# enfiskutensykkel/nvme-strom

Hardware: AMD Instinct MI355X
Metric: SSD→GPU read GiB/s + p50 4KiB IOP latency at 1/2/4/8 MI355X (higher is better)
Workload: dtype uint8

## Files before the change

csrc/engine/core.cc:

```cpp
#include <errno.h>
#include <fcntl.h>
#include <string.h>
#include <sys/mman.h>
#include <time.h>
#include <unistd.h>
#include <x86intrin.h>

#include <new>

#include <chrono>
#include <cstdio>
#include <cstdlib>

#include "engine.h"

namespace strom {

static bool parse_bool(const std::string &v) {
  return v == "1" || v == "true" || v == "yes" || v == "on";
}

Config Config::from_env() {
  Config c;
  static const char *keys[] = {"backend", "workers", "queue_depth", "max_request",
                               "staging_slots", "staging_bytes", "spin_us", "inline_max",
                               "bar_map", "bar_max", "bar_nt", "inline_plain", "coalesce", "trace",
                               "ingest", "ingest_grid", "ingest_piece", "ingest_min", "ingest_prio", "hdp_sync",
                               "fixed_bufs", "io_prof", "fd_kcmp", "stage_by_bytes", "slot_lifo",
                               "strict", "direct_io",
                               "pgcache_probe", "gpu_emulation", "numa_bind", "check_freed",
                               "stat_info", "verbose"};
  for (const char *k : keys) {
    std::string env = "STROM_";
    for (const char *p = k; *p; ++p) env += (char)toupper(*p);
    if (const char *v = getenv(env.c_str())) c.set(k, v);
  }
  return c;
}

int Config::set(const std::string &k, const std::string &v) {
  char *end = nullptr;
  long n = strtol(v.c_str(), &end, 0);
  bool num_ok = end && *end == '\0' && !v.empty();
  if (k == "backend") {
    if (v == "psync") backend = BackendKind::kPsync;
    else if (v == "uring") backend = BackendKind::kUring;
    else if (v == "fake") backend = BackendKind::kFake;
    else if (v == "cache") backend = BackendKind::kCache;
    else return -EINVAL;
    return 0;
  }
  if (k == "strict") { strict = parse_bool(v); return 0; }
  if (k == "direct_io") { direct_io = parse_bool(v); return 0; }
  if (k == "pgcache_probe") { pgcache_probe = parse_bool(v); return 0; }
  if (k == "gpu_emulation") { gpu_emulation = parse_bool(v); return 0; }
  if (k == "numa_bind") { numa_bind = parse_bool(v); return 0; }
  if (k == "check_freed") { check_freed = parse_bool(v); return 0; }
  if (!num_ok) return -EINVAL;
  if (k == "workers") { if (n < 1 || n > 256) return -EINVAL; workers = (int)n; return 0; }
  if (k == "queue_depth") { if (n < 1 || n > 4096) return -EINVAL; queue_depth = (int)n; return 0; }
  if (k == "max_request") {
    if (n < 4096 || n > (64l << 20) || (n & 4095)) return -EINVAL;
    max_request = (uint32_t)n;
    return 0;
  }
  if (k == "staging_slots") { if (n < 1 || n > 1024) return -EINVAL; staging_slots = (int)n; return 0; }
  if (k == "staging_bytes") {
    if (n < 0 || n > (1l << 30)) return -EINVAL;
    staging_bytes = (uint32_t)n;
    return 0;
  }
  if (k == "spin_us") { if (n < 0 || n > 10000) return -EINVAL; spin_us = (uint32_t)n; return 0; }
  if (k == "bar_map") { bar_map = parse_bool(v); return 0; }
  if (k == "coalesce") { coalesce = parse_bool(v); return 0; }
  if (k == "ingest") { ingest = parse_bool(v); return 0; }
  if (k == "hdp_sync") {
    if (!num_ok) { hdp_sync = parse_bool(v) ? 1 : 0; return 0; }
    if (n < 0 || n > 2) return -EINVAL;
    hdp_sync = (int)n;
    return 0;
  }
  if (k == "fixed_bufs") { fixed_bufs = parse_bool(v); return 0; }
  if (k == "io_prof") { io_prof = parse_bool(v); return 0; }
  if (k == "fd_kcmp") { fd_kcmp = parse_bool(v); return 0; }
  if (k == "stage_by_bytes") { stage_by_bytes = parse_bool(v); return 0; }
  if (k == "slot_lifo") { slot_lifo = parse_bool(v); return 0; }
  if (k == "ingest_min") {
    if (n < 0 || n > (64l << 20)) return -EINVAL;
    ingest_min = (uint32_t)n;
    return 0;
  }
  if (k == "ingest_prio") { if (n < 0 || n > 1) return -EINVAL; ingest_prio = (int)n; return 0; }
  if (k == "ingest_grid") { if (n < 1 || n > 256) return -EINVAL; ingest_grid = (int)n; return 0; }
  if (k == "ingest_piece") {
    if (n < 4096 || n > (16l << 20) || (n & 4095)) return -EINVAL;
    ingest_piece = (uint32_t)n;
    return 0;
  }
  if (k == "trace") { trace = parse_bool(v); return 0; }
  if (k == "bar_max") {
    if (n < 0 || n > (64l << 20)) return -EINVAL;
    bar_max = (uint32_t)n;
    return 0;
  }
  if (k == "inline_plain") { inline_plain = parse_bool(v); return 0; }
  if (k == "bar_nt") {
    if (!num_ok) { bar_nt = parse_bool(v) ? 1 : 0; return 0; }
    if (n < 0 || n > 1) return -EINVAL;
    bar_nt = (int)n;
    return 0;
  }
  if (k == "inline_max") {
    if (n < 0 || n > (16l << 20) || (n & 4095)) return -EINVAL;
    inline_max = (uint32_t)n;
    return 0;
  }
  if (k == "stat_info") { stat_info = (int)n; return 0; }
  if (k == "verbose") { verbose = (int)n; return 0; }
  return -ENOENT;
}

int Config::get(const std::string &k, std::string *out) const {
  char buf[64];
  if (k == "backend") {
    *out = backend == BackendKind::kPsync   ? "psync"
           : backend == BackendKind::kUring ? "uring"
           : backend == BackendKind::kCache ? "cache"
                                            : "fake";
    return 0;
  }
  long v;
  if (k == "workers") v = workers;
  else if (k == "queue_depth") v = queue_depth;
  else if (k == "max_request") v = max_request;
  else if (k == "staging_slots") v = staging_slots;
  else if (k == "staging_bytes") v = staging_bytes;
  else if (k == "spin_us") v = spin_us;
  else if (k == "inline_max") v = inline_max;
  else if (k == "bar_map") v = bar_map;
  else if (k == "coalesce") v = coalesce;
  else if (k == "ingest") v = ingest;
  else if (k == "ingest_grid") v = ingest_grid;
  else if (k == "ingest_prio") v = ingest_prio;
  else if (k == "ingest_piece") v = ingest_piece;
  else if (k == "hdp_sync") v = hdp_sync;
  else if (k == "fixed_bufs") v = fixed_bufs;
  else if (k == "io_prof") v = io_prof;
  else if (k == "fd_kcmp") v = fd_kcmp;
  else if (k == "stage_by_bytes") v = stage_by_bytes;
  else if (k == "slot_lifo") v = slot_lifo;
  else if (k == "ingest_min") v = ingest_min;
  else if (k == "trace") v = trace;
  else if (k == "bar_max") v = bar_max;
  else if (k == "bar_nt") v = bar_nt;
  else if (k == "inline_plain") v = inline_plain;
  else if (k == "strict") v = strict;
  else if (k == "direct_io") v = direct_io;
  else if (k == "pgcache_probe") v = pgcache_probe;
  else if (k == "gpu_emulation") v = gpu_emulation;
  else if (k == "numa_bind") v = numa_bind;
  else if (k == "check_freed") v = check_freed;
  else if (k == "stat_info") v = stat_info;
  else if (k == "verbose") v = verbose;
  else return -ENOENT;
  snprintf(buf, sizeof buf, "%ld", v);
  *out = buf;
  return 0;
}

Config &config() {
  static Config c = Config::from_env();
  return c;
}

uint64_t tsc_now() { return __rdtsc(); }

uint64_t mono_ns() {
  timespec ts;
  clock_gettime(CLOCK_MONOTONIC, &ts);
  return (uint64_t)ts.tv_sec * 1000000000ull + (uint64_t)ts.tv_nsec;
}

uint64_t tsc_khz() {
  static const uint64_t khz = [] {
    const uint64_t n0 = mono_ns(), c0 = tsc_now();
    while (mono_ns() - n0 < 5000000) _mm_pause();
    const uint64_t n1 = mono_ns(), c1 = tsc_now();
    return (c1 - c0) * 1000000ull / (n1 - n0);
  }();
  return khz;
}

void Hist::add(uint64_t ns) { b[bucket(ns)].fetch_add(1, std::memory_order_relaxed); }

void Hist::copy_to(uint64_t *out, bool reset) {
  for (int i = 0; i < STROM_HIST_BUCKETS; ++i)
    out[i] = reset ? b[i].exchange(0) : b[i].load();
}

void Stats::inflight_inc(uint64_t n) {
  uint64_t cur = cur_dma_count.fetch_add(n, std::memory_order_relaxed) + n;
  uint64_t mx = max_dma_count.load(std::memory_order_relaxed);
  while (cur > mx && !max_dma_count.compare_exchange_weak(mx, cur)) {
  }
}

void Stats::inflight_dec(uint64_t n) { cur_dma_count.fetch_sub(n, std::memory_order_relaxed); }

int Stats::fill(strom_stat_info *o) {
  if (o->version != 1) return -EINVAL;
  int level = config().stat_info;
  if (level == 0) return -ENODATA;
  o->has_debug = level >= 2;
  o->tsc = tsc_now();
  o->nr_ssd2gpu = nr_ssd2gpu.load();
  o->clk_ssd2gpu = clk_ssd2gpu.load();
  o->nr_setup_prps = nr_setup_prps.load();
  o->clk_setup_prps = clk_setup_prps.load();
  o->nr_submit_dma = nr_submit_dma.load();
  o->clk_submit_dma = clk_submit_dma.load();
  o->nr_wait_dtask = nr_wait_dtask.load();
  o->clk_wait_dtask = clk_wait_dtask.load();
  o->nr_wrong_wakeup = nr_wrong_wakeup.load();
  o->cur_dma_count = cur_dma_count.load();
  o->max_dma_count = max_dma_count.exchange(cur_dma_count.load());
  uint64_t *dn[4] = {&o->nr_debug1, &o->nr_debug2, &o->nr_debug3, &o->nr_debug4};
  uint64_t *dc[4] = {&o->clk_debug1, &o->clk_debug2, &o->clk_debug3, &o->clk_debug4};
  for (int i = 0; i < 4; ++i) {
    *dn[i] = o->has_debug ? nr_debug[i].load() : 0;
    *dc[i] = o->has_debug ? clk_debug[i].load() : 0;
  }
  return 0;
}

int Stats::fill_hist(strom_stat_hist *o) {
  if (o->version != 1) return -EINVAL;
  bool r = o->reset != 0;
  io_ns.copy_to(o->io_ns, r);
  copy_ns.copy_to(o->copy_ns, r);
  task_ns.copy_to(o->task_ns, r);
  return 0;
}

static Stats *make_stats() {
  const char *off = getenv("STROM_STAT_SHM");
  if (!(off && strcmp(off, "0") == 0)) {
    char path[96];
    snprintf(path, sizeof path, "/dev/shm/nvme-strom.%d", (int)getpid());
    int fd = open(path, O_RDWR | O_CREAT | O_TRUNC | O_CLOEXEC, 0644);
    if (fd >= 0) {
      size_t len = sizeof(StatsShmHeader) + sizeof(Stats);
      if (ftruncate(fd, (off_t)len) == 0) {
        void *p = mmap(nullptr, len, PROT_READ | PROT_WRITE, MAP_SHARED, fd, 0);
        if (p != MAP_FAILED) {
          close(fd);
          auto *h = new (p) StatsShmHeader();
          h->magic = kStatsShmMagic;
          h->version = 1;
          h->pid = getpid();
          h->stats_bytes = sizeof(Stats);
          h->tsc_hz_hint = 0;
          static char saved[96];
          memcpy(saved, path, sizeof saved);
          atexit([] { unlink(saved); });
          return new ((char *)p + sizeof(StatsShmHeader)) Stats();
        }
      }
      close(fd);
      unlink(path);
    }
  }
  return new Stats();
}

Stats &stats() {
  static Stats *s = make_stats();
  return *s;
}

CallerProf &caller_prof() {
  static CallerProf p;
  return p;
}

Task *TaskTable::create(int session) {
  Task *t = new Task();
  t->id = next_id_.fetch_add(1);
  t->session = session;
  t->t_start_ns = mono_ns();
  Slot &s = slot_of(t->id);
  std::lock_guard<std::mutex> g(s.mu);
  s.running.emplace(t->id, t);
  return t;
}

void TaskTable::get(Task *t, int n) {
  t->refcnt.fetch_add(n, std::memory_order_relaxed);
}

void TaskTable::put_n(Task *t, int n, long status) {
  if (status != 0) {
    long zero = 0;
    t->status.compare_exchange_strong(zero, status);
  }
  if (t->refcnt.fetch_sub(n, std::memory_order_acq_rel) != n) return;
  stats().task_ns.add(mono_ns() - t->t_start_ns);
  Slot &s = slot_of(t->id);
  {
    std::lock_guard<std::mutex> g(s.mu);
    s.running.erase(t->id);
    s.done_seq.fetch_add(1, std::memory_order_release);
    if (t->status.load() != 0) {
      t->gmap.reset();
      t->dbuf.reset();
      s.failed.emplace(t->id, t);
      t = nullptr;
    }
  }
  s.cv.notify_all();
  delete t;
}

int TaskTable::wait(uint64_t id, long *status, int64_t timeout_ns) {
  Slot &s = slot_of(id);
  uint64_t t0 = tsc_now();
  bool slept = false;
  auto deadline = std::chrono::steady_clock::now() +
                  std::chrono::nanoseconds(timeout_ns < 0 ? 0 : timeout_ns);
  std::unique_lock<std::mutex> g(s.mu);
  int rc;
  bool spun = false;
  uint64_t spin_end = 0;
  for (;;) {
    auto f = s.failed.find(id);
    if (f != s.failed.end()) {
      *status = f->second->status.load();
      delete f->second;
      s.failed.erase(f);
      rc = -EIO;
      break;
    }
    if (s.running.count(id)) {
      if (timeout_ns == 0) { rc = -ETIME; break; }
      if (!spun) {
        spun = true;
        uint64_t spin_ns = (uint64_t)config().spin_us * 1000;
        if (timeout_ns > 0 && (uint64_t)timeout_ns < spin_ns) spin_ns = (uint64_t)timeout_ns;
        spin_end = mono_ns() + spin_ns;
      }
      if (mono_ns() < spin_end) {
        const uint64_t seq0 = s.done_seq.load(std::memory_order_acquire);
        g.unlock();
        while (s.done_seq.load(std::memory_order_acquire) == seq0 && mono_ns() < spin_end)
          for (int i = 0; i < 32; ++i) _mm_pause();
        g.lock();
        continue;
      }
      if (slept) stats().nr_wrong_wakeup++;
      slept = true;
      if (timeout_ns < 0) {
        s.cv.wait(g);
      } else if (s.cv.wait_until(g, deadline) == std::cv_status::timeout &&
                 s.running.count(id)) {
        rc = -ETIME;
        break;
      }
      continue;
    }
    *status = 0;
    rc = (id == 0 || id > last_id()) ? -ENOENT : 0;
    break;
  }
  if (slept) {
    stats().nr_wait_dtask++;
    stats().clk_wait_dtask += tsc_now() - t0;
  }
  return rc;
}

int TaskTable::reclaim(int session) {
  int n = 0;
  for (auto &s : slots_) {
    std::lock_guard<std::mutex> g(s.mu);
    for (auto it = s.failed.begin(); it != s.failed.end();) {
      if (it->second->session == session) {
        delete it->second;
        it = s.failed.erase(it);
        ++n;
      } else {
        ++it;
      }
    }
  }
  return n;
}

TaskTable &tasks() {
  static TaskTable t;
  return t;
}

int FaultInjector::on_request(uint32_t *len) {
  long fa = fail_at.load(std::memory_order_relaxed);
  long sa = short_at.load(std::memory_order_relaxed);
  int d = delay_us.load(std::memory_order_relaxed);
  if (!fa && !sa && !d) return 0;
  long n = counter.fetch_add(1) + 1;
  if (d) {
    timespec ts{0, (long)d * 1000};
    nanosleep(&ts, nullptr);
  }
  if (fa && n == fa) return -err.load();
  if (sa && n == sa) {
    int sb = short_bytes.load();
    *len = (uint32_t)sb >= *len ? 0 : *len - (uint32_t)sb;
  }
  return 0;
}

FaultInjector &faults() {
  static FaultInjector f;
  return f;
}

}
```

csrc/engine/engine.cc:

```cpp
#include <errno.h>
#include <fcntl.h>
#include <stdio.h>
#include <stdlib.h>
#include <string.h>
#include <sys/ioctl.h>
#include <sys/mman.h>
#include <sys/stat.h>
#include <sys/syscall.h>
#include <sys/sysmacros.h>
#include <unistd.h>
#include <x86intrin.h>

#include <rocprofiler-sdk-roctx/roctx.h>

#include <algorithm>
#include <set>
#include <thread>

#include "engine.h"

namespace strom {
static thread_local bool tl_sync_call = false;
thread_local uint64_t *tl_phase = nullptr;


struct Engine::OpenFile {
  dev_t dev = 0;
  ino_t ino = 0;
  struct timespec ctim {};
  off_t vsize = -1;
  int fd_direct = -1;
  int fd_buffered = -1;
  FileClass fc;
  std::mutex mu;
  void *map = nullptr;
  size_t map_len = 0;
  ~OpenFile() {
    if (map) munmap(map, map_len);
    if (fd_direct >= 0 && fd_direct != fd_buffered) close(fd_direct);
    if (fd_buffered >= 0) close(fd_buffered);
  }
  long resident(uint64_t off, uint32_t len) {
    if (!map) return -1;
    if (off >= map_len) return 0;
    uint32_t n = (uint32_t)std::min<uint64_t>(len, map_len - off);
    unsigned char vec[1024];
    uint32_t pages = (n + 4095) / 4096;
    long res = 0;
    for (uint32_t p = 0; p < pages; p += 1024) {
      uint32_t cnt = std::min<uint32_t>(1024, pages - p);
      if (mincore((char *)map + off + (uint64_t)p * 4096, (size_t)cnt * 4096, vec) != 0) return -1;
      for (uint32_t i = 0; i < cnt; ++i) res += vec[i] & 1;
    }
    return res;
  }
};

struct Engine::StripeSet {
  std::vector<std::shared_ptr<OpenFile>> m;
  uint32_t unit = 0;
  uint64_t size = 0;
  Raid0Geometry geo{};
  int numa = -1;
};

static std::mutex g_stripes_mu;
static std::map<int, std::shared_ptr<Engine::StripeSet>> g_stripes;
static int g_next_stripe = 0;

static int stripe_ident_bmap(void *, uint64_t fblk, uint64_t *dblk) {
  *dblk = fblk;
  return 0;
}

static std::mutex g_engine_mu;
static Engine *g_engine = nullptr;

Engine &engine() {
  std::lock_guard<std::mutex> g(g_engine_mu);
  if (!g_engine) g_engine = new Engine();
  return *g_engine;
}

void engine_reset() {
  std::lock_guard<std::mutex> g(g_engine_mu);
  delete g_engine;
  g_engine = nullptr;
}

static std::atomic<uint64_t> g_engine_gen{0};

Engine::Engine() : gen_(g_engine_gen.fetch_add(1) + 1) { io_ = std::make_unique<IoEngine>(config()); }
Engine::~Engine() { io_.reset(); }

static std::atomic<int> g_kcmp{-1};

static bool same_description(int fd, int dup) {
  const pid_t me = getpid();
  const long r = syscall(SYS_kcmp, me, me, 0 , fd, dup);
  if (r < 0 && g_kcmp.load(std::memory_order_relaxed) != 1) g_kcmp.store(0);
  return r == 0;
}

struct TlFile {
  int fd = -1;
  int dup = -1;
  uint64_t eng = 0;
  std::shared_ptr<Engine::OpenFile> f;
  ~TlFile() {
    if (dup >= 0) close(dup);
  }
};
static thread_local TlFile tl_file;

void Engine::forget_cached_file() {
  tl_file.f.reset();
  tl_file.fd = -1;
}

const std::shared_ptr<Engine::OpenFile> &Engine::open_file_cached(int fd, int *err, bool *fast) {
  TlFile &tl = tl_file;
  static const std::shared_ptr<OpenFile> none;
  if (fast) *fast = false;
  const bool use_kcmp = config().fd_kcmp && g_kcmp.load(std::memory_order_relaxed) != 0;
  if (use_kcmp && tl.fd == fd && tl.eng == gen_ && tl.f && tl.dup >= 0 &&
      same_description(fd, tl.dup)) {
    g_kcmp.store(1, std::memory_order_relaxed);
    if (fast) *fast = true;
    return tl.f;
  }
  struct stat st;
  if (fstat(fd, &st) != 0) {
    *err = -errno;
    return none;
  }
  const OpenFile *c = tl.f.get();
  const bool same = tl.fd == fd && tl.eng == gen_ && c && c->dev == st.st_dev && c->ino == st.st_ino &&
                    c->vsize == st.st_size && c->ctim.tv_sec == st.st_ctim.tv_sec &&
                    c->ctim.tv_nsec == st.st_ctim.tv_nsec;
  if (!same) {
    tl.f = open_file(fd, err);
    tl.eng = gen_;
    if (!tl.f) {
      tl.fd = -1;
      return none;
    }
  }
  if (!use_kcmp) {
    if (tl.dup >= 0) close(tl.dup);
    tl.dup = -1;
  } else if (tl.fd != fd || tl.dup < 0 || !same) {
    if (tl.dup >= 0) close(tl.dup);
    tl.dup = fcntl(fd, F_DUPFD_CLOEXEC, 0);
  }
  tl.fd = fd;
  return tl.f;
}

struct TlReg {
  int rfd = -1;
  uint64_t eng = 0, ver = 0;
  std::shared_ptr<Engine::OpenFile> f;
};
static thread_local TlReg tl_reg;

const std::shared_ptr<Engine::OpenFile> &Engine::registered(int rfd) {
  TlReg &tl = tl_reg;
  if (tl.rfd == rfd && tl.eng == gen_ && tl.ver == reg_ver_.load(std::memory_order_acquire))
    return tl.f;
  std::lock_guard<std::mutex> g(reg_mu_);
  const uint32_t i = (uint32_t)(rfd - kRegFdBase);
  tl.f = is_registered_id(rfd) && i < reg_.size() ? reg_[i] : nullptr;
  tl.rfd = rfd;
  tl.eng = gen_;
  tl.ver = reg_ver_.load(std::memory_order_relaxed);
  return tl.f;
}

int Engine::register_file(int fd) {
  if (fd >= kRegFdBase) return -EINVAL;
  int err = 0;
  auto f = open_file(fd, &err);
  if (!f) return err ? err : -EBADF;
  std::lock_guard<std::mutex> g(reg_mu_);
  size_t i = 0;
  while (i < reg_.size() && reg_[i]) ++i;
  if (i >= (size_t)kRegMax) return -EMFILE;
  if (i == reg_.size()) reg_.emplace_back();
  reg_[i] = std::move(f);
  reg_ver_.fetch_add(1, std::memory_order_release);
  return kRegFdBase + (int)i;
}

int Engine::unregister_file(int rfd) {
  std::lock_guard<std::mutex> g(reg_mu_);
  const uint32_t i = (uint32_t)(rfd - kRegFdBase);
  if (!is_registered_id(rfd) || i >= reg_.size() || !reg_[i]) return -EBADF;
  reg_[i].reset();
  reg_ver_.fetch_add(1, std::memory_order_release);
  return 0;
}

void Engine::refresh_registered(int rfd) {
  std::shared_ptr<OpenFile> f = registered(rfd);
  if (!f) return;
  int err = 0;
  auto nf = open_file(f->fd_buffered, &err);
  if (!nf || nf == f) return;
  std::lock_guard<std::mutex> g(reg_mu_);
  const uint32_t i = (uint32_t)(rfd - kRegFdBase);
  if (i < reg_.size() && reg_[i] == f) {
    reg_[i] = nf;
    reg_ver_.fetch_add(1, std::memory_order_release);
  }
}

std::shared_ptr<Engine::OpenFile> Engine::task_file(int fd, int *err) {
  if (is_registered_id(fd)) refresh_registered(fd);
  return open_file(fd, err);
}

std::shared_ptr<Engine::OpenFile> Engine::open_file(int fd, int *err) {
  if (is_registered_id(fd)) {
    std::shared_ptr<OpenFile> f = registered(fd);
    if (!f) *err = -EBADF;
    return f;
  }
  struct stat st;
  if (fstat(fd, &st) != 0) {
    *err = -errno;
    return nullptr;
  }
  std::lock_guard<std::mutex> g(files_mu_);
  auto key = std::make_pair(st.st_dev, st.st_ino);
  auto it = files_.find(key);
  if (it != files_.end()) {
    std::shared_ptr<OpenFile> f = it->second;
    if (f->vsize == st.st_size && f->ctim.tv_sec == st.st_ctim.tv_sec &&
        f->ctim.tv_nsec == st.st_ctim.tv_nsec)
      return f;
    struct stat cst;
    bool stale = fstat(f->fd_buffered, &cst) != 0 || cst.st_nlink == 0 ||
                 cst.st_ino != st.st_ino;
    if (!stale) {
      f->ctim = st.st_ctim;
      f->vsize = st.st_size;
      if ((off_t)f->fc.size != st.st_size) {
        std::lock_guard<std::mutex> fg(f->mu);
        f->fc.size = st.st_size;
        if (f->map) munmap(f->map, f->map_len);
        f->map = nullptr;
        if (config().pgcache_probe && st.st_size > 0) {
          void *m = mmap(nullptr, (size_t)st.st_size, PROT_READ, MAP_SHARED, f->fd_buffered, 0);
          if (m != MAP_FAILED) {
            f->map = m;
            f->map_len = (size_t)st.st_size;
          }
        }
      }
      return f;
    }
    files_.erase(it);
  }
  auto f = std::make_shared<OpenFile>();
  int rc = classify_file(fd, &f->fc, config().strict);
  if (rc) {
    *err = rc;
    return nullptr;
  }
  char path[64];
  snprintf(path, sizeof path, "/proc/self/fd/%d", fd);
  f->fd_buffered = open(path, O_RDONLY | O_CLOEXEC);
  if (f->fd_buffered < 0) f->fd_buffered = fcntl(fd, F_DUPFD_CLOEXEC, 0);
  if (f->fd_buffered < 0) {
    *err = -errno;
    return nullptr;
  }
  f->fd_direct = f->fd_buffered;
  if (config().direct_io) {
    int d = open(path, O_RDONLY | O_DIRECT | O_CLOEXEC);
    if (d >= 0) f->fd_direct = d;
  }
  f->dev = st.st_dev;
  f->ino = st.st_ino;
  f->ctim = st.st_ctim;
  f->vsize = st.st_size;
  if (config().pgcache_probe && st.st_size > 0) {
    void *m = mmap(nullptr, (size_t)st.st_size, PROT_READ, MAP_SHARED, f->fd_buffered, 0);
    if (m != MAP_FAILED) {
      f->map = m;
      f->map_len = (size_t)st.st_size;
    }
  }
  if (files_.size() > 256) files_.clear();
  files_[key] = f;
  return f;
}

static void attach_residency(Engine::OpenFile *fp, PlanParams *pp,
                             std::vector<unsigned char> *vec, uint64_t *lo_out) {
  uint64_t lo = UINT64_MAX, hi = 0;
  for (uint32_t i = 0; i < pp->nr_chunks; ++i) {
    uint64_t c = pp->relseg_sz ? pp->ids[i] % pp->relseg_sz : pp->ids[i];
    uint64_t f = c * pp->chunk_sz;
    lo = std::min(lo, f);
    hi = std::max(hi, f + pp->chunk_sz);
  }
  hi = std::min<uint64_t>(hi, fp->map_len);
  uint64_t total = (uint64_t)pp->nr_chunks * pp->chunk_sz;
  uint64_t t0 = tsc_now();
  if (lo < hi && hi - lo <= 4 * total) {
    vec->resize((hi - lo + 4095) / 4096);
    if (mincore((char *)fp->map + lo, hi - lo, vec->data()) == 0) {
      *lo_out = lo;
      std::vector<unsigned char> *v = vec;
      uint64_t base = lo, end = hi;
      pp->resident = [v, base, end](uint64_t off, uint32_t len) -> long {
        if (off >= end) return 0;
        uint64_t e = std::min<uint64_t>(off + len, end);
        long r = 0;
        for (uint64_t p = (off - base) >> 12; p < ((e - base + 4095) >> 12); ++p) r += (*v)[p] & 1;
        return r;
      };
      stats().nr_debug[2].fetch_add(1, std::memory_order_relaxed);
      stats().clk_debug[2].fetch_add(tsc_now() - t0, std::memory_order_relaxed);
      return;
    }
  }
  pp->resident = [fp](uint64_t off, uint32_t len) { return fp->resident(off, len); };
}

int Engine::stripe_open(const int *fds, uint32_t n, uint32_t unit, uint64_t size) {
  if (!fds || n == 0 || n > STROM_RAID0_MAX_DISKS) return -EINVAL;
  if (unit < 4096 || (unit & 4095) || size == 0) return -EINVAL;
  auto ss = std::make_shared<StripeSet>();
  ss->unit = unit;
  ss->size = size;
  const uint64_t nstripes = (size + unit - 1) / unit;
  std::set<int> nodes;
  for (uint32_t k = 0; k < n; ++k) {
    int err = 0;
    auto f = open_file(fds[k], &err);
    if (!f) return err;
    const uint64_t mine = nstripes > k ? (nstripes - k + n - 1) / n : 0;
    uint64_t need = mine * (uint64_t)unit;
    if (mine && (nstripes - 1) % n == k) need -= (uint64_t)unit * nstripes - size;
    if ((uint64_t)f->fc.size < need) return -ERANGE;
    nodes.insert(f->fc.numa_node);
    ss->m.push_back(f);
  }
  ss->numa = nodes.size() == 1 ? *nodes.begin() : -1;
  Raid0Geometry &g = ss->geo;
  g.chunk_sects = unit >> 9;
  g.nzones = 1;
  g.ndisks = n;
  const uint64_t rows = (nstripes + n - 1) / n + ((64ull << 20) / ((uint64_t)unit * n)) + 1;
  g.zone_end[0] = rows * n * (uint64_t)(unit >> 9);
  g.zone_dev_start[0] = 0;
  g.zone_nb_dev[0] = n;
  for (uint32_t k = 0; k < n; ++k) g.zone_devs[0][k] = (uint8_t)k;
  if (strom_core_raid0_check(&g)) return -EINVAL;
  std::lock_guard<std::mutex> l(g_stripes_mu);
  if (g_stripes.size() >= 4096) return -EMFILE;
  int fd;
  do {
    fd = kStripeFdBase + (g_next_stripe++ & 0xffffff);
  } while (g_stripes.count(fd));
  g_stripes[fd] = ss;
  return fd;
}

int Engine::stripe_close(int sfd) {
  std::lock_guard<std::mutex> l(g_stripes_mu);
  return g_stripes.erase(sfd) ? 0 : -EBADF;
}

std::shared_ptr<Engine::StripeSet> Engine::stripe(int fd) {
  if (fd < kStripeFdBase) return nullptr;
  std::lock_guard<std::mutex> l(g_stripes_mu);
  auto it = g_stripes.find(fd);
  return it == g_stripes.end() ? nullptr : it->second;
}

int Engine::check_file(strom_check_file *a) {
  if (a->fdesc >= kStripeFdBase) {
    auto ss = stripe(a->fdesc);
    if (!ss) return -EBADF;
    a->numa_node_id = ss->numa;
    a->support_dma64 = 1;
    return 0;
  }
  FileClass fc;
  if (is_registered_id(a->fdesc)) {
    int err = 0;
    const auto f = task_file(a->fdesc, &err);
    if (!f) return err ? err : -EBADF;
    fc = f->fc;
  } else {
    int rc = classify_file(a->fdesc, &fc, config().strict);
    if (rc) return rc;
  }
  a->numa_node_id = fc.numa_node;
  a->support_dma64 = fc.dma64 ? 1 : 0;
  return 0;
}

static int copy_ram_chunks(int fd, const ChunkPlan &plan, uint32_t chunk_sz, uint64_t file_size,
                           char *dest_base) {
  uint64_t t0 = tsc_now();
  for (size_t i = 0; i < plan.ram_fpos.size(); ++i) {
    char *dst = dest_base + plan.ram_dest[i];
    uint64_t fpos = plan.ram_fpos[i];
    uint32_t want = (uint32_t)std::min<uint64_t>(chunk_sz, file_size - fpos);
    uint32_t done = 0;
    while (done < want) {
      ssize_t n = pread(fd, dst + done, want - done, (off_t)(fpos + done));
      if (n < 0) {
        if (errno == EINTR) continue;
        return -errno;
      }
      if (n == 0) break;
      done += (uint32_t)n;
    }
    if (done < chunk_sz) memset(dst + done, 0, chunk_sz - done);
  }
  stats().nr_debug[1].fetch_add(plan.ram_fpos.size(), std::memory_order_relaxed);
  stats().clk_debug[1].fetch_add(tsc_now() - t0, std::memory_order_relaxed);
  return 0;
}

static void build_requests(Task *t, const ChunkPlan &plan, int fd_direct, int fd_buffered,
                           uint64_t file_size, GpuMapping *gmap, uint64_t dest_base,
                           bool dest_is_host, std::vector<IoReq> *out,
                           const Engine::StripeSet *ss = nullptr) {
  uint64_t t0 = tsc_now();
  out->reserve(plan.ssd.size());
  const uint64_t now_ns = mono_ns(), now_tsc = tsc_now();
  for (const IoRange &r : plan.ssd) {
    IoReq q;
    q.task = t;
    q.fd = fd_direct;
    q.fd_buffered = fd_buffered;
    q.off = r.file_off;
    q.len = r.len;
    q.valid = (uint32_t)std::min<uint64_t>(r.len, file_size > r.file_off ? file_size - r.file_off : 0);
    if (ss && r.member >= 0) {
      const auto &mf = ss->m[(size_t)r.member];
      q.fd = mf->fd_direct;
      q.fd_buffered = mf->fd_buffered;
      q.off = r.msect << 9;
    }
    if (dest_is_host) {
      q.host_dst = (uint8_t *)(dest_base + r.dest_off);
    } else {
      q.gpu_dst = dest_base + r.dest_off;
      q.device = gmap->device;
    }
    q.gmap = gmap;
    q.t_submit_ns = now_ns;
    q.t_submit_tsc = now_tsc;
    out->push_back(q);
  }
  if (const int n = (int)plan.ssd.size()) {
    tasks().get(t, n);
    if (gmap) gmap->inflight.fetch_add(n);
    stats().inflight_inc((uint64_t)n);
  }
  stats().nr_setup_prps.fetch_add(plan.ssd.size(), std::memory_order_relaxed);
  stats().clk_setup_prps.fetch_add(tsc_now() - t0, std::memory_order_relaxed);
}

int Engine::memcpy_ssd2gpu(int session, strom_memcpy_ssd2gpu *a) {
  a->nr_ram2gpu = a->nr_ssd2gpu = a->nr_dma_submit = a->nr_dma_blocks = 0;
  a->dma_task_id = 0;
  if (a->nr_chunks == 0) return -EINVAL;
  if (!a->chunk_ids) return -EFAULT;
  auto gmap = gpu_registry().get(a->handle);
  if (!gmap) return -ENOENT;
  if (int v = gpu_registry().validate(gmap)) return v;
  uint64_t bytes = (uint64_t)a->nr_chunks * a->chunk_sz;
  if (strom_core_check_range(gmap->map_length - gmap->map_offset, a->offset, bytes))
    return -ERANGE;
  int err = 0;
  auto ss = stripe(a->file_desc);
  std::shared_ptr<OpenFile> f;
  if (!ss) {
    if (a->file_desc >= kStripeFdBase) return -EBADF;
    f = task_file(a->file_desc, &err);
    if (!f) return err;
  }

  PlanParams pp;
  pp.ids = a->chunk_ids;
  pp.nr_chunks = a->nr_chunks;
  pp.chunk_sz = a->chunk_sz;
  pp.relseg_sz = a->relseg_sz;
  pp.file_size = ss ? ss->size : (uint64_t)f->fc.size;
  pp.max_request = config().max_request;
  pp.reorder = true;
  if (ss) {
    pp.raid0 = &ss->geo;
    pp.bmap = stripe_ident_bmap;
  }
  phase_mark(0);
  const uint64_t c0 = tsc_now();
  std::vector<unsigned char> resv;
  uint64_t res_lo = 0;
  if (f && config().pgcache_probe && f->map) attach_residency(f.get(), &pp, &resv, &res_lo);
  ChunkPlan plan;
  int rc = plan_chunks(pp, &plan);
  if (rc) return rc;
  phase_mark(1);
  const uint64_t c1 = tsc_now();
  char *ram_dest = a->wb_buffer;
  if (plan.nr_ram && !ram_dest) {
    uint64_t dva = gmap->va + a->offset;
    if (!gmap->bar || dva < gmap->bar_va || dva + bytes > gmap->bar_va + gmap->bar_len)
      return -EFAULT;
    ram_dest = (char *)gmap->bar + (dva - gmap->bar_va);
  }

  Task *t = tasks().create(session);
  t->gmap = gmap;
  bool host_dest = gmap->device < 0;
  std::vector<IoReq> reqs;
  build_requests(t, plan, f ? f->fd_direct : -1, f ? f->fd_buffered : -1, pp.file_size,
                 gmap.get(), gmap->va + a->offset, host_dest, &reqs, ss.get());
  phase_mark(2);
  uint64_t t0 = tsc_now();
  if (reqs.size() == 1 && (reqs[0].len <= config().inline_max || tl_sync_call))
    io_->run_inline(reqs[0]);
  else
    io_->submit(reqs);
  const uint64_t t1 = tsc_now();
  stats().nr_submit_dma.fetch_add(reqs.size(), std::memory_order_relaxed);
  stats().clk_submit_dma.fetch_add(t1 - t0, std::memory_order_relaxed);
  if (config().io_prof) {
    CallerProf &cp = caller_prof();
    cp.calls.fetch_add(1, std::memory_order_relaxed);
    cp.plan.fetch_add(c1 - c0, std::memory_order_relaxed);
    cp.build.fetch_add(t0 - c1, std::memory_order_relaxed);
    cp.submit.fetch_add(t1 - t0, std::memory_order_relaxed);
  }

  if (plan.nr_ram && f) {
    rc = copy_ram_chunks(f->fd_buffered, plan, a->chunk_sz, pp.file_size, ram_dest);
    if (rc == 0 && !a->wb_buffer) gmap->bar_flush((const uint8_t *)ram_dest, true);
  }
  t->frozen = true;
  uint64_t id = t->id;
  tasks().put(t, rc);
  if (rc) {
    long st;
    tasks().wait(id, &st, -1);
    return rc;
  }
  a->dma_task_id = id;
  a->nr_ram2gpu = plan.nr_ram;
  a->nr_ssd2gpu = plan.nr_ssd;
  a->nr_dma_submit = plan.nr_submit;
  a->nr_dma_blocks = plan.nr_blocks;
  memcpy(a->chunk_ids, plan.ids_out.data(), sizeof(uint32_t) * a->nr_chunks);
  return 0;
}

int Engine::memcpy_extents(int session, strom_memcpy_ssd2gpu_extents *a) {
  a->dma_task_id = 0;
  a->nr_dma_submit = a->nr_dma_blocks = 0;
  a->bytes_read = a->gap_bytes = a->dst_bytes = 0;
  if (a->nr_extents && !a->extents) return -EFAULT;
  if (a->nr_extents > (1u << 24) || (a->flags & ~STROM_EXTENTS_PLAN_ONLY)) return -EINVAL;
  int err = 0;
  auto ss = stripe(a->file_desc);
  std::shared_ptr<OpenFile> f;
  if (!ss) {
    if (a->file_desc >= kStripeFdBase) return -EBADF;
    f = task_file(a->file_desc, &err);
    if (!f) return err;
  }
  PlanParams pp;
  pp.file_size = ss ? ss->size : (uint64_t)f->fc.size;
  pp.max_request = config().max_request;
  if (ss) {
    pp.raid0 = &ss->geo;
    pp.bmap = stripe_ident_bmap;
  }
  const bool plan_only = a->flags & STROM_EXTENTS_PLAN_ONLY;
  std::shared_ptr<GpuMapping> gmap;
  if (!plan_only) {
    gmap = gpu_registry().get(a->handle);
    if (!gmap) return -ENOENT;
    if (int v = gpu_registry().validate(gmap)) return v;
  }
  ChunkPlan plan;
  uint64_t dst_bytes = 0, read_bytes = 0;
  int rc = plan_xfer(pp, a->extents, a->nr_extents, a->gap_max, !plan_only, &plan, &dst_bytes,
                     &read_bytes);
  if (rc) return rc;
  uint64_t want = 0;
  for (uint32_t i = 0; i < a->nr_extents; ++i) want += a->extents[i].len;
  a->dst_bytes = dst_bytes;
  a->bytes_read = read_bytes;
  a->gap_bytes = read_bytes - want;
  if (plan_only) return 0;
  if (strom_core_check_range(gmap->map_length - gmap->map_offset, a->offset, dst_bytes))
    return -ERANGE;
  Task *t = tasks().create(session);
  t->gmap = gmap;
  const bool host_dest = gmap->device < 0;
  std::vector<IoReq> reqs;
  build_requests(t, plan, f ? f->fd_direct : -1, f ? f->fd_buffered : -1, pp.file_size,
                 gmap.get(), gmap->va + a->offset, host_dest, &reqs, ss.get());
  const uint64_t t0 = tsc_now();
  if (reqs.size() == 1 && (reqs[0].len <= config().inline_max || tl_sync_call))
    io_->run_inline(reqs[0]);
  else if (!reqs.empty())
    io_->submit(reqs);
  stats().nr_submit_dma.fetch_add(reqs.size(), std::memory_order_relaxed);
  stats().clk_submit_dma.fetch_add(tsc_now() - t0, std::memory_order_relaxed);
  t->frozen = true;
  const uint64_t id = t->id;
  tasks().put(t, 0);
  a->dma_task_id = id;
  a->nr_dma_submit = plan.nr_submit;
  a->nr_dma_blocks = plan.nr_blocks;
  return 0;
}

long Engine::pread_sync(unsigned long handle, size_t offset, int fd, uint64_t file_off,
                        uint64_t len, bool checked) {
  if (len > (16u << 20)) return -EAGAIN;
  if (fd >= kStripeFdBase) return -EAGAIN;
  const auto &gmap = gpu_registry().get_cached(handle);
  if (!gmap) return -ENOENT;
  if (int v = gpu_registry().validate(gmap)) return v;
  if (strom_core_check_range(gmap->map_length - gmap->map_offset, offset, len)) return -ERANGE;
  phase_mark(0);
  int err = 0;
  bool fast = false;
  const bool reg = is_registered_id(fd);
  const auto &f = reg ? registered(fd) : open_file_cached(fd, &err, &fast);
  if (!f) return reg ? -EBADF : err;
  fast |= reg;
  auto recheck = [&] {
    if (reg) refresh_registered(fd);
    else forget_cached_file();
    return pread_sync(handle, offset, fd, file_off, len, true);
  };
  const uint64_t size = (uint64_t)f->fc.size;
  if (file_off >= size) {
    if (!fast || checked) return -ERANGE;
    return recheck();
  }
  phase_mark(1);
  long status = 0;
  IoReq r;
  r.fd = f->fd_direct;
  r.fd_buffered = f->fd_buffered;
  r.off = file_off;
  r.len = (uint32_t)len;
  r.valid = (uint32_t)std::min<uint64_t>(len, size - file_off);
  if (gmap->device < 0) r.host_dst = (uint8_t *)(gmap->va + offset);
  else r.gpu_dst = gmap->va + offset;
  r.device = gmap->device;
  r.gmap = gmap.get();
  r.status_out = &status;
  r.t_submit_ns = mono_ns();
  r.t_submit_tsc = tsc_now();
  gmap->inflight.fetch_add(1);
  stats().inflight_inc();
  stats().nr_setup_prps.fetch_add(1, std::memory_order_relaxed);
  phase_mark(2);
  io_->run_inline(r);
  if (status == -EIO && fast && !checked) {
    return recheck();
  }
  if (status) return status;
  return (long)len;
}

int Engine::memcpy_ssd2ram(int session, strom_memcpy_ssd2ram *a) {
  a->nr_ram2ram = a->nr_ssd2ram = a->nr_dma_submit = a->nr_dma_blocks = 0;
  a->dma_task_id = 0;
  if (a->nr_chunks == 0) return -EINVAL;
  if (!a->chunk_ids || !a->dest_uaddr) return -EFAULT;
  uint64_t bytes = (uint64_t)a->nr_chunks * a->chunk_sz;
  std::shared_ptr<DmaBuffer> dbuf;
  size_t dest_off = 0;
  int rc = dmabuf_registry().resolve(a->dest_uaddr, bytes, &dbuf, &dest_off);
  if (rc) return rc;
  int err = 0;
  auto ss = stripe(a->file_desc);
  std::shared_ptr<OpenFile> f;
  if (!ss) {
    if (a->file_desc >= kStripeFdBase) return -EBADF;
    f = task_file(a->file_desc, &err);
    if (!f) return err;
  }

  PlanParams pp;
  pp.ids = a->chunk_ids;
  pp.nr_chunks = a->nr_chunks;
  pp.chunk_sz = a->chunk_sz;
  pp.relseg_sz = a->relseg_sz;
  pp.file_size = ss ? ss->size : (uint64_t)f->fc.size;
  pp.max_request = config().max_request;
  pp.reorder = false;
  if (ss) {
    pp.raid0 = &ss->geo;
    pp.bmap = stripe_ident_bmap;
  }
  std::vector<unsigned char> resv;
  uint64_t res_lo = 0;
  if (f && config().pgcache_probe && f->map) attach_residency(f.get(), &pp, &resv, &res_lo);
  ChunkPlan plan;
  rc = plan_chunks(pp, &plan);
  if (rc) return rc;

  Task *t = tasks().create(session);
  t->dbuf = dbuf;
  std::vector<IoReq> reqs;
  build_requests(t, plan, f ? f->fd_direct : -1, f ? f->fd_buffered : -1, pp.file_size, nullptr,
                 (uint64_t)a->dest_uaddr, true, &reqs, ss.get());
  uint64_t t0 = tsc_now();
  if (reqs.size() == 1 && (reqs[0].len <= config().inline_max || tl_sync_call))
    io_->run_inline(reqs[0]);
  else
    io_->submit(reqs);
  stats().nr_submit_dma.fetch_add(reqs.size(), std::memory_order_relaxed);
  stats().clk_submit_dma.fetch_add(tsc_now() - t0, std::memory_order_relaxed);
  if (plan.nr_ram && f)
    rc = copy_ram_chunks(f->fd_buffered, plan, a->chunk_sz, pp.file_size, (char *)a->dest_uaddr);
  t->frozen = true;
  uint64_t id = t->id;
  tasks().put(t, rc);
  if (rc) {
    long st;
    tasks().wait(id, &st, -1);
    return rc;
  }
  a->dma_task_id = id;
  a->nr_ram2ram = plan.nr_ram;
  a->nr_ssd2ram = plan.nr_ssd;
  a->nr_dma_submit = plan.nr_submit;
  a->nr_dma_blocks = plan.nr_blocks;
  return 0;
}

int Engine::memcpy_wait(strom_memcpy_wait *a) {
  long st = 0;
  int rc = tasks().wait(a->dma_task_id, &st, -1);
  a->status = st;
  return rc;
}

int Engine::memcpy_wait_timed(strom_memcpy_wait_timed *a) {
  long st = 0;
  int rc = tasks().wait(a->dma_task_id, &st, (int64_t)a->timeout_ns);
  a->status = st;
  return rc;
}

namespace {
const char *cmd_name(unsigned long cmd) {
  switch (cmd) {
    case STROM_IOCTL__CHECK_FILE: return "strom:CHECK_FILE";
    case STROM_IOCTL__MAP_GPU_MEMORY: return "strom:MAP_GPU_MEMORY";
    case STROM_IOCTL__MAP_GPU_DMABUF: return "strom:MAP_GPU_DMABUF";
    case STROM_IOCTL__UNMAP_GPU_MEMORY: return "strom:UNMAP_GPU_MEMORY";
    case STROM_IOCTL__MEMCPY_SSD2GPU: return "strom:MEMCPY_SSD2GPU";
    case STROM_IOCTL__MEMCPY_SSD2RAM: return "strom:MEMCPY_SSD2RAM";
    case STROM_IOCTL__MEMCPY_WAIT: return "strom:MEMCPY_WAIT";
    case STROM_IOCTL__MEMCPY_WAIT_TIMED: return "strom:MEMCPY_WAIT_TIMED";
    case STROM_IOCTL__MEMCPY_SSD2GPU_EXTENTS: return "strom:MEMCPY_SSD2GPU_EXTENTS";
    default: return "strom:ioctl";
  }
}
struct TraceRange {
  bool on;
  explicit TraceRange(unsigned long cmd) : on(config().trace) {
    if (on) roctxRangePushA(cmd_name(cmd));
  }
  ~TraceRange() {
    if (on) roctxRangePop();
  }
};
}

int Engine::ioctl(int session, unsigned long cmd, void *arg) {
  if (!arg) return -EFAULT;
  TraceRange tr(cmd);
  switch (cmd) {
    case STROM_IOCTL__CHECK_FILE:
      return check_file((strom_check_file *)arg);
    case STROM_IOCTL__MAP_GPU_MEMORY: {
      auto *a = (strom_map_gpu_memory *)arg;
      return gpu_registry().map(a->vaddress, a->length, -1, a);
    }
    case STROM_IOCTL__MAP_GPU_DMABUF: {
      auto *a = (strom_map_gpu_dmabuf *)arg;
      strom_map_gpu_memory m{};
      int rc = gpu_registry().map(a->vaddress, a->length, a->dmabuf_fd, &m);
      a->handle = m.handle;
      a->gpu_page_sz = m.gpu_page_sz;
      a->gpu_npages = m.gpu_npages;
      return rc;
    }
    case STROM_IOCTL__UNMAP_GPU_MEMORY:
      return gpu_registry().unmap(((strom_unmap_gpu_memory *)arg)->handle);
    case STROM_IOCTL__LIST_GPU_MEMORY:
      return gpu_registry().list((strom_list_gpu_memory *)arg);
    case STROM_IOCTL__INFO_GPU_MEMORY:
      return gpu_registry().info((strom_info_gpu_memory *)arg);
    case STROM_IOCTL__ALLOC_DMA_BUFFER: {
      auto *a = (strom_alloc_dma_buffer *)arg;
      return dmabuf_registry().alloc(a->length, a->node_id, &a->dmabuf_fdesc);
    }
    case STROM_IOCTL__MEMCPY_SSD2GPU:
      return memcpy_ssd2gpu(session, (strom_memcpy_ssd2gpu *)arg);
    case STROM_IOCTL__MEMCPY_SSD2RAM:
      return memcpy_ssd2ram(session, (strom_memcpy_ssd2ram *)arg);
    case STROM_IOCTL__MEMCPY_SSD2GPU_EXTENTS:
      return memcpy_extents(session, (strom_memcpy_ssd2gpu_extents *)arg);
    case STROM_IOCTL__MEMCPY_WAIT:
      return memcpy_wait((strom_memcpy_wait *)arg);
    case STROM_IOCTL__MEMCPY_WAIT_TIMED:
      return memcpy_wait_timed((strom_memcpy_wait_timed *)arg);
    case STROM_IOCTL__STAT_INFO:
      return stats().fill((strom_stat_info *)arg);
    case STROM_IOCTL__STAT_HIST:
      return stats().fill_hist((strom_stat_hist *)arg);
    case STROM_IOCTL__SET_ROUTE:
      return -EOPNOTSUPP;
    default:
      return -EINVAL;
  }
}

}

using namespace strom;

static std::mutex g_sess_mu;
static int g_next_session = 1;
static std::atomic<int> g_kernel_fd{-2};

static int kernel_fd() {
  const int k = g_kernel_fd.load(std::memory_order_acquire);
  if (k != -2) return k;
  std::lock_guard<std::mutex> g(g_sess_mu);
  int fd = g_kernel_fd.load(std::memory_order_relaxed);
  if (fd != -2) return fd;
  const char *prov = getenv("STROM_PROVIDER");
  if (prov && strcmp(prov, "user") == 0) {
    fd = -1;
  } else {
    fd = open(STROM_DEVICE_PATHNAME, O_RDONLY | O_CLOEXEC);
    if (fd < 0) fd = open(NVME_STROM_IOCTL_PATHNAME, O_RDONLY | O_CLOEXEC);
  }
  g_kernel_fd.store(fd, std::memory_order_release);
  return fd;
}

static int kernel_map_gpu(int kfd, strom_map_gpu_memory *a) {
  if (!hip::available()) return -ENODEV;
  int dfd = -1, dev = -1;
  uint64_t off = 0;
  int rc = hip::export_dmabuf(a->vaddress, a->length, &dfd, &off, &dev);
  if (rc) return rc;
  strom_map_gpu_dmabuf m{};
  m.dmabuf_fd = dfd;
  m.device_id = dev;
  m.vaddress = a->vaddress;
  m.length = a->length;
  m.dmabuf_offset = off;
  int r = ioctl(kfd, STROM_IOCTL__MAP_GPU_DMABUF, &m);
  int e = errno;
  close(dfd);
  if (r < 0) return -e;
  a->handle = m.handle;
  a->gpu_page_sz = m.gpu_page_sz;
  a->gpu_npages = m.gpu_npages;
  return 0;
}

extern "C" {

const char *strom_version(void) { return "strom-mi355x 0.1.0 (abi nvme-strom 0.6)"; }

int strom_provider(void) { return kernel_fd() >= 0 ? 1 : 0; }

int strom_open(void) {
  std::lock_guard<std::mutex> g(g_sess_mu);
  return g_next_session++;
}

int strom_close(int session) {
  if (session <= 0) return -EBADF;
  int n = tasks().reclaim(session);
  if (n) STROM_LOG(0, "session %d closed with %d unclaimed failed task(s)", session, n);
  return n;
}

int strom_ioctl(int session, unsigned long cmd, void *arg) {
  const int kfd = kernel_fd();
  if (kfd >= 0) {
    if (cmd == STROM_IOCTL__MAP_GPU_MEMORY) return kernel_map_gpu(kfd, (strom_map_gpu_memory *)arg);
    int r = ioctl(kfd, cmd, arg);
    return r < 0 ? -errno : r;
  }
  return engine().ioctl(session, cmd, arg);
}

int nvme_strom_ioctl(unsigned long cmd, const void *arg) {
  static thread_local int session = 0;
  if (session == 0) session = strom_open();
  int r = strom_ioctl(session, cmd, (void *)arg);
  if (r < 0) {
    errno = -r;
    return -1;
  }
  return r;
}

long strom_pread_gpu(int session, unsigned long handle, size_t offset, int fd,
                     uint64_t file_off, uint64_t len) {
  if ((file_off | len) & 4095) return -EINVAL;
  if (len == 0) return 0;
  {
    const int kfd = kernel_fd();
    if (kfd < 0) {
      const long r = engine().pread_sync(handle, offset, fd, file_off, len);
      if (r != -EAGAIN) return r;
    }
  }
  uint32_t chunk = 4096;
  for (uint32_t c = config().max_request; c > 4096; c >>= 1)
    if (file_off % c == 0 && len % c == 0) {
      chunk = c;
      break;
    }
  uint64_t n = len / chunk;
  if (n > (1u << 24) || (file_off / chunk + n) > 0xffffffffull) return -E2BIG;
  uint32_t ids_small[16];
  std::vector<uint32_t> ids_big;
  uint32_t *ids = ids_small;
  if (n > 16) {
    ids_big.resize(n);
    ids = ids_big.data();
  }
  for (uint64_t i = 0; i < n; ++i) ids[i] = (uint32_t)(file_off / chunk + i);
  auto gmap = gpu_registry().get(handle);
  if (!gmap) return -ENOENT;
  strom_memcpy_ssd2gpu a{};
  a.handle = handle;
  a.offset = offset;
  a.file_desc = fd;
  a.nr_chunks = (unsigned)n;
  a.chunk_sz = chunk;
  a.chunk_ids = ids;
  std::vector<char> wb;
  if (!gmap->bar) {
    wb.resize(len);
    a.wb_buffer = wb.data();
  }
  strom::tl_sync_call = true;
  int rc = strom_ioctl(session, STROM_IOCTL__MEMCPY_SSD2GPU, &a);
  strom::tl_sync_call = false;
  if (rc) return rc;
  strom_memcpy_wait w{};
  w.dma_task_id = a.dma_task_id;
  rc = strom_ioctl(session, STROM_IOCTL__MEMCPY_WAIT, &w);
  if (rc) return rc;
  if (a.nr_ram2gpu) {
    uint64_t dva = gmap->va + offset;
    const bool host = gmap->device < 0;
    auto hipMemcpyDtoH_wrap = [&](void *dst, uint64_t src, size_t nb) -> int {
      if (host) {
        memcpy(dst, (const void *)src, nb);
        return 0;
      }
      return hip::copy_dtoh(dst, src, nb);
    };
    auto hipMemcpyHtoD_wrap = [&](uint64_t dst, const void *src, size_t nb) -> int {
      if (host) {
        memcpy((void *)dst, src, nb);
        return 0;
      }
      return hip::copy_htod(dst, src, nb);
    };
    std::vector<char> tmp(len);
    const char *src = gmap->bar ? (const char *)gmap->bar + (dva - gmap->bar_va) : nullptr;
    if (!src) {
      if (hipMemcpyDtoH_wrap(tmp.data(), dva, (size_t)a.nr_ssd2gpu * chunk) != 0) return -EIO;
      memcpy(tmp.data() + (size_t)a.nr_ssd2gpu * chunk, wb.data() + (size_t)a.nr_ssd2gpu * chunk,
             (size_t)a.nr_ram2gpu * chunk);
    } else {
      memcpy(tmp.data(), src, len);
    }
    std::vector<char> out(len);
    for (uint64_t i = 0; i < n; ++i) {
      uint64_t pos = ids[i] - file_off / chunk;
      memcpy(out.data() + pos * chunk, tmp.data() + i * chunk, chunk);
    }
    if (gmap->bar) {
      if (!gmap->bar_write(dva, out.data(), len)) return -EIO;
    } else if (hipMemcpyHtoD_wrap(dva, out.data(), len) != 0) {
      return -EIO;
    }
  }
  return (long)len;
}

int strom_pread_gpu_lat(int session, unsigned long handle, size_t offset, int fd,
                        const uint64_t *file_offs, uint32_t n, uint64_t len, uint64_t *ns_out) {
  for (uint32_t i = 0; i < n; ++i) {
    const uint64_t t0 = mono_ns();
    const long r = strom_pread_gpu(session, handle, offset, fd, file_offs[i], len);
    ns_out[i] = mono_ns() - t0;
    if (r < 0) return (int)r;
  }
  return 0;
}

int strom_ioctl_lat(int session, unsigned long handle, size_t offset, int fd,
                    const uint64_t *file_offs, uint32_t n, uint64_t len, uint64_t *ns_out) {
  if (len == 0 || (len & 4095) || len > (1u << 20)) return -EINVAL;
  uint32_t ids[256];
  const uint32_t chunk = 4096, nch = (uint32_t)(len / chunk);
  std::vector<char> wb(len);
  for (uint32_t i = 0; i < n; ++i) {
    const uint64_t t0 = mono_ns();
    for (uint32_t k = 0; k < nch; ++k) ids[k] = (uint32_t)(file_offs[i] / chunk + k);
    strom_memcpy_ssd2gpu a{};
    a.handle = handle;
    a.offset = offset;
    a.file_desc = fd;
    a.nr_chunks = nch;
    a.chunk_sz = chunk;
    a.chunk_ids = ids;
    a.wb_buffer = wb.data();
    int rc = strom_ioctl(session, STROM_IOCTL__MEMCPY_SSD2GPU, &a);
    if (rc) return rc;
    strom_memcpy_wait w{};
    w.dma_task_id = a.dma_task_id;
    rc = strom_ioctl(session, STROM_IOCTL__MEMCPY_WAIT, &w);
    ns_out[i] = mono_ns() - t0;
    if (rc) return rc;
  }
  return 0;
}

int strom_pread_gpu_phases(int session, unsigned long handle, size_t offset, int fd,
                           const uint64_t *file_offs, uint32_t n, uint64_t len,
                           uint64_t *phase_ns) {
  uint64_t st[STROM_NPHASE];
  for (uint32_t i = 0; i < n; ++i) {
    memset(st, 0, sizeof st);
    strom::tl_phase = st;
    const uint64_t t0 = mono_ns();
    const long r = strom_pread_gpu(session, handle, offset, fd, file_offs[i], len);
    st[STROM_NPHASE - 1] = mono_ns();
    strom::tl_phase = nullptr;
    if (r < 0) return (int)r;
    for (int k = 0; k < STROM_NPHASE; ++k)
      phase_ns[(size_t)i * STROM_NPHASE + k] = st[k] ? st[k] - t0 : 0;
  }
  return 0;
}

int strom_pread_raw_lat(int fd, const uint64_t *file_offs, uint32_t n, uint64_t len,
                        uint64_t *ns_out) {
  if (len == 0 || (len & 4095)) return -EINVAL;
  char path[64];
  snprintf(path, sizeof path, "/proc/self/fd/%d", fd);
  int d = open(path, O_RDONLY | O_DIRECT | O_CLOEXEC);
  if (d < 0) return -errno;
  void *buf = nullptr;
  if (posix_memalign(&buf, 4096, len) != 0) {
    close(d);
    return -ENOMEM;
  }
  int rc = 0;
  for (uint32_t i = 0; i < n && rc == 0; ++i) {
    const uint64_t t0 = mono_ns();
    const ssize_t got = pread(d, buf, len, (off_t)file_offs[i]);
    ns_out[i] = mono_ns() - t0;
    if (got < 0) rc = -errno;
  }
  free(buf);
  close(d);
  return rc;
}

int strom_pread_pair_lat(int session, unsigned long handle, size_t offset, int fd,
                         const uint64_t *file_offs, uint32_t npairs, uint64_t len,
                         uint64_t *ns_engine, uint64_t *ns_raw) {
  if (len == 0 || (len & 4095)) return -EINVAL;
  int real = fd;
  if (is_registered_id(fd)) {
    const auto &f = engine().registered(fd);
    if (!f) return -EBADF;
    real = f->fd_buffered;
  }
  char path[64];
  snprintf(path, sizeof path, "/proc/self/fd/%d", real);
  int d = open(path, O_RDONLY | O_DIRECT | O_CLOEXEC);
  if (d < 0) return -errno;
  void *buf = nullptr;
  if (posix_memalign(&buf, 4096, len) != 0) {
    close(d);
    return -ENOMEM;
  }
  int rc = 0;
  for (uint32_t i = 0; i < npairs && rc == 0; ++i) {
    for (int side = 0; side < 2 && rc == 0; ++side) {
      const bool raw = (side == 0) == ((i & 1) == 0);
      const uint64_t off = file_offs[2 * i + (raw ? 0 : 1)];
      const uint64_t t0 = mono_ns();
      if (raw) {
        const ssize_t got = pread(d, buf, len, (off_t)off);
        ns_raw[i] = mono_ns() - t0;
        if (got < 0) rc = -errno;
      } else {
        const long r = strom_pread_gpu(session, handle, offset, fd, off, len);
        ns_engine[i] = mono_ns() - t0;
        if (r < 0) rc = (int)r;
      }
    }
  }
  free(buf);
  close(d);
  return rc;
}

int strom_host_costs(int fd, uint64_t *out, int n) {
  if (n <= 0 || fd < 0) return -EINVAL;
  auto bench = [&](auto &&fn) {
    const uint64_t t0 = mono_ns();
    for (int i = 0; i < n; ++i) fn();
    return (mono_ns() - t0) / (uint64_t)n;
  };
  volatile uint64_t sink = 0;
  timespec ts;
  out[0] = bench([&] { clock_gettime(CLOCK_MONOTONIC, &ts); sink += ts.tv_nsec; });
  out[1] = bench([&] { sink += __rdtsc(); });
  struct stat st;
  out[2] = bench([&] { fstat(fd, &st); sink += st.st_size; });
  void *m = mmap(nullptr, 4096, PROT_READ, MAP_SHARED, fd, 0);
  unsigned char v = 0;
  out[3] = m == MAP_FAILED ? 0 : bench([&] { mincore(m, 4096, &v); sink += v; });
  if (m != MAP_FAILED) munmap(m, 4096);
  out[4] = bench([&] { sink += (uint64_t)getppid(); });
  std::mutex mu;
  out[5] = bench([&] { std::lock_guard<std::mutex> g(mu); sink += 1; });
  std::condition_variable cv;
  out[6] = bench([&] { cv.notify_all(); });
  const int d = fcntl(fd, F_DUPFD_CLOEXEC, 0);
  const pid_t me = getpid();
  out[7] = d < 0 || syscall(SYS_kcmp, me, me, 0 , fd, d) != 0
               ? 0
               : bench([&] { sink += (uint64_t)syscall(SYS_kcmp, me, me, 0, fd, d); });
  if (d >= 0) close(d);
  struct statx sx;
  out[8] = bench([&] {
    statx(fd, "", AT_EMPTY_PATH | AT_STATX_DONT_SYNC, STATX_INO, &sx);
    sink += sx.stx_ino;
  });
  return 0;
}

int strom_engine_costs(unsigned long handle, int fd, uint64_t *out, int n) {
  using namespace strom;
  if (n <= 0 || fd < 0) return -EINVAL;
  auto bench = [&](auto &&fn) {
    const uint64_t t0 = mono_ns();
    for (int i = 0; i < n; ++i) fn();
    return (mono_ns() - t0) / (uint64_t)n;
  };
  volatile uint64_t sink = 0;
  auto g = gpu_registry().get(handle);
  if (!g) return -ENOENT;
  out[0] = bench([&] { sink += (uint64_t)(gpu_registry().get(handle) != nullptr); });
  out[1] = bench([&] { sink += (uint64_t)gpu_registry().validate(g); });
  int err = 0;
  out[2] = bench([&] { sink += (uint64_t)(engine().open_file(fd, &err) != nullptr); });
  out[3] = bench([&] {
    Stats &st = stats();
    st.copy_ns.add(1000);
    st.nr_debug[0].fetch_add(1, std::memory_order_relaxed);
    st.inflight_inc();
    g->inflight.fetch_add(1);
    long status = 0;
    IoReq r;
    r.gmap = g.get();
    r.status_out = &status;
    r.t_submit_tsc = tsc_now();
    finish_request(r, 0);
    sink += (uint64_t)status;
  });
  out[4] = bench([&] { sink += (uint64_t)(gpu_registry().get_cached(handle) != nullptr); });
  out[5] = bench([&] { sink += (uint64_t)(engine().open_file_cached(fd, &err) != nullptr); });
  for (int k = 6; k < 16; ++k) out[k] = 0;
  if (g->bar && g->length >= 4096 && g->va >= g->bar_va && g->va + 4096 <= g->bar_va + g->bar_len) {
    alignas(64) static thread_local uint8_t keep[4096], src[4096];
    memcpy(keep, g->bar + (g->va - g->bar_va), 4096);
    memcpy(src, keep, 4096);
    std::atomic<uint64_t> ctr{0};
    for (int mode = 0; mode < 4; ++mode) {
      uint64_t store = 0, lock = 0;
      for (int i = 0; i < n; ++i) {
        const uint64_t t0 = mono_ns();
        g->bar_write_mode(g->va, src, 4096, mode);
        const uint64_t t1 = mono_ns();
        ctr.fetch_add(1);
        const uint64_t t2 = mono_ns();
        store += t1 - t0;
        lock += t2 - t1;
      }
      out[6 + 2 * mode] = store / (uint64_t)n;
      out[7 + 2 * mode] = lock / (uint64_t)n;
    }
    for (int variant = 0; variant < 2; ++variant) {
      std::atomic<uint64_t> go{0}, done{0};
      std::atomic<bool> quit{false};
      std::thread helper([&] {
        uint64_t seen = 0;
        while (!quit.load(std::memory_order_acquire)) {
          const uint64_t v = go.load(std::memory_order_acquire);
          if (v == seen) {
            _mm_pause();
            continue;
          }
          seen = v;
          if (variant == 0) g->bar_write_mode(g->va + 2048, src + 2048, 2048, 1);
          done.fetch_add(1, std::memory_order_acq_rel);
        }
      });
      uint64_t tot = 0;
      for (int i = 0; i < n; ++i) {
        const uint64_t t0 = mono_ns();
        go.fetch_add(1, std::memory_order_acq_rel);
        if (variant == 0) g->bar_write_mode(g->va, src, 2048, 1);
        ctr.fetch_add(1);
        while (done.load(std::memory_order_acquire) != (uint64_t)i + 1) _mm_pause();
        tot += mono_ns() - t0;
      }
      quit.store(true, std::memory_order_release);
      helper.join();
      out[14 + variant] = tot / (uint64_t)n;
    }
    g->bar_write(g->va, keep, 4096, true);
    sink += ctr.load();
  }
  return 0;
}

void *strom_dmabuf_mmap(int fd, size_t length) {
  void *p = nullptr;
  if (kernel_fd() >= 0) {
    p = mmap(nullptr, length, PROT_READ | PROT_WRITE, MAP_SHARED, fd, 0);
    return p == MAP_FAILED ? nullptr : p;
  }
  int rc = dmabuf_registry().map(fd, length, &p);
  if (rc) {
    errno = -rc;
    return nullptr;
  }
  return p;
}

int strom_dmabuf_munmap(void *addr, size_t length) {
  if (kernel_fd() >= 0) return munmap(addr, length) == 0 ? 0 : -errno;
  return dmabuf_registry().unmap(addr, length);
}

int strom_dmabuf_gc(void) { return dmabuf_registry().gc(); }

int strom_stripe_open(const int *fds, uint32_t n, uint32_t unit, uint64_t size) {
  if (kernel_fd() >= 0) return -EOPNOTSUPP;
  return engine().stripe_open(fds, n, unit, size);
}

int strom_stripe_close(int sfd) { return engine().stripe_close(sfd); }

int strom_register_file(int fd) { return engine().register_file(fd); }
int strom_unregister_file(int rfd) { return engine().unregister_file(rfd); }

int strom_file_topology(int fd, strom_file_topo *out) {
  if (!out) return -EFAULT;
  FileClass fc;
  int rc = classify_file(fd, &fc, false);
  if (rc) return rc;
  memset(out, 0, sizeof *out);
  out->dev_major = major(fc.dev);
  out->dev_minor = minor(fc.dev);
  out->numa_node = fc.numa_node;
  snprintf(out->fs_name, sizeof out->fs_name, "%s", fc.fs_name.c_str());
  snprintf(out->disk, sizeof out->disk, "%s", fc.disk.c_str());
  std::vector<std::string> members;
  if (fc.md_raid0) members = fc.members;
  else if (!fc.disk.empty()) members.push_back(fc.disk);
  for (auto &m : members) {
    if (out->nmembers >= STROM_TOPO_MAX_MEMBERS) break;
    std::string disk = m;
    size_t pp = disk.rfind('p');
    if (pp != std::string::npos && disk.compare(0, 4, "nvme") == 0 &&
        disk.find('n', 4) != std::string::npos && disk.find('n', 4) < pp)
      disk = disk.substr(0, pp);
    snprintf(out->member_disk[out->nmembers], 32, "%s", m.c_str());
    snprintf(out->member_pci[out->nmembers], 16, "%s", nvme_controller_bdf(disk).c_str());
    ++out->nmembers;
  }
  return 0;
}


long strom_gpu_detached(void) { return (long)gpu_registry().detached_count(); }

long strom_gpu_bar_bytes(unsigned long handle) {
  auto m = gpu_registry().get(handle);
  if (!m) return -ENOENT;
  return (long)(m->bar ? m->bar_len : 0);
}

int strom_export_dmabuf(uint64_t va, uint64_t len, int *fd, uint64_t *offset) {
  if (!hip::available()) return -ENODEV;
  int dev = -1;
  return hip::export_dmabuf(va, len, fd, offset, &dev);
}

int strom_config_set(const char *key, const char *value) {
  std::lock_guard<std::mutex> g(g_engine_mu);
  return config().set(key, value);
}

int strom_config_get(const char *key, char *buf, size_t buflen) {
  std::string v;
  int rc = config().get(key, &v);
  if (rc) return rc;
  if (v.size() + 1 > buflen) return -ENOSPC;
  memcpy(buf, v.c_str(), v.size() + 1);
  return 0;
}

int strom_engine_reset(void) {
  engine_reset();
  return 0;
}

int strom_fake_backend(uint64_t seed, uint64_t *completions, uint64_t *reordered) {
  FaultInjector &f = faults();
  if (seed) f.fake_seed = seed;
  if (completions) *completions = f.fake_completions.load();
  if (reordered) *reordered = f.fake_reordered.load();
  return 0;
}

int strom_fault_inject(long fail_at, int err, long short_at, int short_bytes, int delay_us) {
  FaultInjector &f = faults();
  f.counter = 0;
  f.fail_at = fail_at;
  f.err = err ? err : EIO;
  f.short_at = short_at;
  f.short_bytes = short_bytes;
  f.delay_us = delay_us;
  return 0;
}

long strom_resident_bytes(int fd, uint64_t offset, uint64_t length) {
  struct stat st;
  if (fstat(fd, &st) != 0) return -errno;
  if (offset >= (uint64_t)st.st_size) return 0;
  length = std::min<uint64_t>(length, (uint64_t)st.st_size - offset);
  uint64_t lo = offset & ~4095ull;
  size_t maplen = (size_t)(offset + length - lo);
  void *m = mmap(nullptr, maplen, PROT_READ, MAP_SHARED, fd, (off_t)lo);
  if (m == MAP_FAILED) return -errno;
  size_t pages = (maplen + 4095) / 4096;
  std::vector<unsigned char> vec(pages);
  long res = 0;
  if (mincore(m, maplen, vec.data()) == 0) {
    for (auto v : vec) res += v & 1;
  } else {
    res = -errno;
  }
  munmap(m, maplen);
  return res < 0 ? res : res * 4096;
}

int strom_evict_file(int fd) {
  fdatasync(fd);
  int r = posix_fadvise(fd, 0, 0, POSIX_FADV_DONTNEED);
  return -r;
}

int strom_raid0_map(const uint64_t *zone_end, const uint64_t *zone_dev_start,
                    const int *zone_nb_dev, int nzones, uint32_t chunk_sects,
                    const uint64_t *data_offset, int raid_disks, uint64_t sector,
                    uint32_t nr_sects, int *member, uint64_t *member_sector) {
  if (nzones <= 0 || nzones > STROM_RAID0_MAX_ZONES || raid_disks <= 0 ||
      raid_disks > STROM_RAID0_MAX_DISKS)
    return -EINVAL;
  strom_raid0 g;
  memset(&g, 0, sizeof g);
  g.chunk_sects = chunk_sects;
  g.nzones = (uint32_t)nzones;
  g.ndisks = (uint32_t)raid_disks;
  for (int z = 0; z < nzones; ++z) {
    g.zone_end[z] = zone_end[z];
    g.zone_dev_start[z] = zone_dev_start[z];
    if (zone_nb_dev[z] <= 0 || zone_nb_dev[z] > raid_disks) return -EINVAL;
    g.zone_nb_dev[z] = (uint32_t)zone_nb_dev[z];
    for (int k = 0; k < zone_nb_dev[z]; ++k)
      g.zone_devs[z][k] = (uint8_t)(raid_disks - zone_nb_dev[z] + k);
  }
  for (int d = 0; d < raid_disks; ++d) g.data_offset[d] = data_offset ? data_offset[d] : 0;
  return strom_core_raid0_map(&g, sector, nr_sects, member, member_sector);
}

}
```

csrc/engine/engine.h:

```cpp
#pragma once

#include <sys/types.h>

#include <atomic>
#include <condition_variable>
#include <cstdint>
#include <deque>
#include <functional>
#include <map>
#include <memory>
#include <mutex>
#include <string>
#include <thread>
#include <unordered_map>
#include <vector>

#include "strom/strom.h"
#include "../../kmod/strom_core.h"

namespace strom {

enum class BackendKind { kPsync, kUring, kFake, kCache };

struct Config {
  BackendKind backend = BackendKind::kUring;
  int workers = 4;
  int queue_depth = 8;
  uint32_t max_request = 1u << 20;
  int staging_slots = 4;
  bool slot_lifo = true;
  bool stage_by_bytes = true;
  uint32_t staging_bytes = 0;
  uint32_t spin_us = 20;
  uint32_t inline_max = 64u << 10;
  bool bar_map = true;
  bool coalesce = true;
  bool ingest = true;
  int ingest_grid = 16;
  int ingest_prio = 1;
  uint32_t ingest_piece = 256u << 10;
  int hdp_sync = 2;
  bool fixed_bufs = true;
  uint32_t bar_max = 256u << 10;
  int bar_nt = 1;
  bool inline_plain = false;
  uint32_t ingest_min = 0;
  bool io_prof = false;
  bool fd_kcmp = false;
  bool strict = false;
  bool direct_io = true;
  bool pgcache_probe = true;
  bool gpu_emulation = false;
  bool numa_bind = true;
  bool check_freed = true;
  int stat_info = 1;
  int verbose = 0;
  bool trace = false;

  static Config from_env();
  int set(const std::string &key, const std::string &value);
  int get(const std::string &key, std::string *out) const;
};

Config &config();

uint64_t tsc_now();
uint64_t mono_ns();
uint64_t tsc_khz();

struct Hist {
  std::atomic<uint64_t> b[STROM_HIST_BUCKETS];
  static int bucket(uint64_t ns) {
    int k = ns ? 64 - __builtin_clzll(ns) : 0;
    return k >= STROM_HIST_BUCKETS ? STROM_HIST_BUCKETS - 1 : k;
  }
  void add(uint64_t ns);
  void copy_to(uint64_t *out, bool reset);
};

struct Stats {
  std::atomic<uint64_t> nr_ssd2gpu{0}, clk_ssd2gpu{0};
  std::atomic<uint64_t> nr_setup_prps{0}, clk_setup_prps{0};
  std::atomic<uint64_t> nr_submit_dma{0}, clk_submit_dma{0};
  std::atomic<uint64_t> nr_wait_dtask{0}, clk_wait_dtask{0};
  std::atomic<uint64_t> nr_wrong_wakeup{0};
  std::atomic<uint64_t> cur_dma_count{0}, max_dma_count{0};
  std::atomic<uint64_t> nr_debug[4]{}, clk_debug[4]{};
  Hist io_ns, copy_ns, task_ns;

  void inflight_inc(uint64_t n = 1);
  void inflight_dec(uint64_t n = 1);
  int fill(strom_stat_info *out);
  int fill_hist(strom_stat_hist *out);
};

Stats &stats();

struct CallerProf {
  std::atomic<uint64_t> calls{0}, plan{0}, build{0}, submit{0};
};
CallerProf &caller_prof();

static_assert(sizeof(Stats) == (11 + 8 + 3 * STROM_HIST_BUCKETS) * 8, "Stats export layout");

constexpr uint64_t kStatsShmMagic = 0x53544f524d535431ull;
struct StatsShmHeader {
  uint64_t magic;
  uint32_t version;
  int32_t pid;
  uint64_t stats_bytes;
  uint64_t tsc_hz_hint;
  uint64_t reserved[4];
};

struct GpuMapping;
struct DmaBuffer;

struct Task {
  uint64_t id = 0;
  int session = 0;
  std::atomic<int> refcnt{1};
  std::atomic<long> status{0};
  bool frozen = false;
  uint64_t t_start_ns = 0;
  std::shared_ptr<GpuMapping> gmap;
  std::shared_ptr<DmaBuffer> dbuf;
};

class TaskTable {
 public:
  static constexpr int kSlots = 512;
  Task *create(int session);
  void get(Task *t, int n = 1);
  void put(Task *t, long status) { put_n(t, 1, status); }
  void put_n(Task *t, int n, long status);
  int wait(uint64_t id, long *status, int64_t timeout_ns);
  int reclaim(int session);
  uint64_t last_id() const { return next_id_.load() - 1; }

 private:
  struct Slot {
    std::mutex mu;
    std::condition_variable cv;
    std::unordered_map<uint64_t, Task *> running;
    std::unordered_map<uint64_t, Task *> failed;
    std::atomic<uint64_t> done_seq{0};
  };
  Slot &slot_of(uint64_t id) { return slots_[(id * 0x9E3779B97F4A7C15ull) >> 55]; }
  Slot slots_[kSlots];
  std::atomic<uint64_t> next_id_{1};
};

TaskTable &tasks();

struct GpuMapping {
  unsigned long handle = 0;
  uint64_t va = 0;
  uint64_t base = 0;
  size_t length = 0;
  size_t map_offset = 0;
  size_t map_length = 0;
  int device = -1;
  uid_t owner = 0;
  int dmabuf_fd = -1;
  uint32_t version = 1;
  uint64_t ident = 0;
  uint8_t *bar = nullptr;
  uint64_t bar_va = 0;
  size_t bar_len = 0;
  volatile uint32_t *hdp = nullptr;
  std::atomic<int> inflight{0};
  bool bar_write(uint64_t dst, const void *src, size_t len, bool flush = true) const;
  bool bar_write_mode(uint64_t dst, const void *src, size_t len, int mode) const;
  void bar_flush(const uint8_t *last, bool batch = false) const;
  ~GpuMapping();
  bool detached = false;
  std::atomic<bool> draining{false};
  std::mutex mu;
  std::condition_variable cv;
};

class GpuRegistry {
 public:
  int map(uint64_t va, size_t len, int dmabuf_fd, strom_map_gpu_memory *out);
  int unmap(unsigned long handle);
  int list(strom_list_gpu_memory *out);
  int info(strom_info_gpu_memory *out);
  std::shared_ptr<GpuMapping> get(unsigned long handle);
  const std::shared_ptr<GpuMapping> &get_cached(unsigned long handle);
  int validate(const std::shared_ptr<GpuMapping> &m);
  uint64_t detached_count() const { return detached_.load(); }

 private:
  std::mutex mu_;
  std::map<unsigned long, std::shared_ptr<GpuMapping>> maps_;
  unsigned long next_ = 0x5350000000000000ul;
  std::atomic<uint64_t> detached_{0};
  std::atomic<uint64_t> gen_{1};
};

GpuRegistry &gpu_registry();

struct DmaBuffer {
  dev_t dev = 0;
  ino_t ino = 0;
  size_t length = 0;
  int node = -1;
  uint64_t gen = 0;
};

struct VmaInfo {
  uint64_t start = 0, end = 0, pgoff = 0, ino = 0;
  dev_t dev = 0;
  bool dmabuf = false;
};
int vma_query(uint64_t addr, VmaInfo *out);

class DmaBufRegistry {
 public:
  int alloc(size_t length, int node, int *user_fd);
  int resolve(const void *uaddr, size_t len, std::shared_ptr<DmaBuffer> *buf,
              size_t *offset);
  int map(int fd, size_t len, void **addr);
  int unmap(void *addr, size_t len);
  int gc();
  size_t count();

 private:
  struct Range {
    uint64_t end;
    size_t pgoff;
    std::shared_ptr<DmaBuffer> buf;
  };
  std::mutex mu_;
  uint64_t next_gen_ = 1;
  std::map<std::pair<dev_t, ino_t>, std::shared_ptr<DmaBuffer>> bufs_;
  std::map<uint64_t, Range> ranges_;
};

DmaBufRegistry &dmabuf_registry();

using Raid0Geometry = strom_raid0;

struct FileClass {
  dev_t dev = 0;
  ino_t ino = 0;
  off_t size = 0;
  uint32_t fs_bsize = 0;
  uint64_t fs_magic = 0;
  std::string fs_name;
  std::string disk;
  bool nvme = false;
  bool md_raid0 = false;
  int numa_node = -1;
  bool dma64 = true;
  uint64_t part_start_sect = 0;
  Raid0Geometry raid0{};
  std::vector<std::string> members;
};

int classify_file(int fd, FileClass *out, bool strict);
std::string nvme_controller_bdf(const std::string &disk);

struct IoRange {
  uint64_t file_off;
  uint64_t dest_off;
  uint32_t len;
  int member;
  uint64_t msect = 0;
};

struct ChunkPlan {
  std::vector<IoRange> ssd;
  std::vector<uint64_t> ram_fpos;
  std::vector<uint64_t> ram_dest;
  std::vector<uint32_t> ids_out;
  uint32_t nr_ram = 0, nr_ssd = 0, nr_submit = 0, nr_blocks = 0;
};

struct PlanParams {
  const uint32_t *ids = nullptr;
  uint32_t nr_chunks = 0;
  uint32_t chunk_sz = 0;
  uint32_t relseg_sz = 0;
  uint64_t file_size = 0;
  uint32_t max_request = 1u << 20;
  uint64_t dest_segment = 0;
  bool reorder = true;
  const Raid0Geometry *raid0 = nullptr;
  uint64_t part_start_sect = 0;
  int (*bmap)(void *ctx, uint64_t fblk, uint64_t *dblk) = nullptr;
  void *bmap_ctx = nullptr;
  std::function<long(uint64_t, uint32_t)> resident;
};

int plan_chunks(const PlanParams &p, ChunkPlan *out);
int plan_xfer(const PlanParams &p, strom_file_extent *x, uint32_t n, uint32_t gap_max,
              bool planner, ChunkPlan *out, uint64_t *dst_bytes, uint64_t *read_bytes);

struct IoReq {
  Task *task = nullptr;
  int fd = -1;
  int fd_buffered = -1;
  uint64_t off = 0;
  uint32_t len = 0;
  uint32_t valid = 0;
  uint8_t *host_dst = nullptr;
  uint64_t gpu_dst = 0;
  int device = -1;
  uint64_t t_submit_ns = 0;
  uint64_t t_submit_tsc = 0;
  GpuMapping *gmap = nullptr;
  long *status_out = nullptr;
};

class IoEngine {
 public:
  explicit IoEngine(const Config &cfg);
  ~IoEngine();
  void submit(std::vector<IoReq> &reqs);
  static constexpr int kProfPhases = 11, kProfCounts = 5;
  int prof(uint64_t *out, int nout, bool reset);
  void run_inline(IoReq &r);
  int workers() const { return (int)workers_.size(); }

  struct Worker;
 private:
  std::vector<std::unique_ptr<Worker>> workers_;
  std::mutex prof_mu_;
  std::atomic<uint32_t> rr_{0};
};

void finish_request(IoReq &r, long status);

struct FaultInjector {
  std::atomic<long> counter{0};
  std::atomic<long> fail_at{0};
  std::atomic<int> err{5};
  std::atomic<long> short_at{0};
  std::atomic<int> short_bytes{0};
  std::atomic<int> delay_us{0};
  int on_request(uint32_t *len);
  std::atomic<uint64_t> fake_seed{0x5eed};
  std::atomic<uint64_t> fake_completions{0}, fake_reordered{0};
};
FaultInjector &faults();

class Ingest {
 public:
  static Ingest *get(int device);
  bool post(const void *src, uint64_t dst, uint32_t len, uint64_t *seq);
  bool post_many(const void *src, uint64_t dst, uint32_t len, uint32_t piece, uint64_t *first,
                 uint32_t *n);
  struct Run {
    const void *src;
    uint64_t dst;
    uint32_t len;
    bool ok;
    uint64_t first;
    uint32_t n;
  };
  void post_runs(Run *runs, size_t nruns, uint32_t piece);
  bool is_done(uint64_t seq) const;
  void retired(uint32_t n);
  void idle();
  void shutdown();
  void info(uint64_t *out);

 private:
  explicit Ingest(int device);
  bool init();
  int launch_grid();
  int start_locked();
  bool write_desc(uint64_t s, const void *src, uint64_t dst, uint32_t len);

  int device_;
  uint32_t nslots_ = 0, grid_ = 0;
  void *host_ = nullptr, *ring_ = nullptr, *next_ = nullptr;
  volatile uint64_t *done_ = nullptr, *stop_ = nullptr;
  void *stream_ = nullptr, *end_ev_ = nullptr;
  std::mutex mu_;
  std::atomic<uint64_t> post_seq_{0};
  std::atomic<uint64_t> state_{0};
  bool launched_ = false;
  std::atomic<bool> dead_{false};
  std::atomic<bool> gone_{false};
  uint64_t nr_launch_ = 0;
};

namespace hip {
bool available();
int device_count();
int pointer_device(uint64_t va, uint64_t *alloc_base, size_t *alloc_size);
void *host_alloc(size_t bytes, bool coherent = false);
void host_free(void *p);
void *host_alloc_thp(size_t bytes, bool uncached = false);
void host_free_thp(void *p, size_t bytes);
uint8_t *bar_map(uint64_t va, size_t len, uint64_t *map_va, size_t *map_len);
volatile uint32_t *hdp_flush_reg(int device);
void bar_unmap(uint8_t *p, size_t len);
int export_dmabuf(uint64_t va, size_t len, int *fd, uint64_t *offset, int *device);
int copy_dtoh(void *dst, uint64_t src, size_t len);
int copy_htod(uint64_t dst, const void *src, size_t len);
int numa_node_of_device(int device);
uint64_t buffer_id(uint64_t va);
}

class Engine {
 public:
  const uint64_t gen_;
  Engine();
  ~Engine();
  int ioctl(int session, unsigned long cmd, void *arg);
  long pread_sync(unsigned long handle, size_t offset, int fd, uint64_t file_off, uint64_t len,
                  bool checked = false);
  IoEngine &io() { return *io_; }
  struct OpenFile;
  int stripe_open(const int *fds, uint32_t n, uint32_t unit, uint64_t size);
  int stripe_close(int sfd);
  struct StripeSet;

  std::shared_ptr<OpenFile> open_file(int fd, int *err);
  const std::shared_ptr<OpenFile> &open_file_cached(int fd, int *err, bool *fast = nullptr);
  void forget_cached_file();

  int register_file(int fd);
  int unregister_file(int rfd);
  const std::shared_ptr<OpenFile> &registered(int rfd);

 private:
  int check_file(strom_check_file *a);
  int memcpy_ssd2gpu(int session, strom_memcpy_ssd2gpu *a);
  int memcpy_extents(int session, strom_memcpy_ssd2gpu_extents *a);
  int memcpy_ssd2ram(int session, strom_memcpy_ssd2ram *a);
  int memcpy_wait(strom_memcpy_wait *a);
  int memcpy_wait_timed(strom_memcpy_wait_timed *a);

  std::shared_ptr<StripeSet> stripe(int fd);
  void refresh_registered(int rfd);
  std::shared_ptr<OpenFile> task_file(int fd, int *err);

  std::unique_ptr<IoEngine> io_;
  std::mutex files_mu_;
  std::map<std::pair<dev_t, ino_t>, std::shared_ptr<OpenFile>> files_;
  std::mutex reg_mu_;
  std::vector<std::shared_ptr<OpenFile>> reg_;
  std::atomic<uint64_t> reg_ver_{0};
};

constexpr int kStripeFdBase = 0x7f000000;
constexpr int kRegFdBase = 0x7e000000;
constexpr int kRegMax = 4096;
inline bool is_registered_id(int fd) { return fd >= kRegFdBase && fd < kRegFdBase + kRegMax; }

Engine &engine();
void engine_reset();

extern thread_local uint64_t *tl_phase;
inline void phase_mark(int k) {
  if (__builtin_expect(tl_phase != nullptr, 0)) tl_phase[k] = mono_ns();
}

#define STROM_LOG(lvl, ...)                                   \
  do {                                                        \
    if (::strom::config().verbose >= (lvl)) {                 \
      fprintf(stderr, "[strom] " __VA_ARGS__);                \
      fputc('\n', stderr);                                    \
    }                                                         \
  } while (0)

}
```

csrc/engine/ingest.cc:

```cpp
#include <hip/hip_runtime_api.h>
#include <errno.h>
#include <stdlib.h>
#include <string.h>
#include <x86intrin.h>

#include "engine.h"

extern "C" __attribute__((weak)) int strom_ingest_kernel_launch(const void *, void *, const void *,
                                                                void *, uint32_t, uint64_t,
                                                                uint32_t, void *) {
  return -ENOSYS;
}

namespace strom {

namespace {
struct IngestDesc {
  uint64_t src;
  uint64_t dst;
  uint64_t len_tag;
  volatile uint64_t seq;
};
static_assert(sizeof(IngestDesc) == 32, "ingest descriptor layout (ingest.hip)");

std::mutex g_ing_mu;
std::map<int, Ingest *> g_ing;
bool g_ing_atexit = false;

void stop_all_at_exit() {
  std::lock_guard<std::mutex> g(g_ing_mu);
  for (auto &kv : g_ing)
    if (kv.second) kv.second->shutdown();
}
}

Ingest *Ingest::get(int device) {
  if (device < 0 || !config().ingest || !hip::available()) return nullptr;
  std::lock_guard<std::mutex> g(g_ing_mu);
  auto it = g_ing.find(device);
  if (it != g_ing.end()) return it->second;
  Ingest *ing = new Ingest(device);
  if (!ing->init()) {
    STROM_LOG(0, "device %d: ingest grid unavailable, staged copies use SDMA", device);
    delete ing;
    ing = nullptr;
  } else if (!g_ing_atexit) {
    g_ing_atexit = true;
    atexit(stop_all_at_exit);
  }
  g_ing[device] = ing;
  return ing;
}

Ingest::Ingest(int device) : device_(device) {}

bool Ingest::init() {
  nslots_ = 4096;
  grid_ = (uint32_t)std::max(1, std::min(256, config().ingest_grid));
  if (hipSetDevice(device_) != hipSuccess) return false;
  const size_t bytes = nslots_ * sizeof(IngestDesc) + nslots_ * sizeof(uint64_t) + 64;
  void *h = nullptr;
  if (hipHostMalloc(&h, bytes, hipHostMallocCoherent | hipHostMallocPortable) != hipSuccess) {
    (void)hipGetLastError();
    return false;
  }
  memset(h, 0, bytes);
  host_ = h;
  ring_ = h;
  done_ = (volatile uint64_t *)((char *)h + nslots_ * sizeof(IngestDesc));
  stop_ = (volatile uint64_t *)((char *)done_ + nslots_ * sizeof(uint64_t));
  int prio_least = 0, prio_greatest = 0;
  if (config().ingest_prio && hipDeviceGetStreamPriorityRange(&prio_least, &prio_greatest) != hipSuccess)
    prio_greatest = 0;
  if (hipMalloc(&next_, 64) != hipSuccess) {
    (void)hipGetLastError();
    return false;
  }
  bool made = false;
  if (!config().ingest_prio) {
    int cus = 0;
    if (hipDeviceGetAttribute(&cus, hipDeviceAttributeMultiprocessorCount, device_) == hipSuccess &&
        cus > 0 && cus <= 1024) {
      uint32_t mask[32] = {0};
      for (int i = 0; i < cus; ++i) mask[i / 32] |= 1u << (i % 32);
      made = hipExtStreamCreateWithCUMask((hipStream_t *)&stream_, (uint32_t)((cus + 31) / 32),
                                          mask) == hipSuccess;
      if (!made) (void)hipGetLastError();
    }
  }
  if (!made && hipStreamCreateWithPriority((hipStream_t *)&stream_, hipStreamNonBlocking,
                                           config().ingest_prio ? prio_greatest : 0) != hipSuccess) {
    (void)hipGetLastError();
    return false;
  }
  if (hipEventCreateWithFlags((hipEvent_t *)&end_ev_, hipEventDisableTiming) != hipSuccess) {
    (void)hipGetLastError();
    return false;
  }
  *stop_ = 1;
  if (launch_grid() != 0) return false;
  if (hipEventSynchronize((hipEvent_t)end_ev_) != hipSuccess) return false;
  launched_ = false;
  return true;
}

int Ingest::launch_grid() {
  (void)hipSetDevice(device_);
  if (hipMemsetAsync(next_, 0, sizeof(uint32_t), (hipStream_t)stream_) != hipSuccess) return -EIO;
  int rc = strom_ingest_kernel_launch(ring_, (void *)done_, (const void *)stop_, next_, nslots_,
                                      post_seq_.load(), grid_, stream_);
  if (rc) return rc;
  if (hipEventRecord((hipEvent_t)end_ev_, (hipStream_t)stream_) != hipSuccess) return -EIO;
  launched_ = true;
  return 0;
}

int Ingest::start_locked() {
  if (state_.load() & 1) return 0;
  if (launched_) {
    (void)hipSetDevice(device_);
    if (hipEventSynchronize((hipEvent_t)end_ev_) != hipSuccess) return -EIO;
    launched_ = false;
  }
  __atomic_store_n(stop_, 0, __ATOMIC_SEQ_CST);
  int rc = launch_grid();
  if (rc) return rc;
  state_.fetch_or(1);
  nr_launch_++;
  return 0;
}

bool Ingest::post(const void *src, uint64_t dst, uint32_t len, uint64_t *seq) {
  uint32_t n = 0;
  return post_many(src, dst, len, len, seq, &n);
}

bool Ingest::post_many(const void *src, uint64_t dst, uint32_t len, uint32_t piece,
                       uint64_t *first, uint32_t *n) {
  Run r{src, dst, len, false, 0, 0};
  post_runs(&r, 1, piece);
  *first = r.first;
  *n = r.n;
  return r.ok;
}

void Ingest::post_runs(Run *runs, size_t nruns, uint32_t piece) {
  piece = std::max<uint32_t>(16, piece & ~15u);
  uint64_t total = 0;
  for (size_t i = 0; i < nruns; ++i) {
    Run &r = runs[i];
    r.n = 0;
    r.ok = r.len != 0 && !(r.len & 15) && !(((uint64_t)r.src | r.dst) & 15);
    if (r.ok) total += (r.len + piece - 1) / piece;
  }
  auto fail_all = [&] {
    for (size_t i = 0; i < nruns; ++i) runs[i].ok = false;
  };
  if (total == 0) return;
  if (dead_.load(std::memory_order_relaxed)) return fail_all();
  const uint64_t old = state_.fetch_add(2 * total);
  if (!(old & 1)) {
    std::lock_guard<std::mutex> g(mu_);
    if (dead_.load() || start_locked() != 0) {
      dead_.store(true);
      state_.fetch_sub(2 * total);
      return fail_all();
    }
  }
  uint64_t s = post_seq_.fetch_add(total);
  for (size_t i = 0; i < nruns; ++i) {
    Run &r = runs[i];
    if (!r.ok) continue;
    r.first = s + 1;
    for (uint32_t off = 0; off < r.len; off += piece, ++s, ++r.n)
      if (!write_desc(s, (const char *)r.src + off, r.dst + off, std::min(piece, r.len - off))) {
        for (size_t j = i; j < nruns; ++j) runs[j].ok = false;
        return;
      }
  }
}

bool Ingest::write_desc(uint64_t s, const void *src, uint64_t dst, uint32_t len) {
  const uint32_t k = (uint32_t)(s % nslots_);
  if (s >= nslots_)
    while (__atomic_load_n(&done_[k], __ATOMIC_ACQUIRE) < s - nslots_ + 1) {
      if (gone_.load(std::memory_order_acquire)) return false;
      _mm_pause();
    }
  IngestDesc *d = (IngestDesc *)ring_ + k;
  d->src = (uint64_t)src;
  d->dst = dst;
  d->len_tag = len;
  __atomic_store_n(&d->seq, s + 1, __ATOMIC_RELEASE);
  return true;
}

bool Ingest::is_done(uint64_t seq) const {
  return __atomic_load_n(&done_[(seq - 1) % nslots_], __ATOMIC_ACQUIRE) >= seq;
}

void Ingest::info(uint64_t *out) {
  out[0] = dead_.load() ? 0 : 1;
  {
    std::lock_guard<std::mutex> g(mu_);
    out[1] = nr_launch_;
  }
  out[2] = post_seq_.load();
  out[3] = state_.load() >> 1;
}

void Ingest::retired(uint32_t n) { state_.fetch_sub(2ull * n); }

void Ingest::idle() {
  if (state_.load(std::memory_order_relaxed) != 1) return;
  std::lock_guard<std::mutex> g(mu_);
  uint64_t running_idle = 1;
  if (state_.compare_exchange_strong(running_idle, 0)) __atomic_store_n(stop_, 1, __ATOMIC_SEQ_CST);
}

void Ingest::shutdown() {
  {
    std::lock_guard<std::mutex> g(mu_);
    dead_.store(true);
  }
  const uint64_t drain_end = mono_ns() + 200000000ull;
  while ((state_.load() >> 1) != 0 && (state_.load() & 1) && mono_ns() < drain_end) _mm_pause();
  std::lock_guard<std::mutex> g(mu_);
  state_.fetch_and(~1ull);
  __atomic_store_n(stop_, 1, __ATOMIC_SEQ_CST);
  if (launched_) {
    const uint64_t end = mono_ns() + 2000000000ull;
    while (hipEventQuery((hipEvent_t)end_ev_) == hipErrorNotReady && mono_ns() < end)
      _mm_pause();
    launched_ = false;
  }
  gone_.store(true, std::memory_order_release);
}

}

extern "C" int strom_ingest_info(int device, uint64_t *out) {
  strom::Ingest *ing = strom::Ingest::get(device);
  if (!ing) return -ENODEV;
  ing->info(out);
  return 0;
}
```

csrc/engine/io.cc:

```cpp
#include <hip/hip_runtime_api.h>
#include <errno.h>
#include <fcntl.h>
#include <linux/io_uring.h>
#include <sched.h>
#include <stdio.h>
#include <string.h>
#include <sys/mman.h>
#include <sys/stat.h>
#include <sys/syscall.h>
#include <sys/uio.h>
#include <unistd.h>
#include <x86intrin.h>

#include <algorithm>
#include <functional>
#include <fstream>

#include "engine.h"

#ifndef MPOL_PREFERRED
#define MPOL_PREFERRED 1
#endif

namespace strom {

class Uring {
 public:
  ~Uring() { close_ring(); }
  int init(unsigned entries) {
    io_uring_params p;
    memset(&p, 0, sizeof p);
    fd_ = (int)syscall(__NR_io_uring_setup, entries, &p);
    if (fd_ < 0) return -errno;
    sq_sz_ = p.sq_off.array + p.sq_entries * sizeof(unsigned);
    cq_sz_ = p.cq_off.cqes + p.cq_entries * sizeof(io_uring_cqe);
    bool single = p.features & IORING_FEAT_SINGLE_MMAP;
    if (single) sq_sz_ = cq_sz_ = std::max(sq_sz_, cq_sz_);
    sq_ptr_ = mmap(nullptr, sq_sz_, PROT_READ | PROT_WRITE, MAP_SHARED | MAP_POPULATE, fd_,
                   IORING_OFF_SQ_RING);
    if (sq_ptr_ == MAP_FAILED) return fail();
    cq_ptr_ = single ? sq_ptr_
                     : mmap(nullptr, cq_sz_, PROT_READ | PROT_WRITE, MAP_SHARED | MAP_POPULATE,
                            fd_, IORING_OFF_CQ_RING);
    if (cq_ptr_ == MAP_FAILED) return fail();
    sqe_sz_ = p.sq_entries * sizeof(io_uring_sqe);
    sqes_ = (io_uring_sqe *)mmap(nullptr, sqe_sz_, PROT_READ | PROT_WRITE,
                                 MAP_SHARED | MAP_POPULATE, fd_, IORING_OFF_SQES);
    if (sqes_ == MAP_FAILED) return fail();
    char *sq = (char *)sq_ptr_, *cq = (char *)cq_ptr_;
    sq_head_ = (unsigned *)(sq + p.sq_off.head);
    sq_tail_ = (unsigned *)(sq + p.sq_off.tail);
    sq_mask_ = *(unsigned *)(sq + p.sq_off.ring_mask);
    sq_array_ = (unsigned *)(sq + p.sq_off.array);
    cq_head_ = (unsigned *)(cq + p.cq_off.head);
    cq_tail_ = (unsigned *)(cq + p.cq_off.tail);
    cq_mask_ = *(unsigned *)(cq + p.cq_off.ring_mask);
    cqes_ = (io_uring_cqe *)(cq + p.cq_off.cqes);
    entries_ = p.sq_entries;
    return 0;
  }
  io_uring_sqe *next_sqe() {
    unsigned tail = *sq_tail_;
    unsigned head = __atomic_load_n(sq_head_, __ATOMIC_ACQUIRE);
    if (tail - head >= entries_) return nullptr;
    unsigned idx = tail & sq_mask_;
    io_uring_sqe *s = &sqes_[idx];
    memset(s, 0, sizeof *s);
    sq_array_[idx] = idx;
    __atomic_store_n(sq_tail_, tail + 1, __ATOMIC_RELEASE);
    ++pending_;
    return s;
  }
  int enter(unsigned min_complete) {
    unsigned flags = min_complete ? IORING_ENTER_GETEVENTS : 0;
    int r = (int)syscall(__NR_io_uring_enter, fd_, pending_, min_complete, flags, nullptr, 0);
    if (r < 0) return -errno;
    pending_ -= (unsigned)r <= pending_ ? (unsigned)r : pending_;
    return r;
  }
  bool peek(io_uring_cqe *out) {
    unsigned head = *cq_head_;
    if (head == __atomic_load_n(cq_tail_, __ATOMIC_ACQUIRE)) return false;
    *out = cqes_[head & cq_mask_];
    __atomic_store_n(cq_head_, head + 1, __ATOMIC_RELEASE);
    return true;
  }
  unsigned pending() const { return pending_; }
  bool ok() const { return fd_ >= 0; }
  void unregister_buffers() {
    (void)syscall(__NR_io_uring_register, fd_, IORING_UNREGISTER_BUFFERS, nullptr, 0u);
  }
  int register_buffer(void *p, size_t len) {
    iovec iov{p, len};
    int r = (int)syscall(__NR_io_uring_register, fd_, IORING_REGISTER_BUFFERS, &iov, 1u);
    return r < 0 ? -errno : 0;
  }

 private:
  int fail() {
    int e = errno;
    close_ring();
    return -e;
  }
  void close_ring() {
    if (sqes_ && sqes_ != MAP_FAILED) munmap(sqes_, sqe_sz_);
    if (cq_ptr_ && cq_ptr_ != MAP_FAILED && cq_ptr_ != sq_ptr_) munmap(cq_ptr_, cq_sz_);
    if (sq_ptr_ && sq_ptr_ != MAP_FAILED) munmap(sq_ptr_, sq_sz_);
    if (fd_ >= 0) close(fd_);
    fd_ = -1;
    sqes_ = nullptr;
    sq_ptr_ = cq_ptr_ = nullptr;
  }
  int fd_ = -1;
  void *sq_ptr_ = nullptr, *cq_ptr_ = nullptr;
  size_t sq_sz_ = 0, cq_sz_ = 0, sqe_sz_ = 0;
  io_uring_sqe *sqes_ = nullptr;
  io_uring_cqe *cqes_ = nullptr;
  unsigned *sq_head_ = nullptr, *sq_tail_ = nullptr, *sq_array_ = nullptr;
  unsigned *cq_head_ = nullptr, *cq_tail_ = nullptr;
  unsigned sq_mask_ = 0, cq_mask_ = 0, entries_ = 0, pending_ = 0;
};

static std::atomic<uint64_t> g_fixed_workers{0}, g_fixed_refused{0}, g_fixed_errno{0};

void finish_request(IoReq &r, long status) {
  Stats &st = stats();
  st.nr_ssd2gpu.fetch_add(1, std::memory_order_relaxed);
  st.clk_ssd2gpu.fetch_add(tsc_now() - r.t_submit_tsc, std::memory_order_relaxed);
  st.inflight_dec();
  if (r.gmap) {
    if (r.gmap->inflight.fetch_sub(1) == 1 && r.gmap->draining.load()) {
      std::lock_guard<std::mutex> g(r.gmap->mu);
      r.gmap->cv.notify_all();
    }
  }
  if (r.task) tasks().put(r.task, status);
  else if (r.status_out) *r.status_out = status;
}

static long pread_full(int fd, uint8_t *buf, uint32_t len, uint64_t off) {
  uint32_t done = 0;
  while (done < len) {
    ssize_t n = pread(fd, buf + done, len - done, (off_t)(off + done));
    if (n < 0) {
      if (errno == EINTR) continue;
      return -errno;
    }
    if (n == 0) break;
    done += (uint32_t)n;
  }
  return done;
}

static long finalize_read(const IoReq &r, uint8_t *dst, uint32_t len, long got) {
  if (got == -EINVAL && r.fd_buffered >= 0 && r.fd_buffered != r.fd)
    got = pread_full(r.fd_buffered, dst, len, r.off);
  if (got < 0) return got;
  if ((uint32_t)got < r.valid) return -EIO;
  if ((uint32_t)got < r.len) memset(dst + got, 0, r.len - (uint32_t)got);
  return 0;
}

enum ProfPhase {
  PF_IDLE,
  PF_TAKE,
  PF_START,
  PF_SUBMIT,
  PF_REAP,
  PF_BAR,
  PF_POST,
  PF_HDP,
  PF_FINISH,
  PF_RETIRE,
  PF_WAIT,
};
static_assert(PF_WAIT + 1 == IoEngine::kProfPhases, "phase count");
enum ProfCount { PC_REQ, PC_BATCH, PC_ENTER, PC_SLEEP, PC_DESC };
static_assert(PC_DESC + 1 == IoEngine::kProfCounts, "count count");

static void bind_to_node(int node) {
  if (node < 0) return;
  std::ifstream f("/sys/devices/system/node/node" + std::to_string(node) + "/cpulist");
  std::string list;
  if (!(f >> list)) return;
  cpu_set_t want, allowed, use;
  CPU_ZERO(&want);
  size_t pos = 0;
  while (pos < list.size()) {
    size_t comma = list.find(',', pos);
    std::string part = list.substr(pos, comma == std::string::npos ? std::string::npos : comma - pos);
    int a = 0, b = 0;
    if (sscanf(part.c_str(), "%d-%d", &a, &b) == 2) {
      for (int c = a; c <= b && c < CPU_SETSIZE; ++c) CPU_SET(c, &want);
    } else if (sscanf(part.c_str(), "%d", &a) == 1 && a < CPU_SETSIZE) {
      CPU_SET(a, &want);
    }
    if (comma == std::string::npos) break;
    pos = comma + 1;
  }
  if (sched_getaffinity(0, sizeof allowed, &allowed) != 0) return;
  CPU_AND(&use, &want, &allowed);
  if (CPU_COUNT(&use) > 0) sched_setaffinity(0, sizeof use, &use);
  unsigned long mask[16] = {0};
  if (node < 1024) {
    mask[node / 64] = 1ul << (node % 64);
    syscall(SYS_set_mempolicy, MPOL_PREFERRED, mask, 1024ul);
  }
}

struct IoEngine::Worker {
  struct Slot {
    uint8_t *buf = nullptr;
    hipEvent_t ev = nullptr;
    int ev_dev = -1;
    IoReq req;
    uint64_t t_copy_ns = 0;
    int ev_slot = -1;
    Ingest *ing = nullptr;
    uint64_t seq_first = 0;
    uint32_t nseq = 0;
    uint32_t nret = 0;
    uint32_t held = 0;
  };
  struct Ctx {
    IoReq req;
    int slot = -1;
    uint8_t *dst = nullptr;
    uint32_t len = 0;
    uint64_t t0 = 0;
    long got = 0;
    uint64_t seq = 0;
  };

  std::vector<Ctx> fake_cq;
  uint64_t fake_rng = 0, fake_seq = 0, fake_next = 0;

  uint64_t fake_rand() {
    fake_rng ^= fake_rng << 13;
    fake_rng ^= fake_rng >> 7;
    fake_rng ^= fake_rng << 17;
    return fake_rng;
  }

  void reap_fake() {
    now_ns = mono_ns();
    while (!fake_cq.empty()) {
      const size_t i = (size_t)(fake_rand() % fake_cq.size());
      Ctx c = fake_cq[i];
      fake_cq[i] = fake_cq.back();
      fake_cq.pop_back();
      --reads_inflight;
      faults().fake_completions.fetch_add(1, std::memory_order_relaxed);
      if (c.seq != fake_next) faults().fake_reordered.fetch_add(1, std::memory_order_relaxed);
      fake_next = c.seq + 1;
      on_read_done(c, c.got);
    }
    post_ingest();
    flush_staged();
  }

  int idx = 0;
  Config cfg;
  std::thread th;
  std::mutex mu;
  std::condition_variable cv;
  std::vector<IoReq> q;
  bool stop = false;
  bool sleeping = false;
  std::atomic<int> pending{0};
  std::vector<Slot> slots;
  uint8_t *staging = nullptr;
  size_t staging_bytes = 0;
  bool staging_thp = false;
  bool fixed = false;
  std::deque<int> free_slots;
  size_t stage_inflight = 0;
  std::deque<int> copying;
  std::vector<int> staged;
  std::vector<int> ing_staged;
  std::vector<int> ingesting;
  std::vector<std::pair<int, Ingest *>> ings;
  std::vector<Ingest::Run> runs;
  std::vector<std::pair<size_t, size_t>> span;
  std::vector<hipStream_t> streams;
  int cur_dev = -2;
  Uring ring;
  std::vector<Ctx> ctx;
  std::vector<int> free_ctx;
  int reads_inflight = 0;
  int numa_node = -1;
  uint64_t now_ns = 0;

  struct Fin {
    Task *task;
    GpuMapping *gmap;
    long status;
    long *status_out;
  };
  std::vector<Fin> fin;
  uint64_t fin_clk = 0;
  std::vector<std::pair<GpuMapping *, const uint8_t *>> bar_dirty;
  uint32_t nbar = 0;
  uint64_t ndesc = 0;
  uint64_t copy_clk = 0;
  uint32_t lh_io[STROM_HIST_BUCKETS] = {}, lh_copy[STROM_HIST_BUCKETS] = {};
  uint64_t lh_io_mask = 0, lh_copy_mask = 0;

  bool prof_on = false;
  uint64_t prof_t = 0;
  std::atomic<uint64_t> prof_cyc[kProfPhases] = {};
  std::atomic<uint64_t> prof_cnt[kProfCounts] = {};
  uint64_t prof_base_cyc[kProfPhases] = {};
  uint64_t prof_base_cnt[kProfCounts] = {};
  static void bump(std::atomic<uint64_t> &c, uint64_t d) {
    c.store(c.load(std::memory_order_relaxed) + d, std::memory_order_relaxed);
  }
  void lap(int k) {
    if (__builtin_expect(prof_on, 0)) {
      const uint64_t t = tsc_now();
      bump(prof_cyc[k], t - prof_t);
      prof_t = t;
    }
  }

  void hist_io(uint64_t ns) {
    const int b = Hist::bucket(ns);
    ++lh_io[b];
    lh_io_mask |= 1ull << b;
  }
  void hist_copy(uint64_t ns, uint32_t n = 1) {
    const int b = Hist::bucket(ns);
    lh_copy[b] += n;
    lh_copy_mask |= 1ull << b;
  }

  void complete(const IoReq &r, long status) {
    fin.push_back(Fin{r.task, r.gmap, status, r.status_out});
    fin_clk += tsc_now() - r.t_submit_tsc;
  }

  void flush_done() {
    if (fin.empty()) return;
    for (auto &b : bar_dirty) b.first->bar_flush(b.second, true);
    bar_dirty.clear();
    if (nbar) {
      hist_copy(mono_ns() - now_ns, nbar);
      nbar = 0;
    }
    lap(PF_HDP);
    Stats &st = stats();
    const uint64_t n = fin.size();
    st.nr_ssd2gpu.fetch_add(n, std::memory_order_relaxed);
    st.clk_ssd2gpu.fetch_add(fin_clk, std::memory_order_relaxed);
    st.inflight_dec(n);
    fin_clk = 0;
    if (ndesc) {
      st.nr_debug[0].fetch_add(ndesc, std::memory_order_relaxed);
      st.clk_debug[0].fetch_add(copy_clk, std::memory_order_relaxed);
      ndesc = copy_clk = 0;
    }
    for (uint64_t m = lh_io_mask; m; m &= m - 1) {
      const int b = __builtin_ctzll(m);
      st.io_ns.b[b].fetch_add(lh_io[b], std::memory_order_relaxed);
      lh_io[b] = 0;
    }
    for (uint64_t m = lh_copy_mask; m; m &= m - 1) {
      const int b = __builtin_ctzll(m);
      st.copy_ns.b[b].fetch_add(lh_copy[b], std::memory_order_relaxed);
      lh_copy[b] = 0;
    }
    lh_io_mask = lh_copy_mask = 0;
    for (size_t i = 0; i < fin.size();) {
      GpuMapping *g = fin[i].gmap;
      size_t j = i + 1;
      while (j < fin.size() && fin[j].gmap == g) ++j;
      if (g) {
        const int k = (int)(j - i);
        if (g->inflight.fetch_sub(k) == k && g->draining.load()) {
          std::lock_guard<std::mutex> lk(g->mu);
          g->cv.notify_all();
        }
      }
      i = j;
    }
    for (size_t i = 0; i < fin.size();) {
      Task *t = fin[i].task;
      long status = fin[i].status;
      size_t j = i + 1;
      if (t) {
        while (j < fin.size() && fin[j].task == t) {
          if (!status) status = fin[j].status;
          ++j;
        }
        tasks().put_n(t, (int)(j - i), status);
      } else if (fin[i].status_out) {
        *fin[i].status_out = status;
      }
      i = j;
    }
    bump(prof_cnt[PC_REQ], n);
    bump(prof_cnt[PC_BATCH], 1);
    fin.clear();
    lap(PF_FINISH);
  }

  void bind_numa() {
    if (cfg.numa_bind) bind_to_node(numa_node);
  }

  int nslots() const {
    const size_t budget = (size_t)cfg.staging_slots << 20;
    const size_t small = std::min<size_t>((size_t)cfg.queue_depth * 4, budget / cfg.max_request);
    const size_t by_bytes = std::min<size_t>(cfg.staging_bytes / cfg.max_request, 256);
    return (int)std::min<size_t>(256, std::max<size_t>({(size_t)cfg.staging_slots, small, by_bytes,
                                                        cfg.stage_by_bytes ? (size_t)cfg.queue_depth : 0}));
  }
  size_t stage_budget() const {
    const size_t budget = std::max<size_t>((size_t)cfg.staging_slots << 20, cfg.staging_bytes);
    return std::min<size_t>(budget, (size_t)nslots() * cfg.max_request);
  }
  void release_slot(int si) {
    stage_inflight -= slots[si].held;
    slots[si].held = 0;
    free_slots.push_back(si);
  }

  bool ensure_slots() {
    if (!slots.empty()) return true;
    const int ns = nslots();
    size_t bytes = (size_t)ns * cfg.max_request;
    staging = (uint8_t *)hip::host_alloc_thp(bytes, cfg.ingest);
    staging_thp = staging != nullptr;
    if (!staging) staging = (uint8_t *)hip::host_alloc(bytes, cfg.ingest);
    if (!staging) {
      STROM_LOG(0, "worker %d: pinned staging allocation failed", idx);
      return false;
    }
    staging_bytes = bytes;
    slots.resize(ns);
    for (int i = 0; i < ns; ++i) {
      slots[i].buf = staging + (size_t)i * cfg.max_request;
      free_slots.push_back(i);
    }
    fixed = false;
    if (cfg.fixed_bufs && ring.ok()) {
      int rc = ring.register_buffer(staging, bytes);
      fixed = rc == 0;
      if (rc) {
        STROM_LOG(1, "worker %d: io_uring buffer registration refused (%d)", idx, rc);
        g_fixed_refused.fetch_add(1);
        g_fixed_errno.store((uint64_t)-rc);
      } else {
        g_fixed_workers.fetch_add(1);
      }
    }
    return true;
  }

  void free_staging() {
    if (!staging) return;
    if (fixed) {
      ring.unregister_buffers();
      g_fixed_workers.fetch_sub(1);
    }
    fixed = false;
    if (staging_thp) hip::host_free_thp(staging, staging_bytes);
    else hip::host_free(staging);
    staging = nullptr;
  }

  hipStream_t stream_for(int dev) {
    if (dev != cur_dev) {
      (void)hipSetDevice(dev);
      cur_dev = dev;
    }
    if ((int)streams.size() <= dev) streams.resize(dev + 1, nullptr);
    if (!streams[dev]) (void)hipStreamCreateWithFlags(&streams[dev], hipStreamNonBlocking);
    return streams[dev];
  }

  Ingest *ingest_for(int dev) {
    for (auto &p : ings)
      if (p.first == dev) return p.second;
    Ingest *ing = cfg.ingest ? Ingest::get(dev) : nullptr;
    ings.emplace_back(dev, ing);
    return ing;
  }

  bool retire_ingest() {
    bool any = false;
    uint64_t now = 0;
    for (size_t i = 0; i < ingesting.size();) {
      const int si = ingesting[i];
      Slot &s = slots[si];
      bool all = true;
      for (uint32_t k = 0; k < s.nseq && all; ++k) all = s.ing->is_done(s.seq_first + k);
      if (!all) {
        ++i;
        continue;
      }
      if (!now) now = mono_ns();
      const uint64_t dt = now - s.t_copy_ns;
      hist_copy(dt);
      copy_clk += dt;
      if (s.nret) s.ing->retired(s.nret);
      ingesting[i] = ingesting.back();
      ingesting.pop_back();
      release_slot(si);
      complete(s.req, 0);
      any = true;
    }
    return any;
  }

  void on_read_done(Ctx &c, long got) {
    IoReq &r = c.req;
    hist_io(now_ns - c.t0);
    long status = finalize_read(r, c.dst, c.len, got);
    if (c.slot < 0) {
      complete(r, status);
      return;
    }
    Slot &s = slots[c.slot];
    if (status != 0) {
      release_slot(c.slot);
      complete(r, status);
      return;
    }
    s.req = r;
    s.t_copy_ns = now_ns;
    if (r.gmap && r.len >= cfg.ingest_min && ingest_for(r.device)) {
      ing_staged.push_back(c.slot);
      return;
    }
    to_hbm(c.slot);
  }

  void to_hbm(int si) {
    Slot &s = slots[si];
    const IoReq &r = s.req;
    constexpr uint32_t kWorkerBarMax = 64u << 10;
    if (r.len <= std::min(cfg.bar_max, kWorkerBarMax) && r.gmap) {
      lap(PF_REAP);
      const bool ok = r.gmap->bar_write(r.gpu_dst, s.buf, r.len, false);
      lap(PF_BAR);
      if (ok) {
        const uint8_t *last = r.gmap->bar + (r.gpu_dst - r.gmap->bar_va) + ((r.len - 1) & ~3u);
        if (!bar_dirty.empty() && bar_dirty.back().first == r.gmap) bar_dirty.back().second = last;
        else bar_dirty.emplace_back(r.gmap, last);
        ++nbar;
        ++ndesc;
        release_slot(si);
        complete(r, 0);
        return;
      }
    }
    staged.push_back(si);
  }

  void post_ingest() {
    if (ing_staged.empty()) return;
    lap(PF_REAP);
    std::sort(ing_staged.begin(), ing_staged.end());
    size_t i = 0;
    while (i < ing_staged.size()) {
      const int dev = slots[ing_staged[i]].req.device;
      Ingest *ing = ingest_for(dev);
      runs.clear();
      span.clear();
      size_t k = i;
      while (k < ing_staged.size() && slots[ing_staged[k]].req.device == dev) {
        size_t j = k + 1;
        uint64_t bytes = slots[ing_staged[k]].req.len;
        while (cfg.coalesce && j < ing_staged.size()) {
          const Slot &p = slots[ing_staged[j - 1]], &q2 = slots[ing_staged[j]];
          if (ing_staged[j] != ing_staged[j - 1] + 1 || p.req.len != cfg.max_request ||
              q2.req.device != dev || q2.req.gpu_dst != p.req.gpu_dst + p.req.len ||
              bytes + q2.req.len > (64u << 20))
            break;
          bytes += q2.req.len;
          ++j;
        }
        const Slot &h = slots[ing_staged[k]];
        runs.push_back(Ingest::Run{h.buf, h.req.gpu_dst, (uint32_t)bytes, false, 0, 0});
        span.emplace_back(k, j);
        k = j;
      }
      ing->post_runs(runs.data(), runs.size(), cfg.ingest_piece);
      for (size_t r = 0; r < runs.size(); ++r) {
        const Ingest::Run &run = runs[r];
        for (size_t m = span[r].first; m < span[r].second; ++m) {
          const int si = ing_staged[m];
          if (!run.ok) {
            to_hbm(si);
            continue;
          }
          Slot &s = slots[si];
          s.ing = ing;
          s.seq_first = run.first;
          s.nseq = run.n;
          s.nret = m == span[r].first ? run.n : 0;
          ingesting.push_back(si);
        }
        if (run.ok) {
          ndesc += run.n;
          bump(prof_cnt[PC_DESC], run.n);
        }
      }
      i = k;
    }
    ing_staged.clear();
    lap(PF_POST);
  }

  void flush_staged() {
    if (staged.empty()) return;
    std::sort(staged.begin(), staged.end());
    size_t i = 0;
    while (i < staged.size()) {
      size_t j = i + 1;
      uint64_t bytes = slots[staged[i]].req.len;
      while (cfg.coalesce && j < staged.size()) {
        const Slot &p = slots[staged[j - 1]], &q = slots[staged[j]];
        if (staged[j] != staged[j - 1] + 1 || p.req.len != cfg.max_request ||
            q.req.device != p.req.device || q.req.gpu_dst != p.req.gpu_dst + p.req.len)
          break;
        bytes += q.req.len;
        ++j;
      }
      Slot &head = slots[staged[i]];
      const int last = staged[j - 1];
      Slot &tail = slots[last];
      const int dev = head.req.device;
      hipStream_t st = stream_for(dev);
      if (!tail.ev || tail.ev_dev != dev) {
        if (tail.ev) (void)hipEventDestroy(tail.ev);
        (void)hipEventCreateWithFlags(&tail.ev, hipEventDisableTiming);
        tail.ev_dev = dev;
      }
      hipError_t e = hipMemcpyAsync((void *)head.req.gpu_dst, head.buf, bytes,
                                    hipMemcpyHostToDevice, st);
      if (e == hipSuccess) e = hipEventRecord(tail.ev, st);
      for (size_t k = i; k < j; ++k) {
        const int si = staged[k];
        if (e != hipSuccess) {
          release_slot(si);
          complete(slots[si].req, -EIO);
          continue;
        }
        slots[si].ev_slot = last;
        copying.push_back(si);
      }
      if (e != hipSuccess) STROM_LOG(0, "hipMemcpyAsync failed: %s", hipGetErrorString(e));
      else ++ndesc;
      i = j;
    }
    staged.clear();
  }

  void retire(bool block) {
    while (!copying.empty()) {
      Slot &s = slots[copying.front()];
      hipEvent_t ev = slots[s.ev_slot].ev;
      hipError_t e = block ? hipEventSynchronize(ev) : hipEventQuery(ev);
      if (e == hipErrorNotReady) return;
      uint64_t dt = mono_ns() - s.t_copy_ns;
      hist_copy(dt);
      copy_clk += dt;
      int si = copying.front();
      copying.pop_front();
      release_slot(si);
      complete(s.req, e == hipSuccess ? 0 : -EIO);
      block = false;
    }
  }

  bool start(IoReq &r, bool use_ring) {
    int slot = -1;
    uint8_t *dst = r.host_dst;
    if (!dst) {
      if (!ensure_slots()) {
        complete(r, -ENOMEM);
        return true;
      }
      if (free_slots.empty()) return false;
      if (cfg.stage_by_bytes && stage_inflight && stage_inflight + r.len > stage_budget()) return false;
      if (cfg.coalesce && !cfg.slot_lifo) {
        slot = free_slots.front();
        free_slots.pop_front();
      } else {
        slot = free_slots.back();
        free_slots.pop_back();
      }
      dst = slots[slot].buf;
      slots[slot].held = r.len;
      stage_inflight += r.len;
    }
    uint32_t len = r.len;
    int frc = faults().on_request(&len);
    Ctx c;
    c.req = r;
    c.slot = slot;
    c.dst = dst;
    c.len = len;
    c.t0 = now_ns;
    if (frc && cfg.backend != BackendKind::kFake) {
      on_read_done(c, frc);
      post_ingest();
      flush_staged();
      return true;
    }
    if (cfg.backend == BackendKind::kFake) {
      c.got = frc ? frc : pread_full(r.fd, dst, len, r.off);
      c.seq = fake_seq++;
      fake_cq.push_back(c);
      ++reads_inflight;
      return true;
    }
    if (use_ring) {
      int ci;
      if (free_ctx.empty()) {
        ci = (int)ctx.size();
        ctx.push_back(c);
      } else {
        ci = free_ctx.back();
        free_ctx.pop_back();
        ctx[ci] = c;
      }
      io_uring_sqe *sqe = ring.next_sqe();
      if (!sqe) {
        ring.enter(0);
        sqe = ring.next_sqe();
      }
      if (fixed && slot >= 0) {
        sqe->opcode = IORING_OP_READ_FIXED;
        sqe->buf_index = 0;
      } else {
        sqe->opcode = IORING_OP_READ;
      }
      sqe->fd = read_fd(r);
      sqe->addr = (uint64_t)dst;
      sqe->len = len;
      sqe->off = r.off;
      sqe->user_data = (uint64_t)ci;
      ++reads_inflight;
      return true;
    }
    long got = pread_full(read_fd(r), dst, len, r.off);
    now_ns = mono_ns();
    on_read_done(c, got);
    post_ingest();
    flush_staged();
    return true;
  }
  int read_fd(const IoReq &r) const {
    return cfg.backend == BackendKind::kCache && r.fd_buffered >= 0 ? r.fd_buffered : r.fd;
  }

  void reap() {
    io_uring_cqe cqe;
    bool first = true;
    while (ring.peek(&cqe)) {
      if (first) {
        now_ns = mono_ns();
        first = false;
      }
      int ci = (int)cqe.user_data;
      Ctx c = ctx[ci];
      free_ctx.push_back(ci);
      --reads_inflight;
      long got = cqe.res;
      if (got >= 0 && (uint32_t)got < c.len) {
        long more = pread_full(read_fd(c.req), c.dst + got, c.len - (uint32_t)got, c.req.off + got);
        got = more < 0 ? more : got + more;
      }
      on_read_done(c, got);
    }
    post_ingest();
    flush_staged();
    lap(PF_REAP);
  }

  void run() {
    bind_numa();
    const bool fake = cfg.backend == BackendKind::kFake;
    bool use_ring = cfg.backend == BackendKind::kUring || cfg.backend == BackendKind::kCache;
    const int qd_cfg = (int)std::max<size_t>(
        {(size_t)cfg.queue_depth, (size_t)cfg.staging_slots,
         std::min<size_t>(cfg.staging_bytes / cfg.max_request, 256)});
    if (use_ring && ring.init((unsigned)std::max(8, qd_cfg * 2)) != 0) use_ring = false;
    int qd = use_ring || fake ? qd_cfg : 1;
    fake_rng = faults().fake_seed.load() * 2654435761u + (uint64_t)idx * 0x9E3779B97F4A7C15ull + 1;
    const uint64_t spin_ns = (uint64_t)cfg.spin_us * 1000;
    prof_on = cfg.io_prof;
    prof_t = tsc_now();
    std::vector<IoReq> local;
    size_t lpos = 0;
    for (;;) {
      flush_done();
      if (lpos == local.size()) {
        const bool quiet = reads_inflight == 0 && copying.empty() && ingesting.empty();
        if (spin_ns && quiet && !pending.load(std::memory_order_acquire)) {
          const uint64_t end = mono_ns() + spin_ns;
          while (!pending.load(std::memory_order_acquire) && mono_ns() < end)
            for (int i = 0; i < 32; ++i) _mm_pause();
        }
        if (quiet && !pending.load(std::memory_order_acquire)) {
          for (auto &p : ings)
            if (p.second) p.second->idle();
        }
        lap(PF_IDLE);
        std::unique_lock<std::mutex> g(mu);
        if (q.empty() && quiet) {
          if (stop) break;
          sleeping = true;
          bump(prof_cnt[PC_SLEEP], 1);
          cv.wait(g, [&] { return stop || !q.empty(); });
          sleeping = false;
          lap(PF_IDLE);
        }
        local.clear();
        lpos = 0;
        local.swap(q);
        pending.store(0, std::memory_order_relaxed);
        g.unlock();
        lap(PF_TAKE);
      }
      bool blocked = false;
      now_ns = mono_ns();
      while (lpos < local.size() && reads_inflight < qd) {
        if (!start(local[lpos], use_ring)) {
          blocked = true;
          break;
        }
        ++lpos;
      }
      lap(PF_START);
      if (use_ring && ring.pending()) {
        ring.enter(0);
        bump(prof_cnt[PC_ENTER], 1);
        lap(PF_SUBMIT);
      }
      const bool drained = lpos == local.size();
      if (fake && (drained || blocked || reads_inflight >= qd)) reap_fake();
      retire(false);
      retire_ingest();
      lap(PF_RETIRE);
      if (use_ring) reap();
      flush_done();
      if (lpos < local.size() && !blocked && reads_inflight < qd) continue;
      const bool hbm_busy = !copying.empty() || !ingesting.empty();
      if (reads_inflight > 0 && !hbm_busy) {
        if (fake) {
          reap_fake();
        } else {
          ring.enter(1);
          bump(prof_cnt[PC_ENTER], 1);
          lap(PF_WAIT);
          reap();
        }
      } else if (reads_inflight == 0 && hbm_busy) {
        if (lpos == local.size()) {
          std::lock_guard<std::mutex> g(mu);
          if (!q.empty()) continue;
        }
        if (!ingesting.empty()) {
          const uint64_t end = mono_ns() + 200000;
          while (!retire_ingest() && mono_ns() < end) {
            for (int i = 0; i < 16; ++i) _mm_pause();
            if (pending.load(std::memory_order_acquire)) break;
          }
          retire(false);
          lap(PF_WAIT);
        } else {
          retire(true);
          lap(PF_WAIT);
        }
      } else if (reads_inflight > 0) {
        if (!retire_ingest()) sched_yield();
        lap(PF_WAIT);
      }
    }
    for (auto &s : slots)
      if (s.ev) (void)hipEventDestroy(s.ev);
    free_staging();
    for (auto st : streams)
      if (st) (void)hipStreamDestroy(st);
  }
};

int IoEngine::prof(uint64_t *out, int nout, bool reset) {
  const int need = 2 + kProfPhases + kProfCounts + 4;
  if (nout < need) return -EINVAL;
  memset(out, 0, sizeof(uint64_t) * need);
  out[0] = workers_.size();
  out[1] = tsc_khz();
  std::lock_guard<std::mutex> lk(prof_mu_);
  for (auto &w : workers_) {
    for (int k = 0; k < kProfPhases; ++k) {
      const uint64_t v = w->prof_cyc[k].load(std::memory_order_relaxed);
      out[2 + k] += v - w->prof_base_cyc[k];
      if (reset) w->prof_base_cyc[k] = v;
    }
    for (int k = 0; k < kProfCounts; ++k) {
      const uint64_t v = w->prof_cnt[k].load(std::memory_order_relaxed);
      out[2 + kProfPhases + k] += v - w->prof_base_cnt[k];
      if (reset) w->prof_base_cnt[k] = v;
    }
  }
  CallerProf &cp = caller_prof();
  std::atomic<uint64_t> *c[4] = {&cp.calls, &cp.plan, &cp.build, &cp.submit};
  for (int k = 0; k < 4; ++k) out[2 + kProfPhases + kProfCounts + k] = reset ? c[k]->exchange(0) : c[k]->load();
  return need;
}

IoEngine::IoEngine(const Config &cfg) {
  int node = -1;
  if (cfg.numa_bind && hip::available()) {
    int dev = 0;
    (void)hipGetDevice(&dev);
    node = hip::numa_node_of_device(dev);
  }
  for (int i = 0; i < cfg.workers; ++i) {
    auto w = std::make_unique<Worker>();
    w->idx = i;
    w->cfg = cfg;
    w->numa_node = node;
    Worker *wp = w.get();
    w->th = std::thread([wp] { wp->run(); });
    workers_.push_back(std::move(w));
  }
}

IoEngine::~IoEngine() {
  for (auto &w : workers_) {
    std::lock_guard<std::mutex> g(w->mu);
    w->stop = true;
    w->cv.notify_all();
  }
  for (auto &w : workers_) w->th.join();
}

struct InlineCtx {
  uint8_t *buf = nullptr;
  size_t cap = 0;
  uint8_t *plain = nullptr;
  size_t plain_cap = 0;
  int dev = -1;
  hipStream_t st = nullptr;
  hipEvent_t ev = nullptr;
};
static thread_local InlineCtx tl_inline;

void IoEngine::run_inline(IoReq &r) {
  InlineCtx &c = tl_inline;
  uint32_t len = r.len;
  int frc = faults().on_request(&len);
  uint64_t t0 = mono_ns();
  if (r.host_dst) {
    long got = frc ? frc : pread_full(r.fd, r.host_dst, len, r.off);
    stats().io_ns.add(mono_ns() - t0);
    phase_mark(3);
    finish_request(r, finalize_read(r, r.host_dst, len, got));
    phase_mark(6);
    return;
  }
  const bool ing_ok = config().ingest;
  if (c.cap < r.len) {
    size_t cap = std::max<size_t>(r.len, 64u << 10);
    uint8_t *b = (uint8_t *)hip::host_alloc_thp(cap, ing_ok);
    if (!b) b = (uint8_t *)hip::host_alloc(cap, ing_ok);
    if (!b) {
      finish_request(r, -ENOMEM);
      return;
    }
    c.buf = b;
    c.cap = cap;
  }
  const int rfd = config().backend == BackendKind::kCache && r.fd_buffered >= 0 ? r.fd_buffered : r.fd;
  const bool to_bar = r.len <= config().bar_max && r.gmap && r.gmap->bar;
  uint8_t *rb = c.buf;
  if (to_bar && config().inline_plain) {
    if (c.plain_cap < r.len) {
      free(c.plain);
      c.plain_cap = 0;
      const size_t cap = std::max<size_t>(r.len, 64u << 10);
      c.plain = posix_memalign((void **)&c.plain, 4096, cap) == 0 ? c.plain : nullptr;
      if (c.plain) c.plain_cap = cap;
    }
    if (c.plain) rb = c.plain;
  }
  long got = frc ? frc : pread_full(rfd, rb, len, r.off);
  uint64_t t1 = mono_ns();
  if (tl_phase) tl_phase[3] = t1;
  stats().io_ns.add(t1 - t0);
  long status = finalize_read(r, rb, len, got);
  Ingest *ing = nullptr;
  uint64_t first = 0;
  uint32_t nseq = 0;
  const bool bar_ok = status == 0 && to_bar && r.gmap->bar_write(r.gpu_dst, rb, r.len);
  if (!bar_ok && status == 0 && rb != c.buf) memcpy(c.buf, rb, r.len);
  if (bar_ok) {
    stats().copy_ns.add(mono_ns() - t1);
    stats().nr_debug[0].fetch_add(1, std::memory_order_relaxed);
  } else if (status == 0 && ing_ok && r.gmap && (ing = Ingest::get(r.device)) &&
             ing->post_many(c.buf, r.gpu_dst, r.len, config().ingest_piece, &first, &nseq)) {
    for (uint32_t k = 0; k < nseq; ++k)
      while (!ing->is_done(first + k)) _mm_pause();
    ing->retired(nseq);
    ing->idle();
    phase_mark(4);
    stats().copy_ns.add(mono_ns() - t1);
    stats().nr_debug[0].fetch_add(nseq, std::memory_order_relaxed);
  } else if (status == 0) {
    if (c.dev != r.device) {
      (void)hipSetDevice(r.device);
      (void)hipStreamCreateWithFlags(&c.st, hipStreamNonBlocking);
      (void)hipEventCreateWithFlags(&c.ev, hipEventDisableTiming);
      c.dev = r.device;
    }
    hipError_t e = hipMemcpyAsync((void *)r.gpu_dst, c.buf, r.len, hipMemcpyHostToDevice, c.st);
    if (e == hipSuccess) e = hipStreamSynchronize(c.st);
    phase_mark(4);
    if (e != hipSuccess) status = -EIO;
    stats().copy_ns.add(mono_ns() - t1);
    stats().nr_debug[0].fetch_add(1, std::memory_order_relaxed);
  }
  finish_request(r, status);
  phase_mark(6);
}

void IoEngine::submit(std::vector<IoReq> &reqs) {
  const size_t n = workers_.size();
  if (reqs.empty()) return;
  uint32_t start = rr_.fetch_add((uint32_t)reqs.size());
  size_t per = (reqs.size() + n - 1) / n;
  for (size_t k = 0; k < n; ++k) {
    size_t lo = k * per, hi = std::min(reqs.size(), lo + per);
    if (lo >= hi) break;
    Worker &w = *workers_[(start + k) % n];
    bool wake;
    {
      std::lock_guard<std::mutex> g(w.mu);
      w.q.insert(w.q.end(), reqs.begin() + lo, reqs.begin() + hi);
      w.pending.store(1, std::memory_order_release);
      wake = w.sleeping;
    }
    if (wake) w.cv.notify_one();
  }
}

}

extern "C" int strom_io_prof(uint64_t *out, int nout, int reset) {
  return strom::engine().io().prof(out, nout, reset != 0);
}

extern "C" int strom_io_info(uint64_t *out) {
  out[0] = strom::g_fixed_workers.load();
  out[1] = strom::g_fixed_refused.load();
  out[2] = strom::g_fixed_errno.load();
  return 0;
}

namespace {
int raw_reads(int fd, int mode, uint32_t threads, uint32_t qd, uint64_t slot,
              const std::function<bool(uint32_t, uint32_t, uint64_t *, uint32_t *)> &next,
              uint64_t *bytes_out, double *sec_out) {
  using namespace strom;
  const bool fixed = (mode & 4) != 0;
  if (slot * qd > (4ull << 30)) return -E2BIG;
  int node = -1;
  if (config().numa_bind && hip::available()) {
    int dev = 0;
    (void)hipGetDevice(&dev);
    node = hip::numa_node_of_device(dev);
  }
  char path[64];
  snprintf(path, sizeof path, "/proc/self/fd/%d", fd);
  int d = open(path, O_RDONLY | ((mode & 2) ? 0 : O_DIRECT) | O_CLOEXEC);
  if (d < 0) return -errno;
  std::atomic<int> err{0};
  std::atomic<uint64_t> total{0};
  auto body = [&](uint32_t tid) {
    bind_to_node(node);
    Uring ring;
    int rc = ring.init(qd);
    void *buf = nullptr;
    const size_t bytes = (size_t)slot * qd, huge = (bytes + (2u << 20) - 1) & ~(size_t)((2u << 20) - 1);
    bool mapped = false, reg = false;
    if (rc == 0 && fixed) {
      void *m = mmap(nullptr, huge + (2u << 20), PROT_READ | PROT_WRITE, MAP_PRIVATE | MAP_ANONYMOUS, -1, 0);
      if (m != MAP_FAILED) {
        uint8_t *a = (uint8_t *)(((uintptr_t)m + (2u << 20) - 1) & ~(uintptr_t)((2u << 20) - 1));
        if (a > (uint8_t *)m) munmap(m, (size_t)(a - (uint8_t *)m));
        const size_t tail = (size_t)((uint8_t *)m + huge + (2u << 20) - (a + huge));
        if (tail) munmap(a + huge, tail);
        (void)madvise(a, huge, MADV_HUGEPAGE);
        memset(a, 0, huge);
        buf = a;
        mapped = true;
        reg = ring.register_buffer(buf, bytes) == 0;
      }
    }
    if (rc == 0 && !buf && posix_memalign(&buf, 4096, bytes) != 0) rc = -ENOMEM;
    uint32_t inflight = 0, k = 0;
    uint64_t got_bytes = 0;
    bool more = true;
    std::vector<uint32_t> freeslot;
    for (uint32_t s = 0; s < qd; ++s) freeslot.push_back(s);
    bool init_ok = rc == 0;
    while (init_ok) {
      while (rc == 0 && more && !freeslot.empty()) {
        uint64_t off = 0;
        uint32_t len = 0;
        if (!(more = next(tid, k, &off, &len))) break;
        ++k;
        uint32_t s = freeslot.back();
        freeslot.pop_back();
        io_uring_sqe *q = ring.next_sqe();
        q->opcode = reg ? IORING_OP_READ_FIXED : IORING_OP_READ;
        q->buf_index = 0;
        q->fd = d;
        q->addr = (uint64_t)buf + (uint64_t)s * slot;
        q->len = len;
        q->off = off;
        q->user_data = s;
        ++inflight;
      }
      if (inflight == 0) break;
      int r = ring.pending() ? ring.enter(0) : 0;
      if (r < 0 && r != -EINTR && rc == 0) rc = r;
      io_uring_cqe c;
      uint32_t got = 0;
      auto reap = [&] {
        while (ring.peek(&c)) {
          if (c.res < 0 && rc == 0) rc = c.res;
          if (c.res > 0) got_bytes += (uint64_t)c.res;
          freeslot.push_back((uint32_t)c.user_data);
          --inflight;
          ++got;
        }
      };
      for (uint64_t t0 = mono_ns(); !got && mono_ns() - t0 < 20000;) {
        reap();
        if (!got) _mm_pause();
      }
      if (!got) {
        r = ring.enter(1);
        if (r < 0 && r != -EINTR && rc == 0) rc = r;
        reap();
      }
    }
    if (rc) err.store(rc);
    total.fetch_add(got_bytes);
    if (reg) ring.unregister_buffers();
    if (mapped) munmap(buf, huge);
    else free(buf);
  };
  const uint64_t t0 = mono_ns();
  std::vector<std::thread> th;
  for (uint32_t t = 0; t < threads; ++t) th.emplace_back(body, t);
  for (auto &t : th) t.join();
  *sec_out = (mono_ns() - t0) * 1e-9;
  *bytes_out = total.load();
  close(d);
  return err.load();
}
}

extern "C" int strom_raw_read_rate(int fd, uint64_t block, uint32_t nreq, uint32_t threads,
                                   uint32_t qd, int mode, double *iops, double *gibps) {
  const bool sequential = mode & 1;
  if (block == 0 || (block & 4095) || block > (1ull << 30) || nreq == 0 || threads == 0 || qd == 0 ||
      qd > 256)
    return -EINVAL;
  struct stat st;
  if (fstat(fd, &st) != 0) return -errno;
  const uint64_t nblk = (uint64_t)st.st_size / block;
  if (nblk == 0) return -ERANGE;
  const uint64_t run = std::max<uint64_t>(1, nblk / threads);
  std::vector<uint64_t> x(threads);
  for (uint32_t t = 0; t < threads; ++t) x[t] = 0x9e3779b97f4a7c15ull * (t + 1);
  auto next = [&](uint32_t tid, uint32_t k, uint64_t *off, uint32_t *len) {
    const uint32_t mine = nreq / threads + (tid < nreq % threads ? 1 : 0);
    if (k >= mine) return false;
    uint64_t &r = x[tid];
    r ^= r << 13, r ^= r >> 7, r ^= r << 17;
    *off = (sequential ? ((uint64_t)tid * run + k % run) % nblk : r % nblk) * block;
    *len = (uint32_t)block;
    return true;
  };
  uint64_t bytes = 0;
  double sec = 0;
  const int rc = raw_reads(fd, mode, threads, qd, block, next, &bytes, &sec);
  if (rc) return rc;
  if (iops) *iops = nreq / sec;
  if (gibps) *gibps = (double)nreq * block / sec / (1 << 30);
  return 0;
}

extern "C" int strom_raw_read_list(int fd, const uint64_t *off, const uint32_t *len, uint32_t n,
                                   uint32_t threads, uint32_t qd, int mode, double *iops,
                                   double *gibps) {
  if (!off || !len || n == 0 || threads == 0 || qd == 0 || qd > 256) return -EINVAL;
  uint32_t slot = 0;
  for (uint32_t i = 0; i < n; ++i) {
    if ((off[i] & 4095) || len[i] == 0 || (len[i] & 4095) || len[i] > (64u << 20)) return -EINVAL;
    slot = std::max(slot, len[i]);
  }
  threads = std::min(threads, n);
  auto next = [&](uint32_t tid, uint32_t k, uint64_t *o, uint32_t *l) {
    const uint64_t lo = (uint64_t)n * tid / threads, hi = (uint64_t)n * (tid + 1) / threads;
    if (lo + k >= hi) return false;
    *o = off[lo + k];
    *l = len[lo + k];
    return true;
  };
  uint64_t bytes = 0;
  double sec = 0;
  const int rc = raw_reads(fd, mode & ~1, threads, qd, slot, next, &bytes, &sec);
  if (rc) return rc;
  if (iops) *iops = n / sec;
  if (gibps) *gibps = (double)bytes / sec / (1 << 30);
  return 0;
}
```

nvme_strom_amd/api.py:

```python
from __future__ import annotations

import ctypes as C
import errno as _errno
import os
from dataclasses import dataclass, field
from typing import List, Optional

import numpy as np

from . import _native as N


class StromError(OSError):
    def __init__(self, err: int, what: str, status: int = 0):
        super().__init__(err, f"{what}: {os.strerror(err)}" + (f" (status {status})" if status else ""))
        self.status = status


def _check(rc: int, what: str, status: int = 0) -> int:
    if rc < 0:
        raise StromError(-rc, what, status)
    return rc


class Session:

    def __init__(self):
        self.lib = N.lib()
        self.sid = _check(self.lib.strom_open(), "strom_open")
        self.closed = False

    def ioctl(self, cmd: int, arg, what: str = "ioctl") -> int:
        rc = self.lib.strom_ioctl(self.sid, cmd, C.byref(arg))
        return _check(rc, what)

    def ioctl_rc(self, cmd: int, arg) -> int:
        return self.lib.strom_ioctl(self.sid, cmd, C.byref(arg))

    def close(self) -> int:
        if self.closed:
            return 0
        self.closed = True
        return self.lib.strom_close(self.sid)

    def __enter__(self):
        return self

    def __exit__(self, *exc):
        self.close()


_default: Optional[Session] = None


def session() -> Session:
    global _default
    if _default is None or _default.closed:
        _default = Session()
    return _default


def version() -> str:
    return N.lib().strom_version().decode()


def provider() -> str:
    return "kernel" if N.lib().strom_provider() == 1 else "userspace"


def config_set(key: str, value) -> None:
    if isinstance(value, bool):
        value = int(value)
    _check(N.lib().strom_config_set(key.encode(), str(value).encode()), f"config {key}")


def config_get(key: str) -> str:
    buf = C.create_string_buffer(64)
    _check(N.lib().strom_config_get(key.encode(), buf, 64), f"config {key}")
    return buf.value.decode()


def configure(reset: bool = True, **kv) -> None:
    for k, v in kv.items():
        config_set(k, v)
    if reset:
        engine_reset()


def engine_reset() -> None:
    N.lib().strom_engine_reset()


def fault_inject(fail_at: int = 0, err: int = _errno.EIO, short_at: int = 0,
                 short_bytes: int = 0, delay_us: int = 0) -> None:
    N.lib().strom_fault_inject(fail_at, err, short_at, short_bytes, delay_us)


def fake_backend(seed: int = 0) -> tuple:
    c, r = C.c_uint64(), C.c_uint64()
    N.lib().strom_fake_backend(seed, C.byref(c), C.byref(r))
    return c.value, r.value


def ingest_info(device: int = 0) -> Optional[dict]:
    out = np.zeros(4, dtype=np.uint64)
    if N.lib().strom_ingest_info(device, out.ctypes.data) < 0:
        return None
    return dict(available=bool(out[0]), launches=int(out[1]), posted=int(out[2]),
                outstanding=int(out[3]))


def io_info() -> dict:
    out = np.zeros(3, dtype=np.uint64)
    _check(N.lib().strom_io_info(out.ctypes.data), "io_info")
    return dict(fixed_workers=int(out[0]), fixed_refused=int(out[1]), fixed_errno=int(out[2]))


IO_PROF_PHASES = ("idle", "take", "start", "submit", "reap", "bar", "post", "hdp", "finish",
                  "retire", "wait")
IO_PROF_COUNTS = ("requests", "batches", "enters", "sleeps", "descriptors")


def io_prof(reset: bool = False) -> dict:
    n = 2 + len(IO_PROF_PHASES) + len(IO_PROF_COUNTS) + 4
    out = np.zeros(n, dtype=np.uint64)
    _check(N.lib().strom_io_prof(out.ctypes.data, n, 1 if reset else 0), "io_prof")
    khz = max(int(out[1]), 1)
    ns = {k: int(out[2 + i]) * 1e6 / khz for i, k in enumerate(IO_PROF_PHASES)}
    cnt = {k: int(out[2 + len(IO_PROF_PHASES) + i]) for i, k in enumerate(IO_PROF_COUNTS)}
    req = max(cnt["requests"], 1)
    c0 = 2 + len(IO_PROF_PHASES) + len(IO_PROF_COUNTS)
    caller = dict(calls=int(out[c0]), **{k: round(int(out[c0 + 1 + i]) * 1e6 / khz / req, 1)
                                         for i, k in enumerate(("plan_ns_per_req", "build_ns_per_req",
                                                                "submit_ns_per_req"))})
    return dict(workers=int(out[0]), tsc_khz=khz, ns=ns, counts=cnt, caller=caller,
                ns_per_req={k: round(v / req, 1) for k, v in ns.items()},
                busy_ns_per_req=round(sum(v for k, v in ns.items() if k != "idle") / req, 1))


HOST_COSTS = ("clock_gettime", "rdtsc", "fstat", "mincore", "syscall", "mutex", "cv_notify",
              "kcmp_file", "statx_ino")


def host_costs(fd: int, n: int = 20000) -> dict:
    out = np.zeros(len(HOST_COSTS), dtype=np.uint64)
    _check(N.lib().strom_host_costs(fd, out.ctypes.data, n), "host_costs")
    return {k: int(v) for k, v in zip(HOST_COSTS, out)}


ENGINE_COSTS = ("registry_get", "validate", "open_file", "completion", "registry_get_cached",
                "open_file_cached", "bar_store_4k", "lock_after_bar_store", "bar_store_4k_nt",
                "lock_after_bar_store_nt", "bar_store_4k_nt_rev", "lock_after_bar_store_nt_rev",
                "bar_store_4k_movsb", "lock_after_bar_store_movsb", "bar_store_4k_two_cores",
                "two_core_handoff")


def engine_costs(handle: int, fd: int, n: int = 20000) -> dict:
    out = np.zeros(len(ENGINE_COSTS), dtype=np.uint64)
    _check(N.lib().strom_engine_costs(handle, fd, out.ctypes.data, n), "engine_costs")
    return {k: int(v) for k, v in zip(ENGINE_COSTS, out)}


def resident_bytes(fd: int, offset: int = 0, length: int = 1 << 62) -> int:
    return _check(N.lib().strom_resident_bytes(fd, offset, length), "resident_bytes")


def evict_file(fd: int) -> None:
    _check(N.lib().strom_evict_file(fd), "evict_file")


def crc32c_host(data, crc: int = 0) -> int:
    buf = memoryview(data).cast("B")
    arr = (C.c_char * len(buf)).from_buffer_copy(buf) if buf.readonly else (C.c_char * len(buf)).from_buffer(buf)
    return N.lib().strom_crc32c_host(crc, arr, len(buf))


@dataclass
class FileInfo:
    numa_node_id: int
    support_dma64: bool


def check_file(fd: int, sess: Optional[Session] = None) -> FileInfo:
    a = N.CheckFile(fdesc=fd)
    (sess or session()).ioctl(N.CHECK_FILE, a, "CHECK_FILE")
    return FileInfo(a.numa_node_id, bool(a.support_dma64))


@dataclass
class GpuMapping:
    handle: int
    gpu_page_sz: int
    gpu_npages: int
    vaddress: int
    length: int
    sess: Session = field(repr=False, default=None)

    def unmap(self) -> None:
        if self.handle:
            unmap_gpu_memory(self.handle, self.sess)
            self.handle = 0

    def __enter__(self):
        return self

    def __exit__(self, *exc):
        self.unmap()


def map_gpu_memory(vaddress: int, length: int, sess: Optional[Session] = None) -> GpuMapping:
    s = sess or session()
    a = N.MapGpuMemory(vaddress=vaddress, length=length)
    s.ioctl(N.MAP_GPU_MEMORY, a, "MAP_GPU_MEMORY")
    return GpuMapping(a.handle, a.gpu_page_sz, a.gpu_npages, vaddress, length, s)


def unmap_gpu_memory(handle: int, sess: Optional[Session] = None) -> None:
    a = N.UnmapGpuMemory(handle=handle)
    (sess or session()).ioctl(N.UNMAP_GPU_MEMORY, a, "UNMAP_GPU_MEMORY")


def list_gpu_memory(sess: Optional[Session] = None) -> List[int]:
    s = sess or session()
    nrooms = 64
    while True:
        a = N.list_gpu_memory_struct(nrooms)(nrooms=nrooms)
        s.ioctl(N.LIST_GPU_MEMORY, a, "LIST_GPU_MEMORY")
        if a.nitems <= nrooms:
            return [int(a.handles[i]) for i in range(a.nitems)]
        nrooms = a.nitems


def info_gpu_memory(handle: int, sess: Optional[Session] = None) -> dict:
    s = sess or session()
    nrooms = 16
    while True:
        a = N.info_gpu_memory_struct(nrooms)(handle=handle, nrooms=nrooms)
        s.ioctl(N.INFO_GPU_MEMORY, a, "INFO_GPU_MEMORY")
        if a.nitems <= nrooms:
            break
        nrooms = a.nitems
    return dict(handle=handle, nitems=a.nitems, version=a.version, gpu_page_sz=a.gpu_page_sz,
                owner=a.owner, map_offset=a.map_offset, map_length=a.map_length,
                paddrs=[int(a.paddrs[i]) for i in range(a.nitems)])


class DmaBuffer:

    def __init__(self, length: int, node: int = -1, sess: Optional[Session] = None):
        a = N.AllocDMABuffer(length=length, node_id=node)
        (sess or session()).ioctl(N.ALLOC_DMA_BUFFER, a, "ALLOC_DMA_BUFFER")
        self.fd = a.dmabuf_fdesc
        self.length = os.fstat(self.fd).st_size
        self.node = node
        self._lib = N.lib()
        addr = self._lib.strom_dmabuf_mmap(self.fd, self.length)
        if not addr:
            err = C.get_errno() or _errno.EINVAL
            os.close(self.fd)
            self.fd = -1
            raise StromError(err, "strom_dmabuf_mmap")
        self.address = int(addr)
        self.array = np.ctypeslib.as_array((C.c_uint8 * self.length).from_address(self.address))

    def close(self) -> None:
        if self.fd >= 0:
            self.array = None
            self._lib.strom_dmabuf_munmap(self.address, self.length)
            os.close(self.fd)
            self.fd = -1

    def __enter__(self):
        return self

    def __exit__(self, *exc):
        self.close()


def dmabuf_gc() -> int:
    return N.lib().strom_dmabuf_gc()


def gpu_detached() -> int:
    return N.lib().strom_gpu_detached()


def alloc_dma_buffer(length: int, node: int = -1, sess: Optional[Session] = None) -> DmaBuffer:
    return DmaBuffer(length, node, sess)


class StripeSet:

    def __init__(self, members, unit: int = 1 << 20, size: Optional[int] = None):
        self.unit = int(unit)
        self._own = []
        fds = []
        for m in members:
            if isinstance(m, int):
                fds.append(m)
            else:
                fd = os.open(m, os.O_RDONLY)
                self._own.append(fd)
                fds.append(fd)
        self.members = list(members)
        self.size = int(size) if size is not None else sum(os.fstat(fd).st_size for fd in fds)
        arr = (C.c_int * len(fds))(*fds)
        rc = N.lib().strom_stripe_open(arr, len(fds), self.unit, self.size)
        if rc < 0:
            for fd in self._own:
                os.close(fd)
            raise StromError(-rc, "strom_stripe_open")
        self.fd = rc

    def close(self) -> None:
        if self.fd >= 0:
            N.lib().strom_stripe_close(self.fd)
            self.fd = -1
            for fd in self._own:
                os.close(fd)
            self._own = []

    def __enter__(self):
        return self

    def __exit__(self, *exc):
        self.close()


class RegisteredFile:

    def __init__(self, f):
        own = None
        if not isinstance(f, int):
            own = fd = os.open(f, os.O_RDONLY)
        else:
            fd = f
        try:
            rc = N.lib().strom_register_file(fd)
        finally:
            if own is not None:
                os.close(own)
        if rc < 0:
            raise StromError(-rc, "strom_register_file")
        self.fd = rc

    def close(self) -> None:
        if self.fd >= 0:
            N.lib().strom_unregister_file(self.fd)
            self.fd = -1

    def __enter__(self):
        return self

    def __exit__(self, *exc):
        self.close()


def write_striped(paths, data, unit: int = 1 << 20) -> int:
    mv = memoryview(np.frombuffer(data, dtype=np.uint8) if not isinstance(data, np.ndarray)
                    else data.view(np.uint8).reshape(-1))
    n = len(paths)
    files = [open(p, "wb") for p in paths]
    try:
        for s, off in enumerate(range(0, len(mv), unit)):
            files[s % n].write(mv[off:off + unit])
        for f in files:
            f.flush()
            os.fsync(f.fileno())
    finally:
        for f in files:
            f.close()
    return len(mv)


@dataclass
class CopyResult:
    dma_task_id: int
    nr_ram: int
    nr_ssd: int
    nr_dma_submit: int
    nr_dma_blocks: int

    @property
    def avg_request_bytes(self) -> float:
        return 512.0 * self.nr_dma_blocks / self.nr_dma_submit if self.nr_dma_submit else 0.0


def _ids_array(chunk_ids) -> np.ndarray:
    ids = np.ascontiguousarray(chunk_ids, dtype=np.uint32)
    return ids


def memcpy_ssd2gpu(handle: int, offset: int, fd: int, chunk_ids: np.ndarray, chunk_sz: int,
                   relseg_sz: int = 0, wb_buffer: int = 0,
                   sess: Optional[Session] = None) -> CopyResult:
    if not (isinstance(chunk_ids, np.ndarray) and chunk_ids.dtype == np.uint32
            and chunk_ids.flags.c_contiguous):
        raise TypeError("chunk_ids must be a contiguous numpy uint32 array (rewritten in place)")
    a = N.MemCopySsdToGpu(handle=handle, offset=offset, file_desc=fd, nr_chunks=len(chunk_ids),
                          chunk_sz=chunk_sz, relseg_sz=relseg_sz,
                          chunk_ids=chunk_ids.ctypes.data_as(C.POINTER(C.c_uint32)),
                          wb_buffer=wb_buffer or None)
    (sess or session()).ioctl(N.MEMCPY_SSD2GPU, a, "MEMCPY_SSD2GPU")
    return CopyResult(a.dma_task_id, a.nr_ram2gpu, a.nr_ssd2gpu, a.nr_dma_submit, a.nr_dma_blocks)


EXTENT_DTYPE = np.dtype([("file_off", "<u8"), ("dst_off", "<u8"), ("len", "<u4"),
                         ("reserved", "<u4")])


@dataclass
class ExtentResult:
    dma_task_id: int
    nr_dma_submit: int
    nr_dma_blocks: int
    bytes_read: int
    gap_bytes: int
    dst_bytes: int
    dst_off: np.ndarray

    @property
    def avg_request_bytes(self) -> float:
        return 512.0 * self.nr_dma_blocks / self.nr_dma_submit if self.nr_dma_submit else 0.0


def extents_array(file_off, length) -> np.ndarray:
    off = np.asarray(file_off, dtype=np.uint64).reshape(-1)
    ln = np.asarray(length, dtype=np.uint64).reshape(-1)
    if off.shape != ln.shape:
        raise ValueError("file_off and length differ in length")
    if len(ln) and int(ln.max()) > 0xFFFFFFFF:
        raise ValueError("an extent longer than 4 GiB")
    x = np.zeros(len(off), dtype=EXTENT_DTYPE)
    x["file_off"], x["len"] = off, ln.astype(np.uint32)
    return x


def memcpy_ssd2gpu_extents(handle: int, offset: int, fd: int, extents: np.ndarray,
                           gap_max: int = 64 << 10, plan_only: bool = False,
                           sess: Optional[Session] = None) -> ExtentResult:
    if not (isinstance(extents, np.ndarray) and extents.dtype == EXTENT_DTYPE
            and extents.flags.c_contiguous):
        raise TypeError("extents must be a contiguous EXTENT_DTYPE array (dst_off written in place)")
    a = N.MemCopySsdToGpuExtents(handle=handle, offset=offset, file_desc=fd,
                                 nr_extents=len(extents), gap_max=int(gap_max),
                                 flags=N.EXTENTS_PLAN_ONLY if plan_only else 0,
                                 extents=extents.ctypes.data if len(extents) else None)
    (sess or session()).ioctl(N.MEMCPY_SSD2GPU_EXTENTS, a, "MEMCPY_SSD2GPU_EXTENTS")
    return ExtentResult(a.dma_task_id, a.nr_dma_submit, a.nr_dma_blocks, a.bytes_read,
                        a.gap_bytes, a.dst_bytes, extents["dst_off"])


def memcpy_ssd2ram(dest_addr: int, fd: int, chunk_ids, chunk_sz: int, relseg_sz: int = 0,
                   sess: Optional[Session] = None) -> CopyResult:
    ids = _ids_array(chunk_ids)
    a = N.MemCopySsdToRam(dest_uaddr=dest_addr, file_desc=fd, nr_chunks=len(ids),
                          chunk_sz=chunk_sz, relseg_sz=relseg_sz,
                          chunk_ids=ids.ctypes.data_as(C.POINTER(C.c_uint32)))
    (sess or session()).ioctl(N.MEMCPY_SSD2RAM, a, "MEMCPY_SSD2RAM")
    return CopyResult(a.dma_task_id, a.nr_ram2ram, a.nr_ssd2ram, a.nr_dma_submit, a.nr_dma_blocks)


def pread_gpu(handle: int, offset: int, fd: int, file_off: int, length: int,
              sess: Optional[Session] = None) -> int:
    s = sess or session()
    return _check(s.lib.strom_pread_gpu(s.sid, handle, offset, fd, file_off, length),
                  "pread_gpu")


def pread_gpu_latency(handle: int, offset: int, fd: int, file_offs, length: int = 4096,
                      sess: Optional[Session] = None) -> np.ndarray:
    s = sess or session()
    offs = np.ascontiguousarray(file_offs, dtype=np.uint64)
    out = np.zeros(len(offs), dtype=np.uint64)
    _check(s.lib.strom_pread_gpu_lat(s.sid, handle, offset, fd, offs.ctypes.data, len(offs),
                                     length, out.ctypes.data), "pread_gpu_lat")
    return out


def ioctl_latency(handle: int, offset: int, fd: int, file_offs, length: int = 4096,
                  sess: Optional[Session] = None) -> np.ndarray:
    s = sess or session()
    offs = np.ascontiguousarray(file_offs, dtype=np.uint64)
    out = np.zeros(len(offs), dtype=np.uint64)
    _check(s.lib.strom_ioctl_lat(s.sid, handle, offset, fd, offs.ctypes.data, len(offs),
                                 length, out.ctypes.data), "ioctl_lat")
    return out


PHASES = ("lookup", "plan", "setup", "storage", "hbm_store", "hdp_flush", "complete", "wait")


def pread_gpu_phases(handle: int, offset: int, fd: int, file_offs, length: int = 4096,
                     sess: Optional[Session] = None) -> np.ndarray:
    s = sess or session()
    offs = np.ascontiguousarray(file_offs, dtype=np.uint64)
    out = np.zeros((len(offs), len(PHASES)), dtype=np.uint64)
    _check(s.lib.strom_pread_gpu_phases(s.sid, handle, offset, fd, offs.ctypes.data, len(offs),
                                        length, out.ctypes.data), "pread_gpu_phases")
    return out


def phase_breakdown(stamps: np.ndarray) -> dict:
    st = stamps.astype(np.float64)
    prev = np.zeros(len(st))
    out = {}
    for k, name in enumerate(PHASES):
        col = st[:, k]
        hit = col > 0
        out[name] = round(float(np.median((col - prev)[hit])) / 1e3, 2) if hit.any() else None
        prev = np.where(hit, col, prev)
    return out


def pread_raw_latency(fd: int, file_offs, length: int = 4096) -> np.ndarray:
    offs = np.ascontiguousarray(file_offs, dtype=np.uint64)
    out = np.zeros(len(offs), dtype=np.uint64)
    _check(N.lib().strom_pread_raw_lat(fd, offs.ctypes.data, len(offs), length, out.ctypes.data),
           "pread_raw_lat")
    return out


def pread_pair_latency(handle: int, offset: int, fd: int, file_offs, length: int = 4096,
                       sess: Optional[Session] = None) -> tuple:
    s = sess or session()
    offs = np.ascontiguousarray(file_offs, dtype=np.uint64)
    n = len(offs) // 2
    eng = np.zeros(n, dtype=np.uint64)
    raw = np.zeros(n, dtype=np.uint64)
    _check(s.lib.strom_pread_pair_lat(s.sid, handle, offset, fd, offs.ctypes.data, n, length,
                                      eng.ctypes.data, raw.ctypes.data), "pread_pair_lat")
    return eng, raw


def raw_read_rate(fd: int, block: int, nreq: int, threads: int = 4, qd: int = 8,
                  sequential: bool = False, buffered: bool = False,
                  fixed: bool = False) -> tuple:
    iops, gibps = C.c_double(), C.c_double()
    _check(N.lib().strom_raw_read_rate(fd, block, nreq, threads, qd,
                                       int(sequential) | (2 if buffered else 0) |
                                       (4 if fixed else 0),
                                       C.byref(iops), C.byref(gibps)), "raw_read_rate")
    return iops.value, gibps.value


def raw_read_list(fd: int, offs, lens, threads: int = 4, qd: int = 8, buffered: bool = False,
                  fixed: bool = False) -> tuple:
    o = np.ascontiguousarray(offs, dtype=np.uint64)
    n = np.ascontiguousarray(lens, dtype=np.uint32)
    if o.shape != n.shape or o.ndim != 1:
        raise ValueError("offs and lens must be 1-D and of one length")
    iops, gibps = C.c_double(), C.c_double()
    _check(N.lib().strom_raw_read_list(fd, o.ctypes.data, n.ctypes.data, len(o), threads, qd,
                                       (2 if buffered else 0) | (4 if fixed else 0),
                                       C.byref(iops), C.byref(gibps)), "raw_read_list")
    return iops.value, gibps.value


def memcpy_wait(task_id: int, timeout: Optional[float] = None,
                sess: Optional[Session] = None) -> None:
    s = sess or session()
    if timeout is None:
        a = N.MemCopyWait(dma_task_id=task_id)
        rc = s.ioctl_rc(N.MEMCPY_WAIT, a)
    else:
        a = N.MemCopyWaitTimed(dma_task_id=task_id, timeout_ns=int(timeout * 1e9))
        rc = s.ioctl_rc(N.MEMCPY_WAIT_TIMED, a)
    _check(rc, f"MEMCPY_WAIT({task_id})", a.status)


def stat_info(sess: Optional[Session] = None) -> dict:
    a = N.StatInfo(version=1)
    (sess or session()).ioctl(N.STAT_INFO, a, "STAT_INFO")
    return {name: getattr(a, name) for name, _ in N.StatInfo._fields_}


def stat_hist(reset: bool = False, sess: Optional[Session] = None) -> dict:
    a = N.StatHist(version=1, reset=int(reset))
    (sess or session()).ioctl(N.STAT_HIST, a, "STAT_HIST")
    return {k: np.array(getattr(a, k)[:], dtype=np.uint64) for k in ("io_ns", "copy_ns", "task_ns")}


def hist_percentile(hist: np.ndarray, q: float) -> float:
    total = int(hist.sum())
    if total == 0:
        return float("nan")
    target = q / 100.0 * total
    run = 0
    for k, c in enumerate(hist):
        if run + int(c) >= target and c:
            lo = 0.0 if k == 0 else float(1 << (k - 1))
            hi = float(1 << k)
            frac = (target - run) / float(c)
            return lo + (hi - lo) * frac
        run += int(c)
    return float(1 << (len(hist) - 1))
```

Baseline: 21.07.

## Add opt-in blocking io_uring wait for ingest tails and keep ingest kernel alive

Adds an opt-in ingest_wait=block mode. In this mode, once a short poll window expires, worker threads wait in io_uring_enter with an ext-arg timeout instead of spinning or yielding. It also tracks expected ingest requests from submit time so the ingest kernel is not idled while staged work is still on its way. Profiling gains wait/poll phase splits, worker CPU time and byte counts. The goal is to cut CPU burn and avoid relaunching the ingest kernel, at the cost of possible wakeup latency in block mode.

```diff
diff --git a/csrc/engine/core.cc b/csrc/engine/core.cc
--- a/csrc/engine/core.cc
+++ b/csrc/engine/core.cc
@@ -27,7 +27,7 @@
                                "bar_map", "bar_max", "bar_nt", "inline_plain", "coalesce", "trace",
                                "ingest", "ingest_grid", "ingest_piece", "ingest_min", "ingest_prio", "hdp_sync",
                                "fixed_bufs", "io_prof", "fd_kcmp", "stage_by_bytes", "slot_lifo",
-                               "strict", "direct_io",
+                               "ingest_wait", "ingest_wait_us", "strict", "direct_io",
                                "pgcache_probe", "gpu_emulation", "numa_bind", "check_freed",
                                "stat_info", "verbose"};
   for (const char *k : keys) {
@@ -51,6 +51,11 @@
     return 0;
   }
   if (k == "strict") { strict = parse_bool(v); return 0; }
+  if (k == "ingest_wait") {
+    if (v != "block" && v != "poll") return -EINVAL;
+    ingest_block = v == "block";
+    return 0;
+  }
   if (k == "direct_io") { direct_io = parse_bool(v); return 0; }
   if (k == "pgcache_probe") { pgcache_probe = parse_bool(v); return 0; }
   if (k == "gpu_emulation") { gpu_emulation = parse_bool(v); return 0; }
@@ -85,6 +90,7 @@
   if (k == "fd_kcmp") { fd_kcmp = parse_bool(v); return 0; }
   if (k == "stage_by_bytes") { stage_by_bytes = parse_bool(v); return 0; }
   if (k == "slot_lifo") { slot_lifo = parse_bool(v); return 0; }
+  if (k == "ingest_wait_us") { if (n < 1 || n > 10000) return -EINVAL; ingest_wait_us = (uint32_t)n; return 0; }
   if (k == "ingest_min") {
     if (n < 0 || n > (64l << 20)) return -EINVAL;
     ingest_min = (uint32_t)n;
@@ -127,6 +133,10 @@
            : backend == BackendKind::kUring ? "uring"
            : backend == BackendKind::kCache ? "cache"
                                             : "fake";
+    return 0;
+  }
+  if (k == "ingest_wait") {
+    *out = ingest_block ? "block" : "poll";
     return 0;
   }
   long v;
@@ -149,6 +159,7 @@
   else if (k == "fd_kcmp") v = fd_kcmp;
   else if (k == "stage_by_bytes") v = stage_by_bytes;
   else if (k == "slot_lifo") v = slot_lifo;
+  else if (k == "ingest_wait_us") v = ingest_wait_us;
   else if (k == "ingest_min") v = ingest_min;
   else if (k == "trace") v = trace;
   else if (k == "bar_max") v = bar_max;
diff --git a/csrc/engine/engine.cc b/csrc/engine/engine.cc
--- a/csrc/engine/engine.cc
+++ b/csrc/engine/engine.cc
@@ -747,7 +747,29 @@
   return 0;
 }
 
+namespace {
+struct WaitProf {
+  const bool on = config().io_prof;
+  uint64_t cpu0 = 0, wall0 = 0;
+  static uint64_t thread_cpu_ns() {
+    timespec ts;
+    clock_gettime(CLOCK_THREAD_CPUTIME_ID, &ts);
+    return (uint64_t)ts.tv_sec * 1000000000ull + (uint64_t)ts.tv_nsec;
+  }
+  WaitProf() {
+    if (on) cpu0 = thread_cpu_ns(), wall0 = mono_ns();
+  }
+  ~WaitProf() {
+    if (!on) return;
+    CallerProf &cp = caller_prof();
+    cp.wait_cpu_ns.fetch_add(thread_cpu_ns() - cpu0, std::memory_order_relaxed);
+    cp.wait_wall_ns.fetch_add(mono_ns() - wall0, std::memory_order_relaxed);
+  }
+};
+}
+
 int Engine::memcpy_wait(strom_memcpy_wait *a) {
+  WaitProf wp;
   long st = 0;
   int rc = tasks().wait(a->dma_task_id, &st, -1);
   a->status = st;
@@ -755,6 +777,7 @@
 }
 
 int Engine::memcpy_wait_timed(strom_memcpy_wait_timed *a) {
+  WaitProf wp;
   long st = 0;
   int rc = tasks().wait(a->dma_task_id, &st, (int64_t)a->timeout_ns);
   a->status = st;
diff --git a/csrc/engine/engine.h b/csrc/engine/engine.h
--- a/csrc/engine/engine.h
+++ b/csrc/engine/engine.h
@@ -46,6 +46,8 @@
   bool inline_plain = false;
   uint32_t ingest_min = 0;
   bool io_prof = false;
+  bool ingest_block = false;
+  uint32_t ingest_wait_us = 20;
   bool fd_kcmp = false;
   bool strict = false;
   bool direct_io = true;
@@ -98,6 +100,7 @@
 
 struct CallerProf {
   std::atomic<uint64_t> calls{0}, plan{0}, build{0}, submit{0};
+  std::atomic<uint64_t> wait_cpu_ns{0}, wait_wall_ns{0};
 };
 CallerProf &caller_prof();
 
@@ -298,6 +301,7 @@
 int plan_xfer(const PlanParams &p, strom_file_extent *x, uint32_t n, uint32_t gap_max,
               bool planner, ChunkPlan *out, uint64_t *dst_bytes, uint64_t *read_bytes);
 
+class Ingest;
 struct IoReq {
   Task *task = nullptr;
   int fd = -1;
@@ -312,6 +316,7 @@
   uint64_t t_submit_tsc = 0;
   GpuMapping *gmap = nullptr;
   long *status_out = nullptr;
+  Ingest *expect = nullptr;
 };
 
 class IoEngine {
@@ -319,7 +324,8 @@
   explicit IoEngine(const Config &cfg);
   ~IoEngine();
   void submit(std::vector<IoReq> &reqs);
-  static constexpr int kProfPhases = 11, kProfCounts = 5;
+  static constexpr int kProfPhases = 12, kProfCounts = 5;
+  static constexpr int kProfOutV1 = 22, kProfOut = 28;
   int prof(uint64_t *out, int nout, bool reset);
   void run_inline(IoReq &r);
   int workers() const { return (int)workers_.size(); }
@@ -327,6 +333,7 @@
   struct Worker;
  private:
   std::vector<std::unique_ptr<Worker>> workers_;
+  Config cfg_;
   std::mutex prof_mu_;
   std::atomic<uint32_t> rr_{0};
 };
@@ -349,6 +356,7 @@
 class Ingest {
  public:
   static Ingest *get(int device);
+  static Ingest *find(int device);
   bool post(const void *src, uint64_t dst, uint32_t len, uint64_t *seq);
   bool post_many(const void *src, uint64_t dst, uint32_t len, uint32_t piece, uint64_t *first,
                  uint32_t *n);
@@ -363,6 +371,8 @@
   void post_runs(Run *runs, size_t nruns, uint32_t piece);
   bool is_done(uint64_t seq) const;
   void retired(uint32_t n);
+  void expect(uint32_t n) { expected_.fetch_add(n, std::memory_order_relaxed); }
+  void expect_done(uint32_t n) { expected_.fetch_sub(n, std::memory_order_release); }
   void idle();
   void shutdown();
   void info(uint64_t *out);
@@ -382,6 +392,7 @@
   std::mutex mu_;
   std::atomic<uint64_t> post_seq_{0};
   std::atomic<uint64_t> state_{0};
+  std::atomic<uint64_t> expected_{0};
   bool launched_ = false;
   std::atomic<bool> dead_{false};
   std::atomic<bool> gone_{false};
diff --git a/csrc/engine/ingest.cc b/csrc/engine/ingest.cc
--- a/csrc/engine/ingest.cc
+++ b/csrc/engine/ingest.cc
@@ -52,6 +52,12 @@
   return ing;
 }
 
+Ingest *Ingest::find(int device) {
+  std::lock_guard<std::mutex> g(g_ing_mu);
+  auto it = g_ing.find(device);
+  return it == g_ing.end() ? nullptr : it->second;
+}
+
 Ingest::Ingest(int device) : device_(device) {}
 
 bool Ingest::init() {
@@ -213,6 +219,7 @@
 
 void Ingest::idle() {
   if (state_.load(std::memory_order_relaxed) != 1) return;
+  if (expected_.load(std::memory_order_acquire) != 0) return;
   std::lock_guard<std::mutex> g(mu_);
   uint64_t running_idle = 1;
   if (state_.compare_exchange_strong(running_idle, 0)) __atomic_store_n(stop_, 1, __ATOMIC_SEQ_CST);
diff --git a/csrc/engine/io.cc b/csrc/engine/io.cc
--- a/csrc/engine/io.cc
+++ b/csrc/engine/io.cc
@@ -2,6 +2,7 @@
 #include <errno.h>
 #include <fcntl.h>
 #include <linux/io_uring.h>
+#include <pthread.h>
 #include <sched.h>
 #include <stdio.h>
 #include <string.h>
@@ -9,6 +10,7 @@
 #include <sys/stat.h>
 #include <sys/syscall.h>
 #include <sys/uio.h>
+#include <time.h>
 #include <unistd.h>
 #include <x86intrin.h>
 
@@ -17,109 +19,13 @@
 #include <fstream>
 
 #include "engine.h"
+#include "uring.h"
 
 #ifndef MPOL_PREFERRED
 #define MPOL_PREFERRED 1
 #endif
 
 namespace strom {
-
-class Uring {
- public:
-  ~Uring() { close_ring(); }
-  int init(unsigned entries) {
-    io_uring_params p;
-    memset(&p, 0, sizeof p);
-    fd_ = (int)syscall(__NR_io_uring_setup, entries, &p);
-    if (fd_ < 0) return -errno;
-    sq_sz_ = p.sq_off.array + p.sq_entries * sizeof(unsigned);
-    cq_sz_ = p.cq_off.cqes + p.cq_entries * sizeof(io_uring_cqe);
-    bool single = p.features & IORING_FEAT_SINGLE_MMAP;
-    if (single) sq_sz_ = cq_sz_ = std::max(sq_sz_, cq_sz_);
-    sq_ptr_ = mmap(nullptr, sq_sz_, PROT_READ | PROT_WRITE, MAP_SHARED | MAP_POPULATE, fd_,
-                   IORING_OFF_SQ_RING);
-    if (sq_ptr_ == MAP_FAILED) return fail();
-    cq_ptr_ = single ? sq_ptr_
-                     : mmap(nullptr, cq_sz_, PROT_READ | PROT_WRITE, MAP_SHARED | MAP_POPULATE,
-                            fd_, IORING_OFF_CQ_RING);
-    if (cq_ptr_ == MAP_FAILED) return fail();
-    sqe_sz_ = p.sq_entries * sizeof(io_uring_sqe);
-    sqes_ = (io_uring_sqe *)mmap(nullptr, sqe_sz_, PROT_READ | PROT_WRITE,
-                                 MAP_SHARED | MAP_POPULATE, fd_, IORING_OFF_SQES);
-    if (sqes_ == MAP_FAILED) return fail();
-    char *sq = (char *)sq_ptr_, *cq = (char *)cq_ptr_;
-    sq_head_ = (unsigned *)(sq + p.sq_off.head);
-    sq_tail_ = (unsigned *)(sq + p.sq_off.tail);
-    sq_mask_ = *(unsigned *)(sq + p.sq_off.ring_mask);
-    sq_array_ = (unsigned *)(sq + p.sq_off.array);
-    cq_head_ = (unsigned *)(cq + p.cq_off.head);
-    cq_tail_ = (unsigned *)(cq + p.cq_off.tail);
-    cq_mask_ = *(unsigned *)(cq + p.cq_off.ring_mask);
-    cqes_ = (io_uring_cqe *)(cq + p.cq_off.cqes);
-    entries_ = p.sq_entries;
-    return 0;
-  }
-  io_uring_sqe *next_sqe() {
-    unsigned tail = *sq_tail_;
-    unsigned head = __atomic_load_n(sq_head_, __ATOMIC_ACQUIRE);
-    if (tail - head >= entries_) return nullptr;
-    unsigned idx = tail & sq_mask_;
-    io_uring_sqe *s = &sqes_[idx];
-    memset(s, 0, sizeof *s);
-    sq_array_[idx] = idx;
-    __atomic_store_n(sq_tail_, tail + 1, __ATOMIC_RELEASE);
-    ++pending_;
-    return s;
-  }
-  int enter(unsigned min_complete) {
-    unsigned flags = min_complete ? IORING_ENTER_GETEVENTS : 0;
-    int r = (int)syscall(__NR_io_uring_enter, fd_, pending_, min_complete, flags, nullptr, 0);
-    if (r < 0) return -errno;
-    pending_ -= (unsigned)r <= pending_ ? (unsigned)r : pending_;
-    return r;
-  }
-  bool peek(io_uring_cqe *out) {
-    unsigned head = *cq_head_;
-    if (head == __atomic_load_n(cq_tail_, __ATOMIC_ACQUIRE)) return false;
-    *out = cqes_[head & cq_mask_];
-    __atomic_store_n(cq_head_, head + 1, __ATOMIC_RELEASE);
-    return true;
-  }
-  unsigned pending() const { return pending_; }
-  bool ok() const { return fd_ >= 0; }
-  void unregister_buffers() {
-    (void)syscall(__NR_io_uring_register, fd_, IORING_UNREGISTER_BUFFERS, nullptr, 0u);
-  }
-  int register_buffer(void *p, size_t len) {
-    iovec iov{p, len};
-    int r = (int)syscall(__NR_io_uring_register, fd_, IORING_REGISTER_BUFFERS, &iov, 1u);
-    return r < 0 ? -errno : 0;
-  }
-
- private:
-  int fail() {
-    int e = errno;
-    close_ring();
-    return -e;
-  }
-  void close_ring() {
-    if (sqes_ && sqes_ != MAP_FAILED) munmap(sqes_, sqe_sz_);
-    if (cq_ptr_ && cq_ptr_ != MAP_FAILED && cq_ptr_ != sq_ptr_) munmap(cq_ptr_, cq_sz_);
-    if (sq_ptr_ && sq_ptr_ != MAP_FAILED) munmap(sq_ptr_, sq_sz_);
-    if (fd_ >= 0) close(fd_);
-    fd_ = -1;
-    sqes_ = nullptr;
-    sq_ptr_ = cq_ptr_ = nullptr;
-  }
-  int fd_ = -1;
-  void *sq_ptr_ = nullptr, *cq_ptr_ = nullptr;
-  size_t sq_sz_ = 0, cq_sz_ = 0, sqe_sz_ = 0;
-  io_uring_sqe *sqes_ = nullptr;
-  io_uring_cqe *cqes_ = nullptr;
-  unsigned *sq_head_ = nullptr, *sq_tail_ = nullptr, *sq_array_ = nullptr;
-  unsigned *cq_head_ = nullptr, *cq_tail_ = nullptr;
-  unsigned sq_mask_ = 0, cq_mask_ = 0, entries_ = 0, pending_ = 0;
-};
 
 static std::atomic<uint64_t> g_fixed_workers{0}, g_fixed_refused{0}, g_fixed_errno{0};
 
@@ -173,8 +79,11 @@
   PF_FINISH,
   PF_RETIRE,
   PF_WAIT,
+  PF_POLL,
 };
-static_assert(PF_WAIT + 1 == IoEngine::kProfPhases, "phase count");
+static_assert(PF_POLL + 1 == IoEngine::kProfPhases, "phase count");
+constexpr uint64_t kTailPollNs = 256000;
+
 enum ProfCount { PC_REQ, PC_BATCH, PC_ENTER, PC_SLEEP, PC_DESC };
 static_assert(PC_DESC + 1 == IoEngine::kProfCounts, "count count");
 
@@ -221,6 +130,7 @@
     uint32_t nseq = 0;
     uint32_t nret = 0;
     uint32_t held = 0;
+    Ingest *expect = nullptr;
   };
   struct Ctx {
     IoReq req;
@@ -312,6 +222,9 @@
   std::atomic<uint64_t> prof_cnt[kProfCounts] = {};
   uint64_t prof_base_cyc[kProfPhases] = {};
   uint64_t prof_base_cnt[kProfCounts] = {};
+  uint64_t fin_bytes = 0;
+  std::atomic<uint64_t> prof_bytes{0};
+  uint64_t prof_base_bytes = 0, prof_base_cpu_ns = 0;
   static void bump(std::atomic<uint64_t> &c, uint64_t d) {
     c.store(c.load(std::memory_order_relaxed) + d, std::memory_order_relaxed);
   }
@@ -337,6 +250,7 @@
   void complete(const IoReq &r, long status) {
     fin.push_back(Fin{r.task, r.gmap, status, r.status_out});
     fin_clk += tsc_now() - r.t_submit_tsc;
+    if (status == 0) fin_bytes += r.len;
   }
 
   void flush_done() {
@@ -400,6 +314,8 @@
     }
     bump(prof_cnt[PC_REQ], n);
     bump(prof_cnt[PC_BATCH], 1);
+    bump(prof_bytes, fin_bytes);
+    fin_bytes = 0;
     fin.clear();
     lap(PF_FINISH);
   }
@@ -418,6 +334,11 @@
   size_t stage_budget() const {
     const size_t budget = std::max<size_t>((size_t)cfg.staging_slots << 20, cfg.staging_bytes);
     return std::min<size_t>(budget, (size_t)nslots() * cfg.max_request);
+  }
+  void unexpect(int si) {
+    Slot &s = slots[si];
+    if (s.expect) s.expect->expect_done(1);
+    s.expect = nullptr;
   }
   void release_slot(int si) {
     stage_inflight -= slots[si].held;
@@ -523,6 +444,7 @@
     }
     Slot &s = slots[c.slot];
     if (status != 0) {
+      unexpect(c.slot);
       release_slot(c.slot);
       complete(r, status);
       return;
@@ -533,6 +455,7 @@
       ing_staged.push_back(c.slot);
       return;
     }
+    unexpect(c.slot);
     to_hbm(c.slot);
   }
 
@@ -591,6 +514,7 @@
         const Ingest::Run &run = runs[r];
         for (size_t m = span[r].first; m < span[r].second; ++m) {
           const int si = ing_staged[m];
+          unexpect(si);
           if (!run.ok) {
             to_hbm(si);
             continue;
@@ -680,6 +604,7 @@
     uint8_t *dst = r.host_dst;
     if (!dst) {
       if (!ensure_slots()) {
+        if (r.expect) r.expect->expect_done(1);
         complete(r, -ENOMEM);
         return true;
       }
@@ -695,6 +620,9 @@
       dst = slots[slot].buf;
       slots[slot].held = r.len;
       stage_inflight += r.len;
+      Ingest *ing = r.expect;
+      if (!ing && r.gmap && r.len >= cfg.ingest_min && (ing = ingest_for(r.device))) ing->expect(1);
+      slots[slot].expect = ing;
     }
     uint32_t len = r.len;
     int frc = faults().on_request(&len);
@@ -792,6 +720,9 @@
     int qd = use_ring || fake ? qd_cfg : 1;
     fake_rng = faults().fake_seed.load() * 2654435761u + (uint64_t)idx * 0x9E3779B97F4A7C15ull + 1;
     const uint64_t spin_ns = (uint64_t)cfg.spin_us * 1000;
+    const bool block_wait = cfg.ingest_block && use_ring && ring.can_wait_timed();
+    const uint64_t wait_ns = (uint64_t)std::max<uint32_t>(1, cfg.ingest_wait_us) * 1000;
+    bool tail_slow = false;
     prof_on = cfg.io_prof;
     prof_t = tsc_now();
     std::vector<IoReq> local;
@@ -827,15 +758,17 @@
         lap(PF_TAKE);
       }
       bool blocked = false;
-      now_ns = mono_ns();
-      while (lpos < local.size() && reads_inflight < qd) {
-        if (!start(local[lpos], use_ring)) {
-          blocked = true;
-          break;
-        }
-        ++lpos;
-      }
-      lap(PF_START);
+      if (lpos < local.size() && reads_inflight < qd) {
+        now_ns = mono_ns();
+        while (lpos < local.size() && reads_inflight < qd) {
+          if (!start(local[lpos], use_ring)) {
+            blocked = true;
+            break;
+          }
+          ++lpos;
+        }
+        lap(PF_START);
+      }
       if (use_ring && ring.pending()) {
         ring.enter(0);
         bump(prof_cnt[PC_ENTER], 1);
@@ -865,20 +798,39 @@
           if (!q.empty()) continue;
         }
         if (!ingesting.empty()) {
-          const uint64_t end = mono_ns() + 200000;
-          while (!retire_ingest() && mono_ns() < end) {
-            for (int i = 0; i < 16; ++i) _mm_pause();
-            if (pending.load(std::memory_order_acquire)) break;
+          bool got = false;
+          if (!(block_wait && tail_slow)) {
+            const uint64_t end = mono_ns() + (block_wait ? kTailPollNs : 200000);
+            while (!(got = retire_ingest()) && mono_ns() < end) {
+              for (int i = 0; i < 16; ++i) _mm_pause();
+              if (pending.load(std::memory_order_acquire)) break;
+            }
+            retire(false);
+            lap(PF_POLL);
+            tail_slow = block_wait && !got && !pending.load(std::memory_order_acquire);
+          } else {
+            ring.enter_timed(1, wait_ns);
+            bump(prof_cnt[PC_ENTER], 1);
+            lap(PF_WAIT);
+            if (retire_ingest()) tail_slow = false;
+            retire(false);
+            lap(PF_RETIRE);
           }
-          retire(false);
+        } else {
+          retire(true);
+          lap(PF_POLL);
+        }
+      } else if (reads_inflight > 0) {
+        if (retire_ingest()) {
+          lap(PF_RETIRE);
+        } else if (block_wait) {
+          ring.enter_timed(1, wait_ns);
+          bump(prof_cnt[PC_ENTER], 1);
           lap(PF_WAIT);
         } else {
-          retire(true);
-          lap(PF_WAIT);
-        }
-      } else if (reads_inflight > 0) {
-        if (!retire_ingest()) sched_yield();
-        lap(PF_WAIT);
+          sched_yield();
+          lap(PF_POLL);
+        }
       }
     }
     for (auto &s : slots)
@@ -890,31 +842,54 @@
 };
 
 int IoEngine::prof(uint64_t *out, int nout, bool reset) {
-  const int need = 2 + kProfPhases + kProfCounts + 4;
-  if (nout < need) return -EINVAL;
+  static_assert(kProfOutV1 == 2 + (kProfPhases - 1) + kProfCounts + 4, "io_prof v1 layout");
+  if (nout < kProfOutV1) return -EINVAL;
+  const int need = nout >= kProfOut ? kProfOut : kProfOutV1;
   memset(out, 0, sizeof(uint64_t) * need);
   out[0] = workers_.size();
   out[1] = tsc_khz();
+  uint64_t cyc[kProfPhases] = {}, bytes = 0, cpu_ns = 0;
+  const int cnt0 = 2 + kProfPhases - 1;
   std::lock_guard<std::mutex> lk(prof_mu_);
   for (auto &w : workers_) {
     for (int k = 0; k < kProfPhases; ++k) {
       const uint64_t v = w->prof_cyc[k].load(std::memory_order_relaxed);
-      out[2 + k] += v - w->prof_base_cyc[k];
+      cyc[k] += v - w->prof_base_cyc[k];
       if (reset) w->prof_base_cyc[k] = v;
     }
     for (int k = 0; k < kProfCounts; ++k) {
       const uint64_t v = w->prof_cnt[k].load(std::memory_order_relaxed);
-      out[2 + kProfPhases + k] += v - w->prof_base_cnt[k];
+      out[cnt0 + k] += v - w->prof_base_cnt[k];
       if (reset) w->prof_base_cnt[k] = v;
     }
-  }
+    const uint64_t b = w->prof_bytes.load(std::memory_order_relaxed);
+    bytes += b - w->prof_base_bytes;
+    if (reset) w->prof_base_bytes = b;
+    clockid_t cid;
+    timespec ts;
+    if (pthread_getcpuclockid(w->th.native_handle(), &cid) == 0 && clock_gettime(cid, &ts) == 0) {
+      const uint64_t c = (uint64_t)ts.tv_sec * 1000000000ull + (uint64_t)ts.tv_nsec;
+      cpu_ns += c - w->prof_base_cpu_ns;
+      if (reset) w->prof_base_cpu_ns = c;
+    }
+  }
+  for (int k = 0; k < PF_WAIT; ++k) out[2 + k] = cyc[k];
+  out[2 + PF_WAIT] = cyc[PF_WAIT] + cyc[PF_POLL];
   CallerProf &cp = caller_prof();
   std::atomic<uint64_t> *c[4] = {&cp.calls, &cp.plan, &cp.build, &cp.submit};
-  for (int k = 0; k < 4; ++k) out[2 + kProfPhases + kProfCounts + k] = reset ? c[k]->exchange(0) : c[k]->load();
+  for (int k = 0; k < 4; ++k) out[cnt0 + kProfCounts + k] = reset ? c[k]->exchange(0) : c[k]->load();
+  if (need == kProfOut) {
+    out[22] = cyc[PF_WAIT];
+    out[23] = cyc[PF_POLL];
+    out[24] = cpu_ns;
+    out[25] = bytes;
+    out[26] = reset ? cp.wait_cpu_ns.exchange(0) : cp.wait_cpu_ns.load();
+    out[27] = reset ? cp.wait_wall_ns.exchange(0) : cp.wait_wall_ns.load();
+  }
   return need;
 }
 
-IoEngine::IoEngine(const Config &cfg) {
+IoEngine::IoEngine(const Config &cfg) : cfg_(cfg) {
   int node = -1;
   if (cfg.numa_bind && hip::available()) {
     int dev = 0;
@@ -1033,6 +1008,24 @@
 void IoEngine::submit(std::vector<IoReq> &reqs) {
   const size_t n = workers_.size();
   if (reqs.empty()) return;
+  if (cfg_.ingest) {
+    int dev = -2;
+    Ingest *ing = nullptr;
+    uint32_t n = 0;
+    for (IoReq &r : reqs) {
+      if (r.host_dst || !r.gmap || r.len < cfg_.ingest_min) continue;
+      if (r.device != dev) {
+        if (n) ing->expect(n);
+        n = 0;
+        dev = r.device;
+        ing = Ingest::find(dev);
+      }
+      if (!ing) continue;
+      r.expect = ing;
+      ++n;
+    }
+    if (n) ing->expect(n);
+  }
   uint32_t start = rr_.fetch_add((uint32_t)reqs.size());
   size_t per = (reqs.size() + n - 1) / n;
   for (size_t k = 0; k < n; ++k) {
diff --git a/csrc/engine/uring.h b/csrc/engine/uring.h
--- /dev/null
+++ b/csrc/engine/uring.h
@@ -0,0 +1,134 @@
+#pragma once
+
+#include <errno.h>
+#include <linux/io_uring.h>
+#include <linux/time_types.h>
+#include <signal.h>
+#include <stdint.h>
+#include <string.h>
+#include <sys/mman.h>
+#include <sys/syscall.h>
+#include <sys/uio.h>
+#include <unistd.h>
+
+#include <algorithm>
+
+namespace strom {
+
+class Uring {
+ public:
+  ~Uring() { close_ring(); }
+  int init(unsigned entries) {
+    io_uring_params p;
+    memset(&p, 0, sizeof p);
+    fd_ = (int)syscall(__NR_io_uring_setup, entries, &p);
+    if (fd_ < 0) return -errno;
+    sq_sz_ = p.sq_off.array + p.sq_entries * sizeof(unsigned);
+    cq_sz_ = p.cq_off.cqes + p.cq_entries * sizeof(io_uring_cqe);
+    bool single = p.features & IORING_FEAT_SINGLE_MMAP;
+    if (single) sq_sz_ = cq_sz_ = std::max(sq_sz_, cq_sz_);
+    sq_ptr_ = mmap(nullptr, sq_sz_, PROT_READ | PROT_WRITE, MAP_SHARED | MAP_POPULATE, fd_,
+                   IORING_OFF_SQ_RING);
+    if (sq_ptr_ == MAP_FAILED) return fail();
+    cq_ptr_ = single ? sq_ptr_
+                     : mmap(nullptr, cq_sz_, PROT_READ | PROT_WRITE, MAP_SHARED | MAP_POPULATE,
+                            fd_, IORING_OFF_CQ_RING);
+    if (cq_ptr_ == MAP_FAILED) return fail();
+    sqe_sz_ = p.sq_entries * sizeof(io_uring_sqe);
+    sqes_ = (io_uring_sqe *)mmap(nullptr, sqe_sz_, PROT_READ | PROT_WRITE,
+                                 MAP_SHARED | MAP_POPULATE, fd_, IORING_OFF_SQES);
+    if (sqes_ == MAP_FAILED) return fail();
+    char *sq = (char *)sq_ptr_, *cq = (char *)cq_ptr_;
+    sq_head_ = (unsigned *)(sq + p.sq_off.head);
+    sq_tail_ = (unsigned *)(sq + p.sq_off.tail);
+    sq_mask_ = *(unsigned *)(sq + p.sq_off.ring_mask);
+    sq_array_ = (unsigned *)(sq + p.sq_off.array);
+    cq_head_ = (unsigned *)(cq + p.cq_off.head);
+    cq_tail_ = (unsigned *)(cq + p.cq_off.tail);
+    cq_mask_ = *(unsigned *)(cq + p.cq_off.ring_mask);
+    cqes_ = (io_uring_cqe *)(cq + p.cq_off.cqes);
+    entries_ = p.sq_entries;
+    ext_arg_ = (p.features & IORING_FEAT_EXT_ARG) != 0;
+    return 0;
+  }
+  io_uring_sqe *next_sqe() {
+    unsigned tail = *sq_tail_;
+    unsigned head = __atomic_load_n(sq_head_, __ATOMIC_ACQUIRE);
+    if (tail - head >= entries_) return nullptr;
+    unsigned idx = tail & sq_mask_;
+    io_uring_sqe *s = &sqes_[idx];
+    memset(s, 0, sizeof *s);
+    sq_array_[idx] = idx;
+    __atomic_store_n(sq_tail_, tail + 1, __ATOMIC_RELEASE);
+    ++pending_;
+    return s;
+  }
+  int enter(unsigned min_complete) {
+    unsigned flags = min_complete ? IORING_ENTER_GETEVENTS : 0;
+    int r = (int)syscall(__NR_io_uring_enter, fd_, pending_, min_complete, flags, nullptr, 0);
+    if (r < 0) return -errno;
+    pending_ -= (unsigned)r <= pending_ ? (unsigned)r : pending_;
+    return r;
+  }
+  bool can_wait_timed() const { return ext_arg_; }
+  void clear_ext_arg() { ext_arg_ = false; }
+  int enter_timed(unsigned min_complete, uint64_t timeout_ns) {
+    if (!ext_arg_) return -ENOSYS;
+    __kernel_timespec ts;
+    ts.tv_sec = (long long)(timeout_ns / 1000000000ull);
+    ts.tv_nsec = (long long)(timeout_ns % 1000000000ull);
+    io_uring_getevents_arg arg;
+    memset(&arg, 0, sizeof arg);
+    arg.sigmask_sz = _NSIG / 8;
+    arg.ts = (uint64_t)(uintptr_t)&ts;
+    int r = (int)syscall(__NR_io_uring_enter, fd_, pending_, min_complete,
+                         IORING_ENTER_GETEVENTS | IORING_ENTER_EXT_ARG, &arg, sizeof arg);
+    if (r < 0) return -errno;
+    pending_ -= (unsigned)r <= pending_ ? (unsigned)r : pending_;
+    return r;
+  }
+  bool peek(io_uring_cqe *out) {
+    unsigned head = *cq_head_;
+    if (head == __atomic_load_n(cq_tail_, __ATOMIC_ACQUIRE)) return false;
+    *out = cqes_[head & cq_mask_];
+    __atomic_store_n(cq_head_, head + 1, __ATOMIC_RELEASE);
+    return true;
+  }
+  unsigned pending() const { return pending_; }
+  bool ok() const { return fd_ >= 0; }
+  void unregister_buffers() {
+    (void)syscall(__NR_io_uring_register, fd_, IORING_UNREGISTER_BUFFERS, nullptr, 0u);
+  }
+  int register_buffer(void *p, size_t len) {
+    iovec iov{p, len};
+    int r = (int)syscall(__NR_io_uring_register, fd_, IORING_REGISTER_BUFFERS, &iov, 1u);
+    return r < 0 ? -errno : 0;
+  }
+
+ private:
+  int fail() {
+    int e = errno;
+    close_ring();
+    return -e;
+  }
+  void close_ring() {
+    if (sqes_ && sqes_ != MAP_FAILED) munmap(sqes_, sqe_sz_);
+    if (cq_ptr_ && cq_ptr_ != MAP_FAILED && cq_ptr_ != sq_ptr_) munmap(cq_ptr_, cq_sz_);
+    if (sq_ptr_ && sq_ptr_ != MAP_FAILED) munmap(sq_ptr_, sq_sz_);
+    if (fd_ >= 0) close(fd_);
+    fd_ = -1;
+    sqes_ = nullptr;
+    sq_ptr_ = cq_ptr_ = nullptr;
+  }
+  int fd_ = -1;
+  void *sq_ptr_ = nullptr, *cq_ptr_ = nullptr;
+  size_t sq_sz_ = 0, cq_sz_ = 0, sqe_sz_ = 0;
+  io_uring_sqe *sqes_ = nullptr;
+  io_uring_cqe *cqes_ = nullptr;
+  unsigned *sq_head_ = nullptr, *sq_tail_ = nullptr, *sq_array_ = nullptr;
+  unsigned *cq_head_ = nullptr, *cq_tail_ = nullptr;
+  unsigned sq_mask_ = 0, cq_mask_ = 0, entries_ = 0, pending_ = 0;
+  bool ext_arg_ = false;
+};
+
+}
diff --git a/nvme_strom_amd/api.py b/nvme_strom_amd/api.py
--- a/nvme_strom_amd/api.py
+++ b/nvme_strom_amd/api.py
@@ -122,7 +122,7 @@
 
 
 def io_prof(reset: bool = False) -> dict:
-    n = 2 + len(IO_PROF_PHASES) + len(IO_PROF_COUNTS) + 4
+    n = 2 + len(IO_PROF_PHASES) + len(IO_PROF_COUNTS) + 4 + 6
     out = np.zeros(n, dtype=np.uint64)
     _check(N.lib().strom_io_prof(out.ctypes.data, n, 1 if reset else 0), "io_prof")
     khz = max(int(out[1]), 1)
@@ -133,7 +133,13 @@
     caller = dict(calls=int(out[c0]), **{k: round(int(out[c0 + 1 + i]) * 1e6 / khz / req, 1)
                                          for i, k in enumerate(("plan_ns_per_req", "build_ns_per_req",
                                                                 "submit_ns_per_req"))})
+    x = c0 + 4
+    nbytes, cpu_s = int(out[x + 3]), int(out[x + 2]) / 1e9
     return dict(workers=int(out[0]), tsc_khz=khz, ns=ns, counts=cnt, caller=caller,
+                wait_blocked_ns=int(out[x]) * 1e6 / khz, wait_poll_ns=int(out[x + 1]) * 1e6 / khz,
+                worker_cpu_s=cpu_s, bytes=nbytes,
+                cpu_s_per_gib=round(cpu_s / (nbytes / (1 << 30)), 6) if nbytes else None,
+                caller_wait_cpu_s=int(out[x + 4]) / 1e9, caller_wait_wall_s=int(out[x + 5]) / 1e9,
                 ns_per_req={k: round(v / req, 1) for k, v in ns.items()},
                 busy_ns_per_req=round(sum(v for k, v in ns.items() if k != "idle") / req, 1))
 
```

Result: slower. 20.24 (-4.0%).
